# leggedrobotics/wild_visual_navigation

Measured on NVIDIA H100. Metric: frames/sec end-to-end (DINO feat + seg + MLP train-step) at 448x448, higher is better.
Workload: dtype bf16 operands / fp32 accumulate (ViT, STEGO head, per-pixel MLP); fp32 (k-means, train step)

## Files before the change

include/wvn_b200.h:

```cpp
#ifndef WVN_B200_H_
#define WVN_B200_H_

#include <stddef.h>
#include <stdint.h>

#ifdef __cplusplus
extern "C" {
#endif

typedef enum {
  WVN_STATUS_OK = 0,
  WVN_STATUS_INVALID = -1,
  WVN_STATUS_CUDA = -2,
  WVN_STATUS_NO_DEVICE = -3,
  WVN_STATUS_STATE = -4
} wvn_status;

const char* wvn_last_error(void);
int wvn_check_device(void);
int wvn_version(void);
long long wvn_launch_count(void);
void wvn_profile_enable(int category_mask);
int wvn_profile_collect(float* host_ms, long long* host_launches);

int wvn_gemm_bf16(const void* a_bf16, long long lda, const void* w_bf16, const float* bias, void* out, long long ldo,
                  int m, int n, int k, int out_kind, int act, int block_n, void* stream);

typedef struct {
  int m, n, k;
  int epi, act;
  int block_n;
  const void* a;
  long long lda;
  const void* w;
  const float* bias;
  void* out;
  long long ldo;
  const float* pos;
  int tokens_in, npad;
  int dim, heads;
  void* q_out;
  void* k_out;
  void* vt_out;
  int feat, trav_col;
  const void* x;
  long long ldx;
  float* trav;
  float* conf;
  float* loss_reco;
  const float* cg_mean;
  const float* cg_std;
  float cg_std_factor;
  int reverse_m;
  int registers;
  const void* residual;
  long long ldr;
} wvn_gemm_ex_args;
int wvn_gemm_bf16_ex(const wvn_gemm_ex_args* args, void* stream);

int wvn_attention_bf16(const void* q, const void* k, const void* vt, void* out, int batch, int heads, int npad,
                       int n_valid, float scale, void* stream);

int wvn_layernorm(const float* x, const float* gamma, const float* beta, void* out_bf16, long long rows, int dim,
                  float eps, void* stream);

typedef struct wvn_vit wvn_vit_t;

typedef struct {
  int image_size;
  int patch_size;
  int dim;
  int depth;
  int heads;
  int mlp_dim;
  int max_batch;
  int chunk;
  float ln_eps;
  int head_out;
  int registers;
} wvn_vit_config;

int wvn_vit_create(const wvn_vit_config* cfg, wvn_vit_t** out);
void wvn_vit_destroy(wvn_vit_t* h);

int wvn_vit_set_weight(wvn_vit_t* h, const char* name, const float* data, long long numel);

int wvn_vit_forward(wvn_vit_t* h, const float* img, int batch, int in_h, int in_w, int resized_h, int resized_w,
                    float* tokens_out, void* stream);

int wvn_vit_forward_tta(wvn_vit_t* h, const float* img, int batch, int in_h, int in_w, int resized_h, int resized_w,
                        float* tokens_out, void* stream);

int wvn_vit_forward_u8(wvn_vit_t* h, const unsigned char* img_hwc, int batch, int in_h, int in_w, int resized_h,
                       int resized_w, float* tokens_out, void* stream);

int wvn_vit_stego_head(wvn_vit_t* h, int batch, float* out, void* stream);
int wvn_vit_npad(const wvn_vit_t* h);

typedef struct wvn_resnet wvn_resnet_t;

typedef struct {
  int image_size;
  int depth;
  int max_batch;
} wvn_resnet_config;

int wvn_resnet_create(const wvn_resnet_config* cfg, wvn_resnet_t** out);
void wvn_resnet_destroy(wvn_resnet_t* h);
size_t wvn_resnet_workspace_bytes(const wvn_resnet_t* h);
int wvn_resnet_set_weight(wvn_resnet_t* h, const char* name, const float* data, long long numel);
int wvn_resnet_forward(wvn_resnet_t* h, const float* img, int batch, void* const* taps, void* stream);

int wvn_im2col_bf16_nhwc(const void* in, int batch, int h, int w, int c, int k, int stride, int pad, void* out,
                         long long pitch, void* stream);
int wvn_im2col_image(const float* img, int batch, int h, int w, int k, int stride, int pad, void* out, long long pitch,
                     void* stream);
int wvn_maxpool3s2_bf16_nhwc(const void* in, int batch, int h, int w, int c, void* out, void* stream);

int wvn_upsample_dense(const float* tokens, float* out, int batch, int dim, int gh, int gw, int out_h, int out_w,
                       void* stream);
int wvn_logits_argmax(const float* logits, long long ld, int col0, int classes, int col0_b, int classes_b, int batch,
                      int npad, int gh, int gw, int out_h, int out_w, long long* seg, long long* seg_b, void* stream);

int wvn_flip_average(float* head, int batch, int npad, int grid, long long ld, void* stream);
size_t wvn_stego_kmeans_workspace_bytes(int batch, int k, int code_dim);
int wvn_stego_kmeans(float* rows, long long ld, int batch, int npad, int patches, int code_col, int code_dim, int logit_col,
                     int k, int iters, float* centroids_out, void* workspace, void* stream);

size_t wvn_segment_workspace_bytes(int batch, int smax, int gh, int gw);
int wvn_segment_reduce(const long long* seg, int batch, int h, int w, int smax, const float* tokens, int gh, int gw,
                       int dim, float* feat, float* centers, long long* edges, int* n_edges, int max_edges,
                       void* workspace, void* stream);
int wvn_segment_pool_pyramid(const long long* seg, int batch, int h, int w, int smax, const float* centers,
                             void* const* taps, const int* tap_h, const int* tap_w, const int* tap_c, float* out,
                             void* stream);
int wvn_segment_relabel(long long* seg, int batch, long long pix_per_frame, int num_labels, int* scratch, int* counts,
                        void* stream);

int wvn_supervision_pool(const long long* seg, const float* mask, int batch, int channels, int h, int w, int smax,
                         float* y, unsigned char* y_valid, float* count_ws, void* stream);

void wvn_slic_tables(int* g256, int* m9, int* f4096);
int wvn_slic_geometry(int h, int w, int num_components, int* grid_interval, int* nx, int* ny);
size_t wvn_slic_workspace_bytes(int batch, int h, int w, int num_components);
int wvn_slic(const float* img, int batch, int h, int w, int num_components, float compactness, int iters,
             const int* lut_g, const int* lut_m, const int* lut_f, long long* labels, void* workspace, void* stream);

int wvn_project_and_render(const float* K, const float* pose_camera_in_world, const float* points, const float* colors,
                           int color_batched, int batch, int n_points, int h, int w, const float* traversability,
                           float* masks, float* projected, unsigned char* valid, float* supervision_inout, void* stream);

typedef struct wvn_mlp_infer wvn_mlp_infer_t;
int wvn_mlp_infer_create(int dim, int h1, int h2, int chunk_rows, wvn_mlp_infer_t** out);
void wvn_mlp_infer_destroy(wvn_mlp_infer_t* h);
int wvn_mlp_infer_reserve(wvn_mlp_infer_t* h, int tokens_per_frame);
int wvn_mlp_infer_set_params(wvn_mlp_infer_t* h, const float* params, void* stream);
int wvn_mlp_infer_pixels(wvn_mlp_infer_t* h, const float* tokens, int batch, int gh, int gw, int out_h, int out_w,
                         const float* cg_mean, const float* cg_std, float std_factor, float* trav, float* conf,
                         void* stream);
int wvn_mlp_infer_pixels_vit(wvn_mlp_infer_t* h, wvn_vit_t* vit, int batch, int out_h, int out_w, const float* cg_mean,
                             const float* cg_std, float std_factor, float* trav, float* conf, void* stream);
int wvn_mlp_infer_rows(wvn_mlp_infer_t* h, const float* x, long long rows, const float* cg_mean,
                       const float* cg_std, float std_factor, float* trav, float* conf, void* stream);

typedef struct {
  float w_trav, w_reco, std_factor;
  int anomaly_balanced;
  float lr, beta1, beta2, eps;
} wvn_train_config;

size_t wvn_mlp_param_count(int dim, int h1, int h2);
size_t wvn_mlp_train_workspace_bytes(int dim, int h1, int h2, int max_rows);
size_t wvn_mlp_train_scalars_bytes(void);
int wvn_mlp_train_forward_stats(int dim, int h1, int h2, const float* params, const float* x, const float* y,
                                const unsigned char* y_valid, int rows, int max_rows, void* workspace, void* scalars,
                                void* stream);
int wvn_mlp_train_backward(int dim, int h1, int h2, const float* params, const float* x, const float* y,
                           const unsigned char* y_valid, int rows, int max_rows, long long n_total,
                           const wvn_train_config* cfg, void* workspace, void* scalars, float* cg_mean, float* cg_std,
                           float* grads, float* confidence_out, void* stream);
int wvn_mlp_train_apply(int dim, int h1, int h2, float* params, const float* grads, float* exp_avg, float* exp_avg_sq,
                        long long* step_counter, long long n_total, const wvn_train_config* cfg, void* scalars,
                        void* stream);
int wvn_mlp_train_read_metrics(const void* scalars, float* metrics_out, void* stream);
int wvn_mlp_forward_f32(int dim, int h1, int h2, const float* params, const float* x, int rows, float* h1_buf,
                        float* h2_buf, float* out, void* stream);

typedef struct wvn_mlp_trainer wvn_mlp_trainer_t;
size_t wvn_mlp_trainer_scalars_bytes(void);
int wvn_mlp_trainer_create(int dim, int h1, int h2, int max_rows, const wvn_train_config* cfg, void* scalars,
                           float* grads, wvn_mlp_trainer_t** out);
void wvn_mlp_trainer_destroy(wvn_mlp_trainer_t* t);
int wvn_comm_unique_id(void* id128);
int wvn_mlp_trainer_init_comm(wvn_mlp_trainer_t* t, const void* id128, int rank, int world);
int wvn_mlp_trainer_set_confidence(wvn_mlp_trainer_t* t, int method, float* var, double* running_n, double* running_sum,
                                   double* running_sum_of_squares, float kf_proc_cov, float kf_meas_cov);
int wvn_mlp_trainer_copy_confidence(wvn_mlp_trainer_t* dst, const wvn_mlp_trainer_t* src, void* stream);
int wvn_mlp_train_step(wvn_mlp_trainer_t* t, float* params, float* exp_avg, float* exp_avg_sq, long long* step_counter,
                       const float* x, int groups, int rows_per_group, const int* n_rows, const float* y,
                       const unsigned char* y_valid, float* cg_mean, float* cg_std, float* confidence_out,
                       float* metrics_out, int phase_mask, void* stream);

typedef struct wvn_flow wvn_flow_t;
typedef struct {
  const float* mask0;
  const float* mask1;
  const long long* p1;
  const long long* invp1;
  const long long* p3;
  const long long* invp3;
} wvn_flow_buffers;
size_t wvn_flow_param_count(int dim, int hidden);
int wvn_flow_create(int dim, int hidden, int max_rows, const wvn_train_config* cfg, float* grads, wvn_flow_t** out);
void wvn_flow_destroy(wvn_flow_t* h);
int wvn_flow_set_confidence(wvn_flow_t* h, int method, float* var, double* running_n, double* running_sum,
                            double* running_sum_of_squares, float kf_proc_cov, float kf_meas_cov);
int wvn_flow_copy_confidence(wvn_flow_t* dst, const wvn_flow_t* src, void* stream);
int wvn_flow_train_step(wvn_flow_t* h, float* params, float* exp_avg, float* exp_avg_sq, long long* step_counter,
                        const wvn_flow_buffers* buffers, const float* x, int rows, const unsigned char* y_valid,
                        float* cg_mean, float* cg_std, float* confidence_out, float* metrics_out, int phase_mask,
                        void* stream);

typedef struct wvn_flow_infer wvn_flow_infer_t;
int wvn_flow_infer_create(int dim, int hidden, int max_rows, int chunk_pixels, wvn_flow_infer_t** out);
void wvn_flow_infer_destroy(wvn_flow_infer_t* h);
int wvn_flow_infer_set_params(wvn_flow_infer_t* h, const float* params, void* stream);
int wvn_flow_infer_rows(wvn_flow_infer_t* h, const float* params, const wvn_flow_buffers* buffers, const float* x, int rows,
                        float* z, float* log_det, float* logprob, const float* cg_mean, const float* cg_std,
                        float std_factor, float* trav, void* stream);
int wvn_flow_infer_pixels(wvn_flow_infer_t* h, const wvn_flow_buffers* buffers, const float* tokens, int batch, int gh,
                          int gw, int out_h, int out_w, const float* cg_mean, const float* cg_std, float std_factor,
                          float* trav, float* nll, void* stream);

#ifdef __cplusplus
}
#endif
#endif
```

wild_visual_navigation_b200/_C.py:

```python
from __future__ import annotations

import ctypes
import os
from ctypes import POINTER, Structure, byref, c_char_p, c_float, c_int, c_longlong, c_size_t, c_void_p

import torch

_HERE = os.path.dirname(os.path.abspath(__file__))
LIB_PATH = os.environ.get("WVN_B200_LIB", os.path.join(_HERE, "libwvn_b200.so"))


class WvnError(RuntimeError):
    pass


class VitConfig(Structure):
    _fields_ = [
        ("image_size", c_int), ("patch_size", c_int), ("dim", c_int), ("depth", c_int), ("heads", c_int),
        ("mlp_dim", c_int), ("max_batch", c_int), ("chunk", c_int), ("ln_eps", c_float), ("head_out", c_int),
        ("registers", c_int),
    ]


class GemmExArgs(Structure):
    _fields_ = [
        ("m", c_int), ("n", c_int), ("k", c_int), ("epi", c_int), ("act", c_int), ("block_n", c_int),
        ("a", c_void_p), ("lda", c_longlong), ("w", c_void_p), ("bias", c_void_p), ("out", c_void_p), ("ldo", c_longlong),
        ("pos", c_void_p), ("tokens_in", c_int), ("npad", c_int), ("dim", c_int), ("heads", c_int),
        ("q_out", c_void_p), ("k_out", c_void_p), ("vt_out", c_void_p),
        ("feat", c_int), ("trav_col", c_int), ("x", c_void_p), ("ldx", c_longlong), ("trav", c_void_p),
        ("conf", c_void_p), ("loss_reco", c_void_p), ("cg_mean", c_void_p), ("cg_std", c_void_p),
        ("cg_std_factor", c_float), ("reverse_m", c_int), ("registers", c_int), ("residual", c_void_p), ("ldr", c_longlong),
    ]


class ResnetConfig(Structure):
    _fields_ = [("image_size", c_int), ("depth", c_int), ("max_batch", c_int)]


class TrainConfig(Structure):
    _fields_ = [
        ("w_trav", c_float), ("w_reco", c_float), ("std_factor", c_float), ("anomaly_balanced", c_int),
        ("lr", c_float), ("beta1", c_float), ("beta2", c_float), ("eps", c_float),
    ]


class FlowBuffers(Structure):
    _fields_ = [("mask0", c_void_p), ("mask1", c_void_p), ("p1", c_void_p), ("invp1", c_void_p), ("p3", c_void_p),
                ("invp3", c_void_p)]


_lib = None

_P, _I, _L, _F, _S = c_void_p, c_int, c_longlong, c_float, c_size_t
SIGNATURES = {
    "wvn_last_error": (c_char_p, []),
    "wvn_check_device": (_I, []),
    "wvn_version": (_I, []),
    "wvn_launch_count": (_L, []),
    "wvn_profile_enable": (None, [_I]),
    "wvn_profile_collect": (_I, [_P, _P]),
    "wvn_gemm_bf16": (_I, [_P, _L, _P, _P, _P, _L, _I, _I, _I, _I, _I, _I, _P]),
    "wvn_gemm_bf16_ex": (_I, [POINTER(GemmExArgs), _P]),
    "wvn_attention_bf16": (_I, [_P, _P, _P, _P, _I, _I, _I, _I, _F, _P]),
    "wvn_layernorm": (_I, [_P, _P, _P, _P, _L, _I, _F, _P]),
    "wvn_vit_create": (_I, [POINTER(VitConfig), POINTER(_P)]),
    "wvn_vit_destroy": (None, [_P]),
    "wvn_vit_set_weight": (_I, [_P, c_char_p, _P, _L]),
    "wvn_vit_forward": (_I, [_P, _P, _I, _I, _I, _I, _I, _P, _P]),
    "wvn_vit_forward_u8": (_I, [_P, _P, _I, _I, _I, _I, _I, _P, _P]),
    "wvn_vit_forward_tta": (_I, [_P, _P, _I, _I, _I, _I, _I, _P, _P]),
    "wvn_vit_stego_head": (_I, [_P, _I, _P, _P]),
    "wvn_vit_npad": (_I, [_P]),
    "wvn_resnet_create": (_I, [POINTER(ResnetConfig), POINTER(_P)]),
    "wvn_resnet_destroy": (None, [_P]),
    "wvn_resnet_workspace_bytes": (_S, [_P]),
    "wvn_resnet_set_weight": (_I, [_P, c_char_p, _P, _L]),
    "wvn_resnet_forward": (_I, [_P, _P, _I, _P, _P]),
    "wvn_im2col_bf16_nhwc": (_I, [_P, _I, _I, _I, _I, _I, _I, _I, _P, _L, _P]),
    "wvn_im2col_image": (_I, [_P, _I, _I, _I, _I, _I, _I, _P, _L, _P]),
    "wvn_maxpool3s2_bf16_nhwc": (_I, [_P, _I, _I, _I, _I, _P, _P]),
    "wvn_segment_pool_pyramid": (_I, [_P, _I, _I, _I, _I, _P, _P, _P, _P, _P, _P, _P]),
    "wvn_upsample_dense": (_I, [_P, _P, _I, _I, _I, _I, _I, _I, _P]),
    "wvn_logits_argmax": (_I, [_P, _L, _I, _I, _I, _I, _I, _I, _I, _I, _I, _I, _P, _P, _P]),
    "wvn_flip_average": (_I, [_P, _I, _I, _I, _L, _P]),
    "wvn_stego_kmeans_workspace_bytes": (_S, [_I, _I, _I]),
    "wvn_stego_kmeans": (_I, [_P, _L, _I, _I, _I, _I, _I, _I, _I, _I, _P, _P, _P]),
    "wvn_segment_workspace_bytes": (_S, [_I, _I, _I, _I]),
    "wvn_segment_reduce": (_I, [_P, _I, _I, _I, _I, _P, _I, _I, _I, _P, _P, _P, _P, _I, _P, _P]),
    "wvn_segment_relabel": (_I, [_P, _I, _L, _I, _P, _P, _P]),
    "wvn_supervision_pool": (_I, [_P, _P, _I, _I, _I, _I, _I, _P, _P, _P, _P]),
    "wvn_slic_tables": (None, [_P, _P, _P]),
    "wvn_slic_geometry": (_I, [_I, _I, _I, _P, _P, _P]),
    "wvn_slic_workspace_bytes": (_S, [_I, _I, _I, _I]),
    "wvn_slic": (_I, [_P, _I, _I, _I, _I, _F, _I, _P, _P, _P, _P, _P, _P]),
    "wvn_project_and_render": (_I, [_P, _P, _P, _P, _I, _I, _I, _I, _I, _P, _P, _P, _P, _P, _P]),
    "wvn_mlp_infer_create": (_I, [_I, _I, _I, _I, POINTER(_P)]),
    "wvn_mlp_infer_destroy": (None, [_P]),
    "wvn_mlp_infer_reserve": (_I, [_P, _I]),
    "wvn_mlp_infer_set_params": (_I, [_P, _P, _P]),
    "wvn_mlp_infer_pixels": (_I, [_P, _P, _I, _I, _I, _I, _I, _P, _P, _F, _P, _P, _P]),
    "wvn_mlp_infer_pixels_vit": (_I, [_P, _P, _I, _I, _I, _P, _P, _F, _P, _P, _P]),
    "wvn_mlp_infer_rows": (_I, [_P, _P, _L, _P, _P, _F, _P, _P, _P]),
    "wvn_mlp_param_count": (_S, [_I, _I, _I]),
    "wvn_mlp_train_workspace_bytes": (_S, [_I, _I, _I, _I]),
    "wvn_mlp_train_scalars_bytes": (_S, []),
    "wvn_mlp_train_forward_stats": (_I, [_I, _I, _I, _P, _P, _P, _P, _I, _I, _P, _P, _P]),
    "wvn_mlp_train_backward": (_I, [_I, _I, _I, _P, _P, _P, _P, _I, _I, _L, POINTER(TrainConfig), _P, _P, _P, _P, _P, _P, _P]),
    "wvn_mlp_train_apply": (_I, [_I, _I, _I, _P, _P, _P, _P, _P, _L, POINTER(TrainConfig), _P, _P]),
    "wvn_mlp_train_read_metrics": (_I, [_P, _P, _P]),
    "wvn_mlp_forward_f32": (_I, [_I, _I, _I, _P, _P, _I, _P, _P, _P, _P]),
    "wvn_mlp_trainer_scalars_bytes": (_S, []),
    "wvn_mlp_trainer_create": (_I, [_I, _I, _I, _I, POINTER(TrainConfig), _P, _P, POINTER(_P)]),
    "wvn_mlp_trainer_destroy": (None, [_P]),
    "wvn_comm_unique_id": (_I, [_P]),
    "wvn_mlp_trainer_init_comm": (_I, [_P, _P, _I, _I]),
    "wvn_mlp_trainer_set_confidence": (_I, [_P, _I, _P, _P, _P, _P, _F, _F]),
    "wvn_mlp_trainer_copy_confidence": (_I, [_P, _P, _P]),
    "wvn_mlp_train_step": (_I, [_P, _P, _P, _P, _P, _P, _I, _I, _P, _P, _P, _P, _P, _P, _P, _I, _P]),
    "wvn_flow_param_count": (_S, [_I, _I]),
    "wvn_flow_create": (_I, [_I, _I, _I, POINTER(TrainConfig), _P, POINTER(_P)]),
    "wvn_flow_destroy": (None, [_P]),
    "wvn_flow_set_confidence": (_I, [_P, _I, _P, _P, _P, _P, _F, _F]),
    "wvn_flow_copy_confidence": (_I, [_P, _P, _P]),
    "wvn_flow_infer_create": (_I, [_I, _I, _I, _I, POINTER(_P)]),
    "wvn_flow_infer_destroy": (None, [_P]),
    "wvn_flow_infer_set_params": (_I, [_P, _P, _P]),
    "wvn_flow_infer_rows": (_I, [_P, _P, POINTER(FlowBuffers), _P, _I, _P, _P, _P, _P, _P, _F, _P, _P]),
    "wvn_flow_infer_pixels": (_I, [_P, POINTER(FlowBuffers), _P, _I, _I, _I, _I, _I, _P, _P, _F, _P, _P, _P]),
    "wvn_flow_train_step": (_I, [_P, _P, _P, _P, _P, POINTER(FlowBuffers), _P, _I, _P, _P, _P, _P, _P, _I, _P]),
}


def lib() -> ctypes.CDLL:
    global _lib
    if _lib is not None:
        return _lib
    if not os.path.exists(LIB_PATH):
        raise WvnError(
            f"{LIB_PATH} not found: build it with `python -c 'import __graft_entry__ as g; g.build()'` "
            "or `make -C wild_visual_navigation_b200/csrc` (there is no CPU fallback)"
        )
    l = ctypes.CDLL(LIB_PATH)
    for name, (res, args) in SIGNATURES.items():
        fn = getattr(l, name)
        fn.restype = res
        fn.argtypes = args
    _lib = l
    return l


def check(status: int) -> None:
    if status != 0:
        msg = lib().wvn_last_error()
        raise WvnError(f"libwvn_b200 error {status}: {msg.decode() if msg else '?'}")


def require_device() -> None:
    if not torch.cuda.is_available():
        raise WvnError("wild_visual_navigation_b200 needs a CUDA (sm_90a) device; no CPU fallback exists")
    check(lib().wvn_check_device())


def ptr(t) -> c_void_p:
    if t is None:
        return c_void_p(0)
    assert t.is_cuda and t.is_contiguous(), "expected a contiguous CUDA tensor"
    return c_void_p(t.data_ptr())


def stream() -> c_void_p:
    return c_void_p(torch.cuda.current_stream().cuda_stream)
```

wild_visual_navigation_b200/csrc/api.cu:

```cuda
#include <cuda_bf16.h>

#include <stdio.h>
#include <stdlib.h>

#include <map>
#include <string>
#include <vector>

#include "../../include/wvn_b200.h"
#include "attention.h"
#include "dense_kernels.h"
#include "gemm.h"
#include "host_common.h"
#include "mlp_train.h"
#include "mlp_train_fused.h"
#include "pixel_head.h"
#include "resnet_kernels.h"
#include "segment_kernels.h"
#include "flow_train.h"
#include "footprint_kernels.h"
#include "slic_kernels.h"
#include "stego_kmeans.h"
#include "train_core.h"
#include "vit_kernels.h"

using namespace wvn;

namespace {

inline cudaStream_t S(void* s) { return reinterpret_cast<cudaStream_t>(s); }
inline int round_up(int v, int m) { return (v + m - 1) / m * m; }

__global__ void cast_f32_to_bf16_kernel(const float* __restrict__ src, __nv_bfloat16* __restrict__ dst, long long n) {
  for (long long i = blockIdx.x * static_cast<long long>(blockDim.x) + threadIdx.x; i < n;
       i += static_cast<long long>(gridDim.x) * blockDim.x)
    dst[i] = __float2bfloat16_rn(src[i]);
}

__global__ void cast_rows_kernel(const float* __restrict__ src, __nv_bfloat16* __restrict__ dst, long long rows, int dim,
                                 long long ld) {
  const long long n = rows * dim;
  for (long long i = blockIdx.x * static_cast<long long>(blockDim.x) + threadIdx.x; i < n;
       i += static_cast<long long>(gridDim.x) * blockDim.x) {
    const long long r = i / dim;
    const int c = static_cast<int>(i - r * dim);
    dst[r * ld + c] = __float2bfloat16_rn(src[i]);
  }
}

int cast_to_bf16(const float* src, void* dst, long long n, cudaStream_t s) {
  if (n <= 0) return WVN_OK;
  int blocks = static_cast<int>(std::min<long long>((n + 255) / 256, 4096));
  cast_f32_to_bf16_kernel<<<blocks, 256, 0, s>>>(src, reinterpret_cast<__nv_bfloat16*>(dst), n);
  WVN_CHECK_LAUNCH("cast_f32_to_bf16_kernel");
  return WVN_OK;
}

struct DevBuf {
  void* p = nullptr;
  size_t bytes = 0;
  int alloc(size_t n) {
    bytes = n;
    WVN_CHECK_CUDA(cudaMalloc(&p, n ? n : 1));
    WVN_CHECK_CUDA(cudaMemset(p, 0, n ? n : 1));
    return WVN_OK;
  }
  void release() {
    if (p) cudaFree(p);
    p = nullptr;
  }
};

struct Weight {
  void* p = nullptr;
  long long numel = 0;
  bool bf16 = false;
  bool loaded = false;
  int cols = 0, ld = 0;
};

}

struct wvn_vit {
  wvn_vit_config cfg;
  int grid = 0, P = 0, t0 = 1, n_valid = 0, npad = 0, kpe = 0, kpe_ld = 0, chunk = 0;
  std::map<std::string, Weight> w;
  std::vector<DevBuf> owned;
  DevBuf x, xn, q, k, vt, attn, hid, ape, stage;
  DevBuf tok_bf16, head_hidden;
  DevBuf qkv_f32;
  bool precise = false;
  bool forwarded = false;
  int last_batch = 0;

  int add_weight(const std::string& name, long long numel, bool bf16, int cols = 0, int ld = 0) {
    DevBuf b;
    const long long stored = cols > 0 ? numel / cols * ld : numel;
    WVN_PROPAGATE(b.alloc(static_cast<size_t>(stored) * (bf16 ? 2 : 4)));
    owned.push_back(b);
    Weight wt;
    wt.p = b.p; wt.numel = numel; wt.bf16 = bf16; wt.cols = cols; wt.ld = ld;
    w[name] = wt;
    return WVN_OK;
  }
  template <class T>
  T* wp(const std::string& name) { return reinterpret_cast<T*>(w[name].p); }
};

extern "C" {

const char* wvn_last_error(void) { return last_error(); }
int wvn_version(void) { return 104; }

int wvn_check_device(void) {
  int n = 0;
  if (cudaGetDeviceCount(&n) != cudaSuccess || n == 0) return set_error(WVN_ERR_NO_DEVICE, "no CUDA device visible");
  int dev = 0;
  cudaGetDevice(&dev);
  int major = 0;
  cudaDeviceGetAttribute(&major, cudaDevAttrComputeCapabilityMajor, dev);
  int minor = 0;
  cudaDeviceGetAttribute(&minor, cudaDevAttrComputeCapabilityMinor, dev);
  if (major != 9 || minor != 0)
    return set_error(WVN_ERR_NO_DEVICE, "device %d has compute capability %d.%d, need 9.0 (sm_90a)", dev, major, minor);
  return WVN_OK;
}

long long wvn_launch_count(void) { return launch_count(); }
void wvn_profile_enable(int category_mask) { prof_enable(category_mask); }
int wvn_profile_collect(float* host_ms, long long* host_launches) {
  WVN_REQUIRE(host_ms && host_launches, "wvn_profile_collect: null argument");
  return prof_collect(host_ms, host_launches);
}

int wvn_gemm_bf16(const void* a, long long lda, const void* w, const float* bias, void* out, long long ldo, int m, int n,
                  int k, int out_kind, int act, int block_n, void* stream) {
  GemmArgs g;
  g.M = m; g.N = n; g.K = k;
  g.epi = out_kind == 0 ? EPI_BF16 : (out_kind == 1 ? EPI_F32 : EPI_RESID_F32);
  WVN_REQUIRE(out_kind >= 0 && out_kind <= 2, "wvn_gemm_bf16: out_kind %d", out_kind);
  g.act = act; g.bias = bias; g.out = out; g.ldo = ldo;
  return gemm_bf16(g, a, lda, w, block_n, S(stream));
}

int wvn_gemm_bf16_ex(const wvn_gemm_ex_args* x, void* stream) {
  WVN_REQUIRE(x, "wvn_gemm_bf16_ex: null argument");
  GemmArgs g;
  g.M = x->m; g.N = x->n; g.K = x->k; g.epi = x->epi; g.act = x->act;
  g.bias = x->bias; g.out = x->out; g.ldo = x->ldo;
  g.pos = x->pos; g.tokens_in = x->tokens_in; g.npad = x->npad;
  g.dim = x->dim; g.heads = x->heads; g.q = x->q_out; g.k = x->k_out; g.vt = x->vt_out;
  g.feat = x->feat; g.trav_col = x->trav_col; g.x = x->x; g.ldx = x->ldx; g.trav = x->trav; g.conf = x->conf;
  g.loss_reco = x->loss_reco; g.cg_mean = x->cg_mean; g.cg_std = x->cg_std; g.cg_std_factor = x->cg_std_factor;
  g.reverse_m = x->reverse_m; g.registers = x->registers;
  g.residual = x->residual; g.ldr = x->ldr;
  return gemm_bf16(g, x->a, x->lda, x->w, x->block_n, S(stream));
}

int wvn_attention_bf16(const void* q, const void* k, const void* vt, void* out, int batch, int heads, int npad,
                       int n_valid, float scale, void* stream) {
  AttnArgs a;
  a.batch = batch; a.heads = heads; a.npad = npad; a.n_valid = n_valid;
  a.scale_log2 = scale * 1.4426950408889634f;
  a.out = out; a.ldo = static_cast<long long>(heads) * 64;
  return attention_bf16(a, q, k, vt, S(stream));
}

int wvn_layernorm(const float* x, const float* gamma, const float* beta, void* out_bf16, long long rows, int dim,
                  float eps, void* stream) {
  LayerNormArgs a;
  a.rows = rows; a.dim = dim; a.eps = eps;
  return layernorm_rows(x, gamma, beta, out_bf16, nullptr, a, S(stream));
}

int wvn_vit_create(const wvn_vit_config* cfg, wvn_vit_t** out) {
  WVN_REQUIRE(cfg && out, "wvn_vit_create: null argument");
  WVN_PROPAGATE(wvn_check_device());
  WVN_REQUIRE(cfg->dim == 384 || cfg->dim == 768, "vit: dim %d unsupported (384, 768)", cfg->dim);
  WVN_REQUIRE(cfg->heads * 64 == cfg->dim, "vit: heads*64 must equal dim");
  WVN_REQUIRE(cfg->patch_size == 8 || cfg->patch_size == 14 || cfg->patch_size == 16, "vit: patch size %d unsupported",
              cfg->patch_size);
  WVN_REQUIRE(cfg->image_size >= cfg->patch_size, "vit: image size too small");
  WVN_REQUIRE(cfg->mlp_dim % 64 == 0 && cfg->depth > 0 && cfg->max_batch > 0, "vit: bad mlp_dim/depth/max_batch");
  WVN_REQUIRE(cfg->head_out % 64 == 0, "vit: head_out must be a multiple of 64");
  WVN_REQUIRE(cfg->registers >= 0, "vit: registers must be >= 0");
  WVN_REQUIRE(cfg->registers == 0 || cfg->head_out == 0, "vit: register tokens and a STEGO head cannot be combined");
  wvn_vit* h = new wvn_vit();
  h->cfg = *cfg;
  if (h->cfg.ln_eps <= 0.f) h->cfg.ln_eps = 1e-6f;
  h->grid = cfg->image_size / cfg->patch_size;
  h->P = h->grid * h->grid;
  h->t0 = 1 + cfg->registers;
  h->n_valid = h->t0 + h->P;
  h->npad = round_up(h->n_valid, 128);
  h->kpe = 3 * cfg->patch_size * cfg->patch_size;
  h->kpe_ld = patch_pitch(cfg->patch_size);
  h->chunk = cfg->chunk > 0 ? cfg->chunk : 8;
  if (h->chunk > cfg->max_batch) h->chunk = cfg->max_batch;
  const int D = cfg->dim;
  int rc = WVN_OK;
  auto add = [&](const std::string& n, long long numel, bool bf) { if (rc == WVN_OK) rc = h->add_weight(n, numel, bf); };
  add("cls_token", D, false);
  add("pos_embed", static_cast<long long>(1 + h->P) * D, false);
  if (cfg->registers > 0) add("register_tokens", static_cast<long long>(cfg->registers) * D, false);
  if (rc == WVN_OK) rc = h->add_weight("patch_embed.proj.weight", static_cast<long long>(D) * h->kpe, true, h->kpe, h->kpe_ld);
  add("patch_embed.proj.bias", D, false);
  for (int i = 0; i < cfg->depth; ++i) {
    const std::string b = "blocks." + std::to_string(i) + ".";
    add(b + "norm1.weight", D, false);
    add(b + "norm1.bias", D, false);
    add(b + "attn.qkv.weight", 3ll * D * D, true);
    add(b + "attn.qkv.bias", 3 * D, false);
    add(b + "attn.proj.weight", static_cast<long long>(D) * D, true);
    add(b + "attn.proj.bias", D, false);
    add(b + "norm2.weight", D, false);
    add(b + "norm2.bias", D, false);
    add(b + "mlp.fc1.weight", static_cast<long long>(cfg->mlp_dim) * D, true);
    add(b + "mlp.fc1.bias", cfg->mlp_dim, false);
    add(b + "mlp.fc2.weight", static_cast<long long>(D) * cfg->mlp_dim, true);
    add(b + "mlp.fc2.bias", D, false);
  }
  add("norm.weight", D, false);
  add("norm.bias", D, false);
  if (cfg->head_out > 0) {
    add("stego.head_a.weight", static_cast<long long>(cfg->head_out) * D, true);
    add("stego.head_a.bias", cfg->head_out, false);
    add("stego.hidden.weight", static_cast<long long>(D) * D, true);
    add("stego.hidden.bias", D, false);
    add("stego.head_b.weight", static_cast<long long>(cfg->head_out) * D, true);
  }
  const size_t rows = static_cast<size_t>(h->chunk) * h->npad;
  const size_t bh = static_cast<size_t>(h->chunk) * cfg->heads;
  auto alloc = [&](DevBuf& b, size_t bytes) { if (rc == WVN_OK) rc = b.alloc(bytes); };
  alloc(h->x, rows * D * 4);
  alloc(h->xn, rows * D * 2);
  alloc(h->q, bh * h->npad * 64 * 2);
  alloc(h->k, bh * h->npad * 64 * 2);
  alloc(h->vt, bh * 64 * h->npad * 2);
  alloc(h->attn, rows * D * 2);
  alloc(h->hid, rows * cfg->mlp_dim * 2);
  alloc(h->ape, static_cast<size_t>(h->chunk) * h->P * h->kpe_ld * 2);
  alloc(h->stage, 8u << 20);
  alloc(h->tok_bf16, static_cast<size_t>(cfg->max_batch) * h->npad * D * 2);
  if (cfg->head_out > 0) alloc(h->head_hidden, static_cast<size_t>(cfg->max_batch) * h->npad * D * 2);
  {
    const char* e = getenv("WVN_VIT_PRECISE");
    h->precise = e && atoi(e) == 1;
    if (h->precise) alloc(h->qkv_f32, rows * 3 * D * 4);
  }
  if (rc != WVN_OK) {
    wvn_vit_destroy(h);
    return rc;
  }
  *out = h;
  return WVN_OK;
}

void wvn_vit_destroy(wvn_vit_t* h) {
  if (!h) return;
  for (auto& b : h->owned) b.release();
  for (DevBuf* b : {&h->x, &h->xn, &h->q, &h->k, &h->vt, &h->attn, &h->hid, &h->ape, &h->stage, &h->tok_bf16,
                    &h->head_hidden, &h->qkv_f32})
    b->release();
  delete h;
}

int wvn_vit_npad(const wvn_vit_t* h) { return h ? h->npad : 0; }

static int load_weight(Weight& wt, DevBuf& stage, const char* name, const float* data, long long numel) {
  WVN_REQUIRE(wt.numel == numel, "set_weight: '%s' expects %lld elements, got %lld", name, wt.numel, numel);
  cudaPointerAttributes attr;
  bool on_device = false;
  if (cudaPointerGetAttributes(&attr, data) == cudaSuccess)
    on_device = (attr.type == cudaMemoryTypeDevice || attr.type == cudaMemoryTypeManaged);
  else
    cudaGetLastError();
  if (!wt.bf16) {
    WVN_CHECK_CUDA(cudaMemcpy(wt.p, data, numel * 4, on_device ? cudaMemcpyDeviceToDevice : cudaMemcpyHostToDevice));
  } else if (wt.cols > 0) {
    const long long chunk_rows = static_cast<long long>(stage.bytes / 4) / wt.cols;
    const long long rows = numel / wt.cols;
    for (long long r0 = 0; r0 < rows; r0 += chunk_rows) {
      const long long n = std::min(chunk_rows, rows - r0);
      const float* src = data + r0 * wt.cols;
      if (!on_device) {
        WVN_CHECK_CUDA(cudaMemcpy(stage.p, src, n * wt.cols * 4, cudaMemcpyHostToDevice));
        src = reinterpret_cast<const float*>(stage.p);
      }
      const int blocks = static_cast<int>(std::min<long long>((n * wt.cols + 255) / 256, 4096));
      cast_rows_kernel<<<blocks, 256, 0, 0>>>(src, reinterpret_cast<__nv_bfloat16*>(wt.p) + r0 * wt.ld, n, wt.cols, wt.ld);
      WVN_CHECK_LAUNCH("cast_rows_kernel");
      WVN_CHECK_CUDA(cudaStreamSynchronize(0));
    }
  } else {
    const long long chunk_elems = static_cast<long long>(stage.bytes / 4);
    for (long long off = 0; off < numel; off += chunk_elems) {
      const long long n = std::min(chunk_elems, numel - off);
      const float* src = data + off;
      if (!on_device) {
        WVN_CHECK_CUDA(cudaMemcpy(stage.p, src, n * 4, cudaMemcpyHostToDevice));
        src = reinterpret_cast<const float*>(stage.p);
      }
      WVN_PROPAGATE(cast_to_bf16(src, reinterpret_cast<__nv_bfloat16*>(wt.p) + off, n, 0));
      WVN_CHECK_CUDA(cudaStreamSynchronize(0));
    }
  }
  wt.loaded = true;
  return WVN_OK;
}


int wvn_vit_set_weight(wvn_vit_t* h, const char* name, const float* data, long long numel) {
  WVN_REQUIRE(h && name && data, "wvn_vit_set_weight: null argument");
  auto it = h->w.find(name);
  WVN_REQUIRE(it != h->w.end(), "wvn_vit_set_weight: unknown weight '%s'", name);
  return load_weight(it->second, h->stage, name, data, numel);
}

static int vit_check_loaded(wvn_vit* h, bool need_head) {
  for (auto& kv : h->w) {
    const bool is_head = kv.first.rfind("stego.", 0) == 0;
    if (is_head && !need_head) continue;
    if (!kv.second.loaded) return set_error(WVN_ERR_STATE, "vit: weight '%s' was never set", kv.first.c_str());
  }
  return WVN_OK;
}

constexpr int kDefaultSubAttn = 1 << 30;

namespace {
int vit_forward_impl(wvn_vit_t* h, const void* img, bool u8_hwc, int batch, int in_h, int in_w, int resized_h, int resized_w,
                     float* tokens_out, void* stream, bool flip_tta = false);
}

int wvn_vit_forward_tta(wvn_vit_t* h, const float* img, int batch, int in_h, int in_w, int resized_h, int resized_w,
                        float* tokens_out, void* stream) {
  return vit_forward_impl(h, img, false, batch, in_h, in_w, resized_h, resized_w, tokens_out, stream, true);
}

int wvn_vit_forward(wvn_vit_t* h, const float* img, int batch, int in_h, int in_w, int resized_h, int resized_w,
                    float* tokens_out, void* stream) {
  return vit_forward_impl(h, img, false, batch, in_h, in_w, resized_h, resized_w, tokens_out, stream);
}

int wvn_vit_forward_u8(wvn_vit_t* h, const unsigned char* img_hwc, int batch, int in_h, int in_w, int resized_h,
                       int resized_w, float* tokens_out, void* stream) {
  return vit_forward_impl(h, img_hwc, true, batch, in_h, in_w, resized_h, resized_w, tokens_out, stream);
}

namespace {
int vit_forward_impl(wvn_vit_t* h, const void* img, bool u8_hwc, int src_batch, int in_h, int in_w, int resized_h, int resized_w,
                     float* tokens_out, void* stream, bool flip_tta) {
  const int batch = flip_tta ? 2 * src_batch : src_batch;
  WVN_REQUIRE(h && img, "wvn_vit_forward: null argument");
  WVN_REQUIRE(batch > 0 && batch <= h->cfg.max_batch, "wvn_vit_forward: batch %d outside (0, %d]", batch, h->cfg.max_batch);
  WVN_REQUIRE(resized_h >= h->cfg.image_size && resized_w >= h->cfg.image_size,
              "wvn_vit_forward: resized image %dx%d smaller than the crop %d", resized_h, resized_w, h->cfg.image_size);
  WVN_PROPAGATE(vit_check_loaded(h, false));
  cudaStream_t s = S(stream);
  const wvn_vit_config& c = h->cfg;
  const int D = c.dim;

  ImagePatchArgs ia;
  ia.in_h = in_h; ia.in_w = in_w; ia.patch = c.patch_size; ia.grid_h = h->grid; ia.grid_w = h->grid;
  ia.crop_top = static_cast<int>(lrintf((resized_h - c.image_size) / 2.0f));
  ia.crop_left = static_cast<int>(lrintf((resized_w - c.image_size) / 2.0f));
  ia.scale_y = static_cast<float>(in_h) / static_cast<float>(resized_h);
  ia.scale_x = static_cast<float>(in_w) / static_cast<float>(resized_w);

  for (int b0 = 0; b0 < batch; b0 += h->chunk) {
    const int nb = std::min(h->chunk, batch - b0);
    const int rows = nb * h->npad;
    float* x = reinterpret_cast<float*>(h->x.p);
    ia.batch = nb;
    ia.frame0 = b0; ia.src_frames = src_batch; ia.flip_from = flip_tta ? src_batch : (1 << 30);
    WVN_PROPAGATE(image_to_patches(img, u8_hwc, h->ape.p, ia, s));
    const float* reg = c.registers > 0 ? h->wp<float>("register_tokens") : nullptr;
    WVN_PROPAGATE(init_token_rows(x, h->wp<float>("cls_token"), h->wp<float>("pos_embed"), reg, c.registers, nb, h->npad,
                                  h->n_valid, D, s));
    {
      GemmArgs g;
      g.M = nb * h->P; g.N = D; g.K = h->kpe; g.epi = EPI_PATCH; g.bias = h->wp<float>("patch_embed.proj.bias");
      g.out = x; g.ldo = D; g.pos = h->wp<float>("pos_embed"); g.tokens_in = h->P; g.npad = h->npad;
      g.registers = c.registers;
      WVN_PROPAGATE(gemm_bf16(g, h->ape.p, h->kpe_ld, h->wp<void>("patch_embed.proj.weight"), 0, s));
    }
    LayerNormArgs la;
    la.rows = rows; la.dim = D; la.eps = c.ln_eps; la.npad = h->npad; la.n_valid = h->n_valid; la.row0 = h->t0;
    static int sub_env = -1;
    if (sub_env < 0) {
      const char* e = getenv("WVN_VIT_SUBCHUNK");
      sub_env = e ? atoi(e) : (1 << 30);
      if (sub_env < 1) sub_env = 1 << 30;
    }
    const int sub = std::min(sub_env, nb);
    static int snake = -1;
    if (snake < 0) { const char* e = getenv("WVN_VIT_SNAKE"); snake = (e && atoi(e) == 0) ? 0 : 1; }
    int dir = 0;
    auto next_dir = [&]() { dir = snake ? dir ^ 1 : 0; return dir; };
    __nv_bfloat16* xn = reinterpret_cast<__nv_bfloat16*>(h->xn.p);
    __nv_bfloat16* attn = reinterpret_cast<__nv_bfloat16*>(h->attn.p);
    static int sub_attn_env = -1;
    if (sub_attn_env < 0) {
      const char* e = getenv("WVN_VIT_SUB_ATTN");
      sub_attn_env = e ? atoi(e) : kDefaultSubAttn;
      if (sub_attn_env < 1) sub_attn_env = 1 << 30;
    }
    const int sub_a = std::min(sub_attn_env, nb);
    for (int l = 0; l < c.depth; ++l) {
      const std::string b = "blocks." + std::to_string(l) + ".";
      for (int s0 = 0; s0 < nb; s0 += sub_a) {
        const int ns = std::min(sub_a, nb - s0);
        const long long roff = static_cast<long long>(s0) * h->npad;
        LayerNormArgs ls = la;
        ls.rows = static_cast<long long>(ns) * h->npad;
        ls.reverse = next_dir();
        WVN_PROPAGATE(layernorm_rows(x + roff * D, h->wp<float>(b + "norm1.weight"), h->wp<float>(b + "norm1.bias"),
                                     xn + roff * D, nullptr, ls, s));
        if (h->precise) {
          GemmArgs g;
          float* qkv = reinterpret_cast<float*>(h->qkv_f32.p) + roff * 3 * D;
          g.M = ns * h->npad; g.N = 3 * D; g.K = D; g.epi = EPI_F32; g.bias = h->wp<float>(b + "attn.qkv.bias");
          g.out = qkv; g.ldo = 3 * D;
          WVN_PROPAGATE(gemm_bf16(g, xn + roff * D, D, h->wp<void>(b + "attn.qkv.weight"), 0, s));
          WVN_PROPAGATE(attention_f32_debug(qkv, attn + roff * D, ns, c.heads, h->npad, h->n_valid, D, 0.125f, s));
          continue;
        }
        GemmArgs g;
        g.M = ns * h->npad; g.N = 3 * D; g.K = D; g.epi = EPI_QKV; g.bias = h->wp<float>(b + "attn.qkv.bias");
        g.npad = h->npad; g.dim = D; g.heads = c.heads;
        const long long hoff = static_cast<long long>(s0) * c.heads * h->npad * 64;
        g.q = reinterpret_cast<__nv_bfloat16*>(h->q.p) + hoff;
        g.k = reinterpret_cast<__nv_bfloat16*>(h->k.p) + hoff;
        g.vt = reinterpret_cast<__nv_bfloat16*>(h->vt.p) + hoff;
        g.reverse_m = next_dir();
        WVN_PROPAGATE(gemm_bf16(g, xn + roff * D, D, h->wp<void>(b + "attn.qkv.weight"), 0, s));
        AttnArgs a;
        a.batch = ns; a.heads = c.heads; a.npad = h->npad; a.n_valid = h->n_valid;
        a.scale_log2 = 0.125f * 1.4426950408889634f;
        a.out = attn + roff * D; a.ldo = D;
        a.reverse = next_dir();
        WVN_PROPAGATE(attention_bf16(a, g.q, g.k, g.vt, s));
      }
      for (int s0 = 0; s0 < nb; s0 += sub) {
        const int ns = std::min(sub, nb - s0);
        const long long roff = static_cast<long long>(s0) * h->npad;
        const int srows = ns * h->npad;
        LayerNormArgs ls = la;
        ls.rows = srows;
        {
          GemmArgs g;
          g.M = srows; g.N = D; g.K = D; g.epi = EPI_RESID_F32; g.bias = h->wp<float>(b + "attn.proj.bias");
          g.out = x + roff * D; g.ldo = D;
          g.reverse_m = next_dir();
          WVN_PROPAGATE(gemm_bf16(g, attn + roff * D, D, h->wp<void>(b + "attn.proj.weight"), 0, s));
        }
        ls.reverse = next_dir();
        WVN_PROPAGATE(layernorm_rows(x + roff * D, h->wp<float>(b + "norm2.weight"), h->wp<float>(b + "norm2.bias"),
                                     xn + roff * D, nullptr, ls, s));
        {
          GemmArgs g;
          g.M = srows; g.N = c.mlp_dim; g.K = D; g.epi = EPI_BF16; g.act = ACT_GELU;
          g.bias = h->wp<float>(b + "mlp.fc1.bias"); g.out = h->hid.p; g.ldo = c.mlp_dim;
          g.reverse_m = next_dir();
          WVN_PROPAGATE(gemm_bf16(g, xn + roff * D, D, h->wp<void>(b + "mlp.fc1.weight"), 0, s));
        }
        {
          GemmArgs g;
          g.M = srows; g.N = D; g.K = c.mlp_dim; g.epi = EPI_RESID_F32; g.bias = h->wp<float>(b + "mlp.fc2.bias");
          g.out = x + roff * D; g.ldo = D;
          g.reverse_m = next_dir();
          WVN_PROPAGATE(gemm_bf16(g, h->hid.p, c.mlp_dim, h->wp<void>(b + "mlp.fc2.weight"), 0, s));
        }
      }
    }
    __nv_bfloat16* tok_bf = reinterpret_cast<__nv_bfloat16*>(h->tok_bf16.p) + static_cast<long long>(b0) * h->npad * D;
    float* tok_f = tokens_out ? tokens_out + static_cast<long long>(b0) * h->P * D : nullptr;
    la.reverse = next_dir();
    WVN_PROPAGATE(layernorm_rows(x, h->wp<float>("norm.weight"), h->wp<float>("norm.bias"), tok_bf, tok_f, la, s));
  }
  h->forwarded = true;
  h->last_batch = batch;
  return WVN_OK;
}
}

int wvn_vit_stego_head(wvn_vit_t* h, int batch, float* out, void* stream) {
  WVN_REQUIRE(h && out, "wvn_vit_stego_head: null argument");
  WVN_REQUIRE(h->cfg.head_out > 0, "wvn_vit_stego_head: handle was created without a head");
  WVN_REQUIRE(h->forwarded && batch == h->last_batch, "wvn_vit_stego_head: call wvn_vit_forward with the same batch first");
  WVN_PROPAGATE(vit_check_loaded(h, true));
  cudaStream_t s = S(stream);
  const int D = h->cfg.dim, rows = batch * h->npad, HO = h->cfg.head_out;
  GemmArgs g;
  g.M = rows; g.N = D; g.K = D; g.epi = EPI_BF16; g.act = ACT_RELU; g.bias = h->wp<float>("stego.hidden.bias");
  g.out = h->head_hidden.p; g.ldo = D;
  WVN_PROPAGATE(gemm_bf16(g, h->tok_bf16.p, D, h->wp<void>("stego.hidden.weight"), 0, s));
  GemmArgs a;
  a.M = rows; a.N = HO; a.K = D; a.epi = EPI_F32; a.bias = h->wp<float>("stego.head_a.bias"); a.out = out; a.ldo = HO;
  WVN_PROPAGATE(gemm_bf16(a, h->tok_bf16.p, D, h->wp<void>("stego.head_a.weight"), 0, s));
  GemmArgs b;
  b.M = rows; b.N = HO; b.K = D; b.epi = EPI_RESID_F32; b.bias = nullptr; b.out = out; b.ldo = HO;
  WVN_PROPAGATE(gemm_bf16(b, h->head_hidden.p, D, h->wp<void>("stego.head_b.weight"), 0, s));
  return WVN_OK;
}

int wvn_upsample_dense(const float* tokens, float* out, int batch, int dim, int gh, int gw, int out_h, int out_w,
                       void* stream) {
  DenseArgs a;
  a.batch = batch; a.dim = dim; a.grid_h = gh; a.grid_w = gw; a.out_h = out_h; a.out_w = out_w;
  a.scale_y = out_h > 1 ? static_cast<float>(gh - 1) / static_cast<float>(out_h - 1) : 0.f;
  a.scale_x = out_w > 1 ? static_cast<float>(gw - 1) / static_cast<float>(out_w - 1) : 0.f;
  return upsample_tokens_dense(tokens, out, a, S(stream));
}

int wvn_logits_argmax(const float* logits, long long ld, int col0, int classes, int col0_b, int classes_b, int batch,
                      int npad, int gh, int gw, int out_h, int out_w, long long* seg, long long* seg_b, void* stream) {
  LogitsArgs a;
  a.batch = batch; a.classes = classes; a.grid_h = gh; a.grid_w = gw; a.out_h = out_h; a.out_w = out_w;
  a.scale_y = static_cast<float>(gh) / static_cast<float>(out_h);
  a.scale_x = static_cast<float>(gw) / static_cast<float>(out_w);
  a.npad = npad; a.ld = ld; a.col0 = col0; a.col0_b = col0_b; a.classes_b = classes_b;
  return logits_argmax(logits, seg, seg_b, a, S(stream));
}

int wvn_flip_average(float* head, int batch, int npad, int grid, long long ld, void* stream) {
  return flip_average(head, batch, npad, grid, ld, S(stream));
}

size_t wvn_stego_kmeans_workspace_bytes(int batch, int k, int code_dim) { return stego_kmeans_workspace_bytes(batch, k, code_dim); }

int wvn_stego_kmeans(float* rows, long long ld, int batch, int npad, int patches, int code_col, int code_dim, int logit_col,
                     int k, int iters, float* centroids_out, void* workspace, void* stream) {
  KmeansArgs a;
  a.batch = batch; a.npad = npad; a.patches = patches; a.ld = ld; a.code_col = code_col; a.code_dim = code_dim;
  a.logit_col = logit_col; a.k = k; a.iters = iters; a.centroids_out = centroids_out;
  return stego_kmeans(rows, a, reinterpret_cast<float*>(workspace), S(stream));
}

static void seg_ws_layout(int batch, int smax, int gh, int gw, size_t& off_w, size_t& off_adj, size_t& total) {
  const size_t stats = static_cast<size_t>(batch) * smax * 3 * sizeof(unsigned long long);
  off_w = (stats + 255) / 256 * 256;
  const size_t wbytes = static_cast<size_t>(batch) * smax * gh * gw * sizeof(float);
  off_adj = off_w + (wbytes + 255) / 256 * 256;
  total = off_adj + static_cast<size_t>(batch) * smax * ((smax + 31) / 32) * sizeof(unsigned int);
}

size_t wvn_segment_workspace_bytes(int batch, int smax, int gh, int gw) {
  size_t a, b, t;
  seg_ws_layout(batch, smax, gh, gw, a, b, t);
  return t;
}

int wvn_segment_reduce(const long long* seg, int batch, int h, int w, int smax, const float* tokens, int gh, int gw,
                       int dim, float* feat, float* centers, long long* edges, int* n_edges, int max_edges,
                       void* workspace, void* stream) {
  WVN_REQUIRE(seg && workspace, "wvn_segment_reduce: null argument");
  WVN_REQUIRE(feat == nullptr || tokens != nullptr, "wvn_segment_reduce: feat requested without tokens");
  WVN_REQUIRE((edges == nullptr) == (n_edges == nullptr), "wvn_segment_reduce: edges and n_edges go together");
  WVN_REQUIRE(feat == nullptr || w <= h, "wvn_segment_reduce: segment map %dx%d is wider than the (h, h) feature map", h, w);
  size_t off_w, off_adj, total;
  seg_ws_layout(batch, smax, gh, gw, off_w, off_adj, total);
  char* ws = reinterpret_cast<char*>(workspace);
  unsigned long long* stats = reinterpret_cast<unsigned long long*>(ws);
  float* wseg = feat ? reinterpret_cast<float*>(ws + off_w) : nullptr;
  unsigned int* adj = edges ? reinterpret_cast<unsigned int*>(ws + off_adj) : nullptr;
  SegmentArgs a;
  a.batch = batch; a.h = h; a.w = w; a.smax = smax; a.grid_h = gh; a.grid_w = gw; a.dim = dim;
  a.scale_y = h > 1 ? static_cast<float>(gh - 1) / static_cast<float>(h - 1) : 0.f;
  a.scale_x = h > 1 ? static_cast<float>(gw - 1) / static_cast<float>(h - 1) : 0.f;
  WVN_PROPAGATE(segment_accumulate(seg, a, stats, wseg, adj, S(stream)));
  if (feat || centers) WVN_PROPAGATE(segment_pool(wseg, tokens, stats, feat, centers, a, S(stream)));
  if (edges) WVN_PROPAGATE(adjacency_emit(adj, edges, n_edges, batch, smax, max_edges, S(stream)));
  return WVN_OK;
}

int wvn_segment_relabel(long long* seg, int batch, long long pix_per_frame, int num_labels, int* scratch, int* counts,
                        void* stream) {
  return relabel_compact(seg, scratch, counts, batch, pix_per_frame, num_labels, S(stream));
}

int wvn_supervision_pool(const long long* seg, const float* mask, int batch, int channels, int h, int w, int smax,
                         float* y, unsigned char* y_valid, float* count_ws, void* stream) {
  WVN_REQUIRE(seg && mask && y && y_valid && count_ws, "wvn_supervision_pool: null argument");
  return supervision_pool(seg, mask, batch, channels, h, w, smax, y, y_valid, count_ws, S(stream));
}

void wvn_slic_tables(int* g256, int* m9, int* f4096) { slic_tables(g256, m9, f4096); }

int wvn_slic_geometry(int h, int w, int num_components, int* grid_interval, int* nx, int* ny) {
  WVN_REQUIRE(h > 0 && w > 0 && num_components > 0 && grid_interval && nx && ny, "wvn_slic_geometry: bad argument");
  slic_geometry(h, w, num_components, grid_interval, nx, ny);
  return WVN_OK;
}

size_t wvn_slic_workspace_bytes(int batch, int h, int w, int num_components) {
  return slic_workspace_bytes(batch, h, w, num_components);
}

int wvn_slic(const float* img, int batch, int h, int w, int num_components, float compactness, int iters,
             const int* lut_g, const int* lut_m, const int* lut_f, long long* labels, void* workspace, void* stream) {
  WVN_REQUIRE(img && lut_g && lut_m && lut_f && labels && workspace, "wvn_slic: null argument");
  return slic_segment(img, batch, h, w, num_components, compactness, iters, lut_g, lut_m, lut_f, labels, workspace,
                      S(stream));
}

int wvn_project_and_render(const float* K, const float* pose_camera_in_world, const float* points, const float* colors,
                           int color_batched, int batch, int n_points, int h, int w, const float* traversability,
                           float* masks, float* projected, unsigned char* valid, float* supervision_inout, void* stream) {
  WVN_REQUIRE(K && pose_camera_in_world && points, "wvn_project_and_render: null argument");
  WVN_REQUIRE(colors || (!masks && !supervision_inout), "wvn_project_and_render: colors are required to render");
  FootprintArgs a;
  a.batch = batch; a.n_points = n_points; a.h = h; a.w = w; a.color_batched = color_batched;
  return footprint_render(a, K, pose_camera_in_world, points, colors, traversability, masks, projected, valid,
                          supervision_inout, S(stream));
}

}

struct wvn_resnet {
  wvn_resnet_config cfg;
  int bottleneck = 0;
  std::map<std::string, Weight> w;
  std::vector<DevBuf> owned;
  DevBuf stage, col;
  DevBuf act[5];
};

namespace {

enum ResnetPass { RN_REGISTER, RN_SIZE, RN_RUN };

const int kBlocks18[4] = {2, 2, 2, 2};
const int kBlocks50[4] = {3, 4, 6, 3};

struct ResnetRun {
  wvn_resnet* h;
  ResnetPass pass;
  int batch;
  cudaStream_t s;
  size_t need_col = 0, need_act[5] = {0, 0, 0, 0, 0};
  int rc = WVN_OK;

  void conv(const std::string& name, const void* in, int H, int W, int C, int k, int stride, int pad, int Cout,
            void* out, int role, bool relu, const void* residual, int* Ho_, int* Wo_, const float* img = nullptr,
            bool stem = false) {
    const int Ho = (H + 2 * pad - k) / stride + 1, Wo = (W + 2 * pad - k) / stride + 1;
    *Ho_ = Ho; *Wo_ = Wo;
    if (rc != WVN_OK) return;
    const int K = k * k * C;
    const long long M = static_cast<long long>(batch) * Ho * Wo;
    const bool direct = k == 1 && stride == 1 && !stem;
    const long long pitch = gemm_w_pitch(K);
    if (pass == RN_REGISTER) {
      wvn_resnet& r = *h;
      DevBuf b;
      if ((rc = b.alloc(static_cast<size_t>(Cout) * pitch * 2)) != WVN_OK) return;
      r.owned.push_back(b);
      Weight wt;
      wt.p = b.p; wt.numel = static_cast<long long>(Cout) * K; wt.bf16 = true; wt.cols = K; wt.ld = static_cast<int>(pitch);
      r.w[name + ".weight"] = wt;
      DevBuf bb;
      if ((rc = bb.alloc(static_cast<size_t>(Cout) * 4)) != WVN_OK) return;
      r.owned.push_back(bb);
      Weight wb;
      wb.p = bb.p; wb.numel = Cout;
      r.w[name + ".bias"] = wb;
      return;
    }
    if (pass == RN_SIZE) {
      if (!direct) need_col = std::max(need_col, static_cast<size_t>(M * pitch * 2));
      if (role >= 0) need_act[role] = std::max(need_act[role], static_cast<size_t>(M * Cout * 2));
      return;
    }
    const void* A = in;
    long long lda = C;
    if (!direct) {
      rc = stem ? im2col_image(img, batch, H, W, k, stride, pad, h->col.p, pitch, s)
               : im2col_nhwc(in, batch, H, W, C, k, stride, pad, h->col.p, pitch, s);
      if (rc != WVN_OK) return;
      A = h->col.p;
      lda = pitch;
    }
    if (M > 0x7fffffff) {
      rc = set_error(WVN_ERR_INVALID, "resnet: %lld output rows", M);
      return;
    }
    GemmArgs g;
    g.M = static_cast<int>(M); g.N = Cout; g.K = K;
    g.epi = residual ? EPI_BF16_RESID : EPI_BF16;
    g.act = relu ? ACT_RELU : ACT_NONE;
    g.bias = reinterpret_cast<const float*>(h->w[name + ".bias"].p);
    g.out = out; g.ldo = Cout;
    g.residual = residual; g.ldr = Cout;
    rc = gemm_bf16(g, A, lda, h->w[name + ".weight"].p, 0, s);
  }

  void walk(const float* img, void* const* taps) {
    const int S = h->cfg.image_size;
    const bool bn = h->bottleneck != 0;
    const int* blocks = bn ? kBlocks50 : kBlocks18;
    void* A[5];
    for (int i = 0; i < 5; ++i) A[i] = h->act[i].p;
    void* T[4] = {nullptr, nullptr, nullptr, nullptr};
    if (taps) for (int i = 0; i < 4; ++i) T[i] = taps[i];
    int Ho, Wo;
    conv("conv1", nullptr, S, S, 3, 7, 2, 3, 64, A[2], 2, true, nullptr, &Ho, &Wo, img, true);
    int H = (Ho - 1) / 2 + 1, W = (Wo - 1) / 2 + 1, C = 64;
    if (pass == RN_SIZE) need_act[0] = std::max(need_act[0], static_cast<size_t>(batch) * H * W * C * 2);
    if (pass == RN_RUN && rc == WVN_OK) rc = maxpool3s2_nhwc(A[2], batch, Ho, Wo, 64, A[0], s);
    const void* cur = A[0];
    int cur_role = 0;
    for (int L = 1; L <= 4; ++L) {
      const int planes = 64 << (L - 1), out_c = bn ? planes * 4 : planes;
      for (int blk = 0; blk < blocks[L - 1]; ++blk) {
        const std::string p = "layer" + std::to_string(L) + "." + std::to_string(blk) + ".";
        const int stride = (blk == 0 && L > 1) ? 2 : 1;
        const int out_role = cur_role == 0 ? 1 : 0;
        const bool out_tap = bn ? (L == 4 && blk == blocks[3] - 1) : (blk == blocks[L - 1] - 1);
        void* out = out_tap ? T[bn ? 3 : L - 1] : A[out_role];
        int h1, w1, h2, w2, hd, wd;
        const void* res = cur;
        if (blk == 0 && (stride != 1 || C != out_c)) {
          conv(p + "downsample", cur, H, W, C, 1, stride, 0, out_c, A[4], 4, false, nullptr, &hd, &wd);
          res = A[4];
        }
        if (bn) {
          const bool t1_tap = blk == 0 && L >= 2;
          void* t1 = t1_tap ? T[L - 2] : A[2];
          conv(p + "conv1", cur, H, W, C, 1, 1, 0, planes, t1, t1_tap ? -1 : 2, true, nullptr, &h1, &w1);
          conv(p + "conv2", t1, h1, w1, planes, 3, stride, 1, planes, A[3], 3, true, nullptr, &h2, &w2);
          conv(p + "conv3", A[3], h2, w2, planes, 1, 1, 0, out_c, out, out_tap ? -1 : out_role, true, res, &H, &W);
        } else {
          conv(p + "conv1", cur, H, W, C, 3, stride, 1, planes, A[2], 2, true, nullptr, &h1, &w1);
          conv(p + "conv2", A[2], h1, w1, planes, 3, 1, 1, out_c, out, out_tap ? -1 : out_role, true, res, &H, &W);
        }
        C = out_c;
        cur = out;
        cur_role = out_tap ? -1 : out_role;
      }
    }
  }
};

}

extern "C" {

int wvn_resnet_create(const wvn_resnet_config* cfg, wvn_resnet_t** out) {
  WVN_REQUIRE(cfg && out, "wvn_resnet_create: null argument");
  WVN_PROPAGATE(wvn_check_device());
  WVN_REQUIRE(cfg->depth == 18 || cfg->depth == 50, "resnet: depth %d unsupported (18, 50)", cfg->depth);
  WVN_REQUIRE(cfg->image_size >= 32 && cfg->image_size % 32 == 0, "resnet: image size %d must be a multiple of 32",
              cfg->image_size);
  WVN_REQUIRE(cfg->max_batch > 0, "resnet: max_batch must be positive");
  wvn_resnet* h = new wvn_resnet();
  h->cfg = *cfg;
  h->bottleneck = cfg->depth == 50;
  ResnetRun reg{h, RN_REGISTER, cfg->max_batch, 0};
  reg.walk(nullptr, nullptr);
  ResnetRun size{h, RN_SIZE, cfg->max_batch, 0};
  size.walk(nullptr, nullptr);
  int rc = reg.rc;
  auto alloc = [&](DevBuf& b, size_t bytes) { if (rc == WVN_OK) rc = b.alloc(bytes); };
  alloc(h->stage, 8u << 20);
  alloc(h->col, size.need_col);
  for (int i = 0; i < 5; ++i) alloc(h->act[i], size.need_act[i]);
  if (rc != WVN_OK) {
    wvn_resnet_destroy(h);
    return rc;
  }
  *out = h;
  return WVN_OK;
}

void wvn_resnet_destroy(wvn_resnet_t* h) {
  if (!h) return;
  for (auto& b : h->owned) b.release();
  h->stage.release();
  h->col.release();
  for (auto& b : h->act) b.release();
  delete h;
}

size_t wvn_resnet_workspace_bytes(const wvn_resnet_t* h) {
  if (!h) return 0;
  size_t n = h->col.bytes;
  for (const auto& b : h->act) n += b.bytes;
  return n;
}

int wvn_resnet_set_weight(wvn_resnet_t* h, const char* name, const float* data, long long numel) {
  WVN_REQUIRE(h && name && data, "wvn_resnet_set_weight: null argument");
  auto it = h->w.find(name);
  WVN_REQUIRE(it != h->w.end(), "wvn_resnet_set_weight: unknown weight '%s'", name);
  return load_weight(it->second, h->stage, name, data, numel);
}

int wvn_resnet_forward(wvn_resnet_t* h, const float* img, int batch, void* const* taps, void* stream) {
  WVN_REQUIRE(h && img && taps, "wvn_resnet_forward: null argument");
  WVN_REQUIRE(batch > 0 && batch <= h->cfg.max_batch, "wvn_resnet_forward: batch %d outside (0, %d]", batch,
              h->cfg.max_batch);
  for (int i = 0; i < 4; ++i) WVN_REQUIRE(taps[i], "wvn_resnet_forward: tap %d is null", i);
  for (auto& kv : h->w)
    if (!kv.second.loaded) return set_error(WVN_ERR_STATE, "resnet: weight '%s' was never set", kv.first.c_str());
  ResnetRun run{h, RN_RUN, batch, S(stream)};
  run.walk(img, taps);
  return run.rc;
}

int wvn_im2col_bf16_nhwc(const void* in, int batch, int h, int w, int c, int k, int stride, int pad, void* out,
                         long long pitch, void* stream) {
  return im2col_nhwc(in, batch, h, w, c, k, stride, pad, out, pitch, S(stream));
}

int wvn_im2col_image(const float* img, int batch, int h, int w, int k, int stride, int pad, void* out, long long pitch,
                     void* stream) {
  return im2col_image(img, batch, h, w, k, stride, pad, out, pitch, S(stream));
}

int wvn_maxpool3s2_bf16_nhwc(const void* in, int batch, int h, int w, int c, void* out, void* stream) {
  return maxpool3s2_nhwc(in, batch, h, w, c, out, S(stream));
}

int wvn_segment_pool_pyramid(const long long* seg, int batch, int h, int w, int smax, const float* centers,
                             void* const* taps, const int* tap_h, const int* tap_w, const int* tap_c, float* out,
                             void* stream) {
  WVN_REQUIRE(taps && tap_h && tap_w && tap_c, "wvn_segment_pool_pyramid: null argument");
  PyramidArgs a;
  a.batch = batch; a.h = h; a.w = w; a.smax = smax;
  for (int l = 0; l < 4; ++l) {
    a.taps[l] = taps[l]; a.th[l] = tap_h[l]; a.tw[l] = tap_w[l]; a.tc[l] = tap_c[l];
  }
  return segment_pool_pyramid(seg, centers, a, out, S(stream));
}

}

struct wvn_mlp_infer {
  int dim, h1, h2;
  int dim_p, h1_p, h2_p, n3, n3_p, bn3, trav_col;
  int chunk_rows;
  DevBuf w1, b1, w2, b2, w3, b3;
  DevBuf x, a1, a2;
  DevBuf wcat, bias_cat, head_consts, tok_bf16, gu, gram;
  int fused_tokens = 0;
  int force_unfused = 0;
  bool loaded = false;
};

static constexpr int kFusedFrames = 8;

namespace {

__global__ void pack_mlp_kernel(const float* __restrict__ p, MlpOffsets o, int dim, int h1, int h2, int dim_p, int h1_p,
                                int h2_p, int n3_p, int trav_col, __nv_bfloat16* w1, float* b1, __nv_bfloat16* w2,
                                float* b2, __nv_bfloat16* w3, float* b3) {
  const long long n1 = static_cast<long long>(h1_p) * dim_p, n2 = static_cast<long long>(h2_p) * h1_p,
                  n3 = static_cast<long long>(n3_p) * h2_p;
  const long long total = n1 + n2 + n3 + h1_p + h2_p + n3_p;
  for (long long i = blockIdx.x * static_cast<long long>(blockDim.x) + threadIdx.x; i < total;
       i += static_cast<long long>(gridDim.x) * blockDim.x) {
    long long j = i;
    if (j < n1) {
      const int r = static_cast<int>(j / dim_p), c = static_cast<int>(j % dim_p);
      w1[j] = __float2bfloat16_rn((r < h1 && c < dim) ? p[o.w1 + static_cast<long long>(r) * dim + c] : 0.f);
      continue;
    }
    j -= n1;
    if (j < n2) {
      const int r = static_cast<int>(j / h1_p), c = static_cast<int>(j % h1_p);
      w2[j] = __float2bfloat16_rn((r < h2 && c < h1) ? p[o.w2 + static_cast<long long>(r) * h1 + c] : 0.f);
      continue;
    }
    j -= n2;
    if (j < n3) {
      const int r = static_cast<int>(j / h2_p), c = static_cast<int>(j % h2_p);
      int src = -1;
      if (r < dim) src = 1 + r; else if (r == trav_col) src = 0;
      w3[j] = __float2bfloat16_rn((src >= 0 && c < h2) ? p[o.w3 + static_cast<long long>(src) * h2 + c] : 0.f);
      continue;
    }
    j -= n3;
    if (j < h1_p) { b1[j] = j < h1 ? p[o.b1 + j] : 0.f; continue; }
    j -= h1_p;
    if (j < h2_p) { b2[j] = j < h2 ? p[o.b2 + j] : 0.f; continue; }
    j -= h2_p;
    {
      int src = -1;
      if (j < dim) src = 1 + static_cast<int>(j); else if (j == trav_col) src = 0;
      b3[j] = src >= 0 ? p[o.b3 + src] : 0.f;
    }
  }
}

int mlp_infer_chunk(wvn_mlp_infer* h, long long rows, long long row0, const float* cg_mean, const float* cg_std,
                    float std_factor, float* trav, float* conf, cudaStream_t s) {
  GemmArgs g1;
  g1.M = static_cast<int>(rows); g1.N = h->h1_p; g1.K = h->dim_p; g1.epi = EPI_BF16; g1.act = ACT_RELU;
  g1.bias = reinterpret_cast<float*>(h->b1.p); g1.out = h->a1.p; g1.ldo = h->h1_p;
  WVN_PROPAGATE(gemm_bf16(g1, h->x.p, h->dim_p, h->w1.p, 0, s));
  GemmArgs g2;
  g2.M = static_cast<int>(rows); g2.N = h->h2_p; g2.K = h->h1_p; g2.epi = EPI_BF16; g2.act = ACT_RELU;
  g2.bias = reinterpret_cast<float*>(h->b2.p); g2.out = h->a2.p; g2.ldo = h->h2_p;
  WVN_PROPAGATE(gemm_bf16(g2, h->a1.p, h->h1_p, h->w2.p, 0, s));
  GemmArgs g3;
  g3.M = static_cast<int>(rows); g3.N = h->n3_p; g3.K = h->h2_p; g3.epi = EPI_MLP_HEAD;
  g3.bias = reinterpret_cast<float*>(h->b3.p); g3.feat = h->dim; g3.trav_col = h->trav_col; g3.x = h->x.p;
  g3.ldx = h->dim_p; g3.trav = trav + row0; g3.conf = conf + row0; g3.cg_mean = cg_mean; g3.cg_std = cg_std;
  g3.cg_std_factor = std_factor;
  WVN_PROPAGATE(gemm_bf16(g3, h->a2.p, h->h2_p, h->w3.p, h->bn3, s));
  return WVN_OK;
}

}

extern "C" {

int wvn_mlp_infer_create(int dim, int h1, int h2, int chunk_rows, wvn_mlp_infer_t** out) {
  WVN_REQUIRE(out && dim > 0 && h1 > 0 && h2 > 0, "wvn_mlp_infer_create: bad arguments");
  WVN_PROPAGATE(wvn_check_device());
  wvn_mlp_infer* h = new wvn_mlp_infer();
  h->dim = dim; h->h1 = h1; h->h2 = h2;
  h->dim_p = round_up(dim, 64); h->h1_p = round_up(h1, 64); h->h2_p = round_up(h2, 64);
  h->trav_col = round_up(dim, 32);
  h->n3 = h->trav_col + 1;
  int best_bn = 64, best_n = round_up(h->n3, 64);
  for (int bn : {128, 192, 224, 256}) {
    const int n = round_up(h->n3, bn);
    if (n <= best_n) { best_n = n; best_bn = bn; }
  }
  h->bn3 = best_bn; h->n3_p = best_n;
  h->chunk_rows = chunk_rows > 0 ? round_up(chunk_rows, 128) : sm_count() * 128 * 3;
  int rc = WVN_OK;
  auto alloc = [&](DevBuf& b, size_t bytes) { if (rc == WVN_OK) rc = b.alloc(bytes); };
  alloc(h->w1, static_cast<size_t>(h->h1_p) * h->dim_p * 2);
  alloc(h->b1, static_cast<size_t>(h->h1_p) * 4);
  alloc(h->w2, static_cast<size_t>(h->h2_p) * h->h1_p * 2);
  alloc(h->b2, static_cast<size_t>(h->h2_p) * 4);
  alloc(h->w3, static_cast<size_t>(h->n3_p) * h->h2_p * 2);
  alloc(h->b3, static_cast<size_t>(h->n3_p) * 4);
  alloc(h->x, static_cast<size_t>(h->chunk_rows) * h->dim_p * 2);
  alloc(h->a1, static_cast<size_t>(h->chunk_rows) * h->h1_p * 2);
  alloc(h->a2, static_cast<size_t>(h->chunk_rows) * h->h2_p * 2);
  alloc(h->wcat, static_cast<size_t>(kPixelHeadN) * h->dim_p * 2);
  alloc(h->bias_cat, static_cast<size_t>(kPixelHeadN) * 4);
  alloc(h->head_consts, sizeof(PixelHeadConsts));
  {
    const char* e = getenv("WVN_PIXEL_HEAD");
    h->force_unfused = (e && std::string(e) == "unfused") ? 1 : 0;
  }
  if (rc != WVN_OK) {
    wvn_mlp_infer_destroy(h);
    return rc;
  }
  *out = h;
  return WVN_OK;
}

void wvn_mlp_infer_destroy(wvn_mlp_infer_t* h) {
  if (!h) return;
  for (DevBuf* b : {&h->w1, &h->b1, &h->w2, &h->b2, &h->w3, &h->b3, &h->x, &h->a1, &h->a2, &h->wcat, &h->bias_cat,
                    &h->head_consts, &h->tok_bf16, &h->gu, &h->gram})
    b->release();
  delete h;
}

int wvn_mlp_infer_reserve(wvn_mlp_infer_t* h, int tokens_per_frame) {
  WVN_REQUIRE(h && tokens_per_frame > 0, "wvn_mlp_infer_reserve: bad arguments");
  const int P = tokens_per_frame;
  if (h->fused_tokens >= kFusedFrames * P) return WVN_OK;
  for (DevBuf* b : {&h->tok_bf16, &h->gu, &h->gram}) b->release();
  WVN_PROPAGATE(h->tok_bf16.alloc(static_cast<size_t>(kFusedFrames) * P * h->dim_p * 2));
  WVN_PROPAGATE(h->gu.alloc(static_cast<size_t>(kFusedFrames) * P * kPixelHeadN * 4));
  WVN_PROPAGATE(h->gram.alloc(static_cast<size_t>(kFusedFrames) * P * 5 * 4));
  h->fused_tokens = kFusedFrames * P;
  return WVN_OK;
}

int wvn_mlp_infer_set_params(wvn_mlp_infer_t* h, const float* params, void* stream) {
  WVN_REQUIRE(h && params, "wvn_mlp_infer_set_params: null argument");
  MlpShape sh;
  sh.dim = h->dim; sh.h1 = h->h1; sh.h2 = h->h2;
  pack_mlp_kernel<<<256, 256, 0, S(stream)>>>(
      params, mlp_offsets(sh), h->dim, h->h1, h->h2, h->dim_p, h->h1_p, h->h2_p, h->n3_p, h->trav_col,
      reinterpret_cast<__nv_bfloat16*>(h->w1.p), reinterpret_cast<float*>(h->b1.p),
      reinterpret_cast<__nv_bfloat16*>(h->w2.p), reinterpret_cast<float*>(h->b2.p),
      reinterpret_cast<__nv_bfloat16*>(h->w3.p), reinterpret_cast<float*>(h->b3.p));
  WVN_CHECK_LAUNCH("pack_mlp_kernel");
  if (h->h1 == 256 && h->h2 == 32)
    WVN_PROPAGATE(pixel_head_pack(params, sh, h->dim_p, h->wcat.p, reinterpret_cast<float*>(h->bias_cat.p),
                                  reinterpret_cast<PixelHeadConsts*>(h->head_consts.p), S(stream)));
  h->loaded = true;
  return WVN_OK;
}

static int pixels_fused_chunk(wvn_mlp_infer_t* h, const void* tok_bf16, long long frame_rows, int row0, int b0, int nb,
                              int gh, int gw, int out_h, int out_w, int ww, const float* cg_mean, const float* cg_std,
                              float std_factor, float* trav, float* conf, cudaStream_t s) {
  const long long rows = static_cast<long long>(nb) * frame_rows;
  GemmArgs g;
  g.M = static_cast<int>(rows); g.N = kPixelHeadN; g.K = h->dim_p; g.epi = EPI_F32;
  g.bias = reinterpret_cast<float*>(h->bias_cat.p); g.out = h->gu.p; g.ldo = kPixelHeadN;
  WVN_PROPAGATE(gemm_bf16(g, tok_bf16, h->dim_p, h->wcat.p, 64, s));
  WVN_PROPAGATE(token_gram(tok_bf16, reinterpret_cast<float*>(h->gram.p), nb, gh, gw, h->dim_p, frame_rows, row0, s));
  PixelHeadArgs a;
  a.gu = reinterpret_cast<float*>(h->gu.p); a.ldg = kPixelHeadN; a.gram = reinterpret_cast<float*>(h->gram.p);
  a.consts = reinterpret_cast<PixelHeadConsts*>(h->head_consts.p);
  a.cg_mean = cg_mean; a.cg_std = cg_std; a.std_factor = std_factor;
  a.trav = trav + static_cast<long long>(b0) * out_h * out_w;
  a.conf = conf + static_cast<long long>(b0) * out_h * out_w;
  a.batch = nb; a.gh = gh; a.gw = gw; a.H = out_h; a.W = out_w;
  a.sy = static_cast<float>(gh - 1) / static_cast<float>(out_h - 1);
  a.sx = static_cast<float>(gw - 1) / static_cast<float>(out_w - 1);
  a.ww = ww; a.feat = h->dim;
  a.frame_rows = frame_rows; a.row0 = row0;
  WVN_PROPAGATE(pixel_head(a, h->w2.p, h->h1_p, s));
  return WVN_OK;
}

int wvn_mlp_infer_pixels_vit(wvn_mlp_infer_t* h, wvn_vit_t* vit, int batch, int out_h, int out_w, const float* cg_mean,
                             const float* cg_std, float std_factor, float* trav, float* conf, void* stream) {
  WVN_REQUIRE(h && vit && trav && conf && cg_mean && cg_std, "wvn_mlp_infer_pixels_vit: null argument");
  if (!h->loaded) return set_error(WVN_ERR_STATE, "wvn_mlp_infer_pixels_vit: parameters were never set");
  if (!vit->forwarded || batch > vit->last_batch)
    return set_error(WVN_ERR_STATE, "wvn_mlp_infer_pixels_vit: the backbone holds the tokens of %d frames, %d asked",
                     vit->forwarded ? vit->last_batch : 0, batch);
  WVN_REQUIRE(h->dim == vit->cfg.dim && h->dim_p == vit->cfg.dim, "wvn_mlp_infer_pixels_vit: the MLP takes %d-d features, "
              "the backbone's tokens are %d-d", h->dim, vit->cfg.dim);
  const int g = vit->grid;
  const int ww = pixel_head_supported(h->h1, h->h2, g, g, out_h, out_w);
  WVN_REQUIRE(ww > 0, "wvn_mlp_infer_pixels_vit: geometry outside the fused per-pixel head (use wvn_mlp_infer_pixels)");
  if (h->fused_tokens < kFusedFrames * vit->npad) WVN_PROPAGATE(wvn_mlp_infer_reserve(h, vit->npad));
  for (int b0 = 0; b0 < batch; b0 += kFusedFrames) {
    const int nb = std::min(kFusedFrames, batch - b0);
    const __nv_bfloat16* tok = reinterpret_cast<const __nv_bfloat16*>(vit->tok_bf16.p) +
                               static_cast<long long>(b0) * vit->npad * vit->cfg.dim;
    WVN_PROPAGATE(pixels_fused_chunk(h, tok, vit->npad, vit->t0, b0, nb, g, g, out_h, out_w, ww, cg_mean, cg_std, std_factor, trav,
                                     conf, S(stream)));
  }
  return WVN_OK;
}

int wvn_mlp_infer_pixels(wvn_mlp_infer_t* h, const float* tokens, int batch, int gh, int gw, int out_h, int out_w,
                         const float* cg_mean, const float* cg_std, float std_factor, float* trav, float* conf,
                         void* stream) {
  WVN_REQUIRE(h && tokens && trav && conf && cg_mean && cg_std, "wvn_mlp_infer_pixels: null argument");
  if (!h->loaded) return set_error(WVN_ERR_STATE, "wvn_mlp_infer_pixels: parameters were never set");
  cudaStream_t s = S(stream);
  const int ww = h->force_unfused ? 0 : pixel_head_supported(h->h1, h->h2, gh, gw, out_h, out_w);
  if (ww > 0) {
    const int P = gh * gw;
    if (h->fused_tokens < kFusedFrames * P) WVN_PROPAGATE(wvn_mlp_infer_reserve(h, P));
    for (int b0 = 0; b0 < batch; b0 += kFusedFrames) {
      const int nb = std::min(kFusedFrames, batch - b0);
      const long long rows = static_cast<long long>(nb) * P;
      const long long elems = rows * h->dim;
      int blocks = static_cast<int>(std::min<long long>((elems + 255) / 256, 8192));
      cast_rows_kernel<<<blocks, 256, 0, s>>>(tokens + static_cast<long long>(b0) * P * h->dim,
                                             reinterpret_cast<__nv_bfloat16*>(h->tok_bf16.p), rows, h->dim, h->dim_p);
      WVN_CHECK_LAUNCH("cast_rows_kernel");
      WVN_PROPAGATE(pixels_fused_chunk(h, h->tok_bf16.p, P, 0, b0, nb, gh, gw, out_h, out_w, ww, cg_mean, cg_std,
                                       std_factor, trav, conf, s));
    }
    return WVN_OK;
  }
  DenseArgs d;
  d.batch = batch; d.dim = h->dim; d.grid_h = gh; d.grid_w = gw; d.out_h = out_h; d.out_w = out_w;
  d.scale_y = out_h > 1 ? static_cast<float>(gh - 1) / static_cast<float>(out_h - 1) : 0.f;
  d.scale_x = out_w > 1 ? static_cast<float>(gw - 1) / static_cast<float>(out_w - 1) : 0.f;
  d.ld_out = h->dim_p;
  const long long total = static_cast<long long>(batch) * out_h * out_w;
  for (long long p0 = 0; p0 < total; p0 += h->chunk_rows) {
    const long long n = std::min<long long>(h->chunk_rows, total - p0);
    WVN_PROPAGATE(interp_pixel_rows(tokens, h->x.p, d, p0, n, s));
    WVN_PROPAGATE(mlp_infer_chunk(h, n, p0, cg_mean, cg_std, std_factor, trav, conf, s));
  }
  return WVN_OK;
}

int wvn_mlp_infer_rows(wvn_mlp_infer_t* h, const float* x, long long rows, const float* cg_mean, const float* cg_std,
                       float std_factor, float* trav, float* conf, void* stream) {
  WVN_REQUIRE(h && x && trav && conf && cg_mean && cg_std, "wvn_mlp_infer_rows: null argument");
  if (!h->loaded) return set_error(WVN_ERR_STATE, "wvn_mlp_infer_rows: parameters were never set");
  cudaStream_t s = S(stream);
  for (long long r0 = 0; r0 < rows; r0 += h->chunk_rows) {
    const long long n = std::min<long long>(h->chunk_rows, rows - r0);
    const long long elems = n * h->dim;
    int blocks = static_cast<int>(std::min<long long>((elems + 255) / 256, 8192));
    cast_rows_kernel<<<blocks, 256, 0, s>>>(x + r0 * h->dim, reinterpret_cast<__nv_bfloat16*>(h->x.p), n, h->dim,
                                           h->dim_p);
    WVN_CHECK_LAUNCH("cast_rows_kernel");
    WVN_PROPAGATE(mlp_infer_chunk(h, n, r0, cg_mean, cg_std, std_factor, trav, conf, s));
  }
  return WVN_OK;
}

static MlpShape shape_of(int dim, int h1, int h2) {
  MlpShape s;
  s.dim = dim; s.h1 = h1; s.h2 = h2;
  return s;
}
static LossCfg loss_of(const wvn_train_config* c) {
  LossCfg l;
  l.w_trav = c->w_trav; l.w_reco = c->w_reco; l.std_factor = c->std_factor; l.anomaly_balanced = c->anomaly_balanced;
  return l;
}

size_t wvn_mlp_param_count(int dim, int h1, int h2) { return mlp_param_count(shape_of(dim, h1, h2)); }
size_t wvn_mlp_train_workspace_bytes(int dim, int h1, int h2, int max_rows) {
  return mlp_train_workspace_floats(shape_of(dim, h1, h2), max_rows) * sizeof(float);
}
size_t wvn_mlp_train_scalars_bytes(void) { return sizeof(TrainScalars); }

int wvn_mlp_train_forward_stats(int dim, int h1, int h2, const float* params, const float* x, const float* y,
                                const unsigned char* y_valid, int rows, int max_rows, void* workspace, void* scalars,
                                void* stream) {
  WVN_REQUIRE(params && x && y && y_valid && workspace && scalars, "wvn_mlp_train_forward_stats: null argument");
  return mlp_train_forward_stats(shape_of(dim, h1, h2), params, x, y, y_valid, rows, max_rows,
                                 reinterpret_cast<float*>(workspace), reinterpret_cast<TrainScalars*>(scalars), S(stream));
}

int wvn_mlp_train_backward(int dim, int h1, int h2, const float* params, const float* x, const float* y,
                           const unsigned char* y_valid, int rows, int max_rows, long long n_total,
                           const wvn_train_config* cfg, void* workspace, void* scalars, float* cg_mean, float* cg_std,
                           float* grads, float* confidence_out, void* stream) {
  WVN_REQUIRE(params && x && y && y_valid && workspace && scalars && cfg && grads && confidence_out,
              "wvn_mlp_train_backward: null argument");
  return mlp_train_backward(shape_of(dim, h1, h2), params, x, y, y_valid, rows, max_rows, n_total, loss_of(cfg),
                            reinterpret_cast<float*>(workspace), reinterpret_cast<TrainScalars*>(scalars), cg_mean,
                            cg_std, grads, confidence_out, S(stream));
}

int wvn_mlp_train_apply(int dim, int h1, int h2, float* params, const float* grads, float* exp_avg, float* exp_avg_sq,
                        long long* step_counter, long long n_total, const wvn_train_config* cfg, void* scalars,
                        void* stream) {
  WVN_REQUIRE(params && grads && exp_avg && exp_avg_sq && step_counter && cfg && scalars,
              "wvn_mlp_train_apply: null argument");
  const long long n = static_cast<long long>(mlp_param_count(shape_of(dim, h1, h2)));
  WVN_PROPAGATE(mlp_train_finalize(reinterpret_cast<TrainScalars*>(scalars), grads, n, n_total, loss_of(cfg), S(stream)));
  AdamCfg a;
  a.lr = cfg->lr; a.beta1 = cfg->beta1; a.beta2 = cfg->beta2; a.eps = cfg->eps;
  return mlp_adam_step(params, grads, exp_avg, exp_avg_sq, n, a, step_counter, S(stream));
}

__global__ void read_metrics_kernel(const TrainScalars* sc, float* out) {
  out[0] = sc->loss_total; out[1] = sc->loss_trav; out[2] = sc->loss_reco; out[3] = sc->loss_trav_conf;
  out[4] = sc->mean; out[5] = sc->std;
}

int wvn_mlp_train_read_metrics(const void* scalars, float* metrics_out, void* stream) {
  WVN_REQUIRE(scalars && metrics_out, "wvn_mlp_train_read_metrics: null argument");
  read_metrics_kernel<<<1, 1, 0, S(stream)>>>(reinterpret_cast<const TrainScalars*>(scalars), metrics_out);
  WVN_CHECK_LAUNCH("read_metrics_kernel");
  return WVN_OK;
}

int wvn_mlp_forward_f32(int dim, int h1, int h2, const float* params, const float* x, int rows, float* h1_buf,
                        float* h2_buf, float* out, void* stream) {
  WVN_REQUIRE(params && x && h1_buf && h2_buf && out && rows > 0, "wvn_mlp_forward_f32: bad argument");
  return mlp_forward_f32(shape_of(dim, h1, h2), params, x, rows, h1_buf, h2_buf, out, S(stream));
}


struct wvn_mlp_trainer {
  FusedTrainer* impl = nullptr;
};

size_t wvn_mlp_trainer_scalars_bytes(void) { return sizeof(FusedScalars); }

int wvn_mlp_trainer_create(int dim, int h1, int h2, int max_rows, const wvn_train_config* cfg, void* scalars, float* grads,
                           wvn_mlp_trainer_t** out) {
  WVN_REQUIRE(cfg && out, "wvn_mlp_trainer_create: null argument");
  WVN_PROPAGATE(wvn_check_device());
  AdamCfg a;
  a.lr = cfg->lr; a.beta1 = cfg->beta1; a.beta2 = cfg->beta2; a.eps = cfg->eps;
  FusedTrainer* impl = nullptr;
  WVN_PROPAGATE(fused_trainer_create(shape_of(dim, h1, h2), max_rows, loss_of(cfg), a, scalars, grads, &impl));
  wvn_mlp_trainer* t = new wvn_mlp_trainer();
  t->impl = impl;
  *out = t;
  return WVN_OK;
}

void wvn_mlp_trainer_destroy(wvn_mlp_trainer_t* t) {
  if (!t) return;
  fused_trainer_destroy(t->impl);
  delete t;
}

int wvn_comm_unique_id(void* id128) { return fused_comm_unique_id(id128); }

int wvn_mlp_trainer_init_comm(wvn_mlp_trainer_t* t, const void* id128, int rank, int world) {
  WVN_REQUIRE(t, "wvn_mlp_trainer_init_comm: null trainer");
  return fused_trainer_init_comm(t->impl, id128, rank, world);
}

int wvn_mlp_trainer_set_confidence(wvn_mlp_trainer_t* t, int method, float* var, double* running_n, double* running_sum,
                                   double* running_sum_of_squares, float kf_proc_cov, float kf_meas_cov) {
  WVN_REQUIRE(t, "wvn_mlp_trainer_set_confidence: null trainer");
  return trainer_conf_bind(fused_trainer_conf(t->impl), method, var, running_n, running_sum, running_sum_of_squares,
                           kf_proc_cov, kf_meas_cov);
}

int wvn_mlp_trainer_copy_confidence(wvn_mlp_trainer_t* dst, const wvn_mlp_trainer_t* src, void* stream) {
  WVN_REQUIRE(dst && src, "wvn_mlp_trainer_copy_confidence: null trainer");
  return trainer_conf_copy(fused_trainer_conf(dst->impl), fused_trainer_conf(src->impl), S(stream));
}

int wvn_mlp_train_step(wvn_mlp_trainer_t* t, float* params, float* exp_avg, float* exp_avg_sq, long long* step_counter,
                       const float* x, int groups, int rows_per_group, const int* n_rows, const float* y,
                       const unsigned char* y_valid, float* cg_mean, float* cg_std, float* confidence_out,
                       float* metrics_out, int phase_mask, void* stream) {
  WVN_REQUIRE(t, "wvn_mlp_train_step: null trainer");
  return fused_train_step(t->impl, params, exp_avg, exp_avg_sq, step_counter, x, groups, rows_per_group, n_rows, y, y_valid,
                          cg_mean, cg_std, confidence_out, metrics_out, phase_mask, S(stream));
}

}

struct wvn_flow {
  FlowTrainer* impl = nullptr;
};

struct wvn_flow_infer {
  FlowTrainer* rows = nullptr;
  FlowPixels* pix = nullptr;
};

namespace {
FlowBuffers buffers_of(const wvn_flow_buffers* b) {
  FlowBuffers f;
  if (b) {
    f.mask0 = b->mask0; f.mask1 = b->mask1; f.p1 = b->p1; f.invp1 = b->invp1; f.p3 = b->p3; f.invp3 = b->invp3;
  }
  return f;
}
}

extern "C" {

size_t wvn_flow_param_count(int dim, int hidden) {
  FlowShape s;
  s.dim = dim; s.hidden = hidden;
  return flow_param_count(s);
}

int wvn_flow_create(int dim, int hidden, int max_rows, const wvn_train_config* cfg, float* grads, wvn_flow_t** out) {
  WVN_REQUIRE(cfg && out, "wvn_flow_create: null argument");
  WVN_PROPAGATE(wvn_check_device());
  FlowShape s;
  s.dim = dim; s.hidden = hidden;
  AdamCfg a;
  a.lr = cfg->lr; a.beta1 = cfg->beta1; a.beta2 = cfg->beta2; a.eps = cfg->eps;
  FlowTrainer* impl = nullptr;
  WVN_PROPAGATE(flow_trainer_create(s, max_rows, cfg->std_factor, a, grads, false, &impl));
  wvn_flow* h = new wvn_flow();
  h->impl = impl;
  *out = h;
  return WVN_OK;
}

void wvn_flow_destroy(wvn_flow_t* h) {
  if (!h) return;
  flow_trainer_destroy(h->impl);
  delete h;
}

int wvn_flow_set_confidence(wvn_flow_t* h, int method, float* var, double* running_n, double* running_sum,
                            double* running_sum_of_squares, float kf_proc_cov, float kf_meas_cov) {
  WVN_REQUIRE(h, "wvn_flow_set_confidence: null handle");
  return trainer_conf_bind(flow_trainer_conf(h->impl), method, var, running_n, running_sum, running_sum_of_squares,
                           kf_proc_cov, kf_meas_cov);
}

int wvn_flow_copy_confidence(wvn_flow_t* dst, const wvn_flow_t* src, void* stream) {
  WVN_REQUIRE(dst && src, "wvn_flow_copy_confidence: null handle");
  return trainer_conf_copy(flow_trainer_conf(dst->impl), flow_trainer_conf(src->impl), S(stream));
}

int wvn_flow_train_step(wvn_flow_t* h, float* params, float* exp_avg, float* exp_avg_sq, long long* step_counter,
                        const wvn_flow_buffers* buffers, const float* x, int rows, const unsigned char* y_valid,
                        float* cg_mean, float* cg_std, float* confidence_out, float* metrics_out, int phase_mask,
                        void* stream) {
  WVN_REQUIRE(h && buffers, "wvn_flow_train_step: null argument");
  return flow_train_step(h->impl, params, exp_avg, exp_avg_sq, step_counter, buffers_of(buffers), x, rows, y_valid,
                         cg_mean, cg_std, confidence_out, metrics_out, phase_mask, S(stream));
}

int wvn_flow_infer_create(int dim, int hidden, int max_rows, int chunk_pixels, wvn_flow_infer_t** out) {
  WVN_REQUIRE(out && max_rows > 0, "wvn_flow_infer_create: bad arguments");
  WVN_PROPAGATE(wvn_check_device());
  FlowShape s;
  s.dim = dim; s.hidden = hidden;
  wvn_flow_infer* h = new wvn_flow_infer();
  int rc = flow_trainer_create(s, max_rows, 0.5f, AdamCfg(), nullptr, true, &h->rows);
  if (rc == WVN_OK) rc = flow_pixels_create(s, chunk_pixels, &h->pix);
  if (rc != WVN_OK) {
    wvn_flow_infer_destroy(h);
    return rc;
  }
  *out = h;
  return WVN_OK;
}

void wvn_flow_infer_destroy(wvn_flow_infer_t* h) {
  if (!h) return;
  flow_trainer_destroy(h->rows);
  flow_pixels_destroy(h->pix);
  delete h;
}

int wvn_flow_infer_set_params(wvn_flow_infer_t* h, const float* params, void* stream) {
  WVN_REQUIRE(h, "wvn_flow_infer_set_params: null handle");
  return flow_pixels_set_params(h->pix, params, S(stream));
}

int wvn_flow_infer_rows(wvn_flow_infer_t* h, const float* params, const wvn_flow_buffers* buffers, const float* x, int rows,
                        float* z, float* log_det, float* logprob, const float* cg_mean, const float* cg_std,
                        float std_factor, float* trav, void* stream) {
  WVN_REQUIRE(h && buffers, "wvn_flow_infer_rows: null argument");
  return flow_forward_rows(h->rows, params, buffers_of(buffers), x, rows, z, log_det, logprob, cg_mean, cg_std,
                           std_factor, trav, S(stream));
}

int wvn_flow_infer_pixels(wvn_flow_infer_t* h, const wvn_flow_buffers* buffers, const float* tokens, int batch, int gh,
                          int gw, int out_h, int out_w, const float* cg_mean, const float* cg_std, float std_factor,
                          float* trav, float* nll, void* stream) {
  WVN_REQUIRE(h && buffers, "wvn_flow_infer_pixels: null argument");
  return flow_pixels_run(h->pix, buffers_of(buffers), tokens, batch, gh, gw, out_h, out_w, cg_mean, cg_std, std_factor,
                         trav, nll, S(stream));
}

}
```

wild_visual_navigation_b200/csrc/common.cuh:

```cuda
#pragma once

#include <cuda.h>
#include <cuda_bf16.h>
#include <cuda_runtime.h>
#include <stdint.h>
#include <stdio.h>

namespace wvn {

__device__ __forceinline__ uint32_t smem_u32(const void* p) {
  return static_cast<uint32_t>(__cvta_generic_to_shared(p));
}

__device__ __forceinline__ bool elect_one_sync() {
  uint32_t pred;
  asm volatile(
      "{\n\t"
      ".reg .pred p;\n\t"
      "elect.sync _|p, 0xffffffff;\n\t"
      "selp.u32 %0, 1, 0, p;\n\t"
      "}"
      : "=r"(pred));
  return pred != 0;
}

__device__ __forceinline__ uint32_t pack_bf16x2(float lo, float hi) {
  __nv_bfloat162 v = __floats2bfloat162_rn(lo, hi);
  return *reinterpret_cast<uint32_t*>(&v);
}

__device__ __forceinline__ float bf16_lo(uint32_t v) { return __uint_as_float(v << 16); }
__device__ __forceinline__ float bf16_hi(uint32_t v) { return __uint_as_float(v & 0xffff0000u); }

__device__ __forceinline__ void mbar_init(uint64_t* bar, uint32_t count) {
  asm volatile("mbarrier.init.shared::cta.b64 [%0], %1;" ::"r"(smem_u32(bar)), "r"(count) : "memory");
}

__device__ __forceinline__ void fence_mbar_init() {
  asm volatile("fence.mbarrier_init.release.cluster;" ::: "memory");
}

__device__ __forceinline__ void mbar_arrive_expect_tx(uint64_t* bar, uint32_t bytes) {
  asm volatile("mbarrier.arrive.expect_tx.shared::cta.b64 _, [%0], %1;" ::"r"(smem_u32(bar)), "r"(bytes)
               : "memory");
}

__device__ __forceinline__ void mbar_arrive(uint64_t* bar) {
  asm volatile("mbarrier.arrive.shared::cta.b64 _, [%0];" ::"r"(smem_u32(bar)) : "memory");
}

__device__ __forceinline__ bool mbar_try_wait(uint64_t* bar, uint32_t parity) {
  uint32_t ok;
  asm volatile(
      "{\n\t"
      ".reg .pred p;\n\t"
      "mbarrier.try_wait.parity.shared::cta.b64 p, [%1], %2;\n\t"
      "selp.u32 %0, 1, 0, p;\n\t"
      "}"
      : "=r"(ok)
      : "r"(smem_u32(bar)), "r"(parity)
      : "memory");
  return ok != 0;
}

__device__ __forceinline__ bool mbar_test_wait(uint64_t* bar, uint32_t parity) {
  uint32_t ok;
  asm volatile(
      "{\n\t"
      ".reg .pred p;\n\t"
      "mbarrier.test_wait.parity.shared::cta.b64 p, [%1], %2;\n\t"
      "selp.u32 %0, 1, 0, p;\n\t"
      "}"
      : "=r"(ok)
      : "r"(smem_u32(bar)), "r"(parity)
      : "memory");
  return ok != 0;
}

#ifndef WVN_MBAR_TIMEOUT_CYCLES
#define WVN_MBAR_TIMEOUT_CYCLES 4000000000ll
#endif

#ifndef WVN_MBAR_HINT_NS
#define WVN_MBAR_HINT_NS 0
#endif
#define WVN_STR2(x) #x
#define WVN_STR(x) WVN_STR2(x)
#if WVN_MBAR_HINT_NS > 0
#define WVN_TRY_WAIT_PTX "mbarrier.try_wait.parity.shared::cta.b64 p, [%1], %2, " WVN_STR(WVN_MBAR_HINT_NS) ";\n\t"
#else
#define WVN_TRY_WAIT_PTX "mbarrier.try_wait.parity.shared::cta.b64 p, [%1], %2;\n\t"
#endif

__device__ __forceinline__ bool mbar_try_wait_many(uint32_t bar_addr, uint32_t parity) {
  uint32_t ok;
  asm volatile(
      "{\n\t"
      ".reg .pred p;\n\t"
      ".reg .u32 n;\n\t"
      "mov.u32 n, 65536;\n\t"
      "WVN_WAIT_LOOP:\n\t"
      WVN_TRY_WAIT_PTX
      "@p bra WVN_WAIT_DONE;\n\t"
      "sub.u32 n, n, 1;\n\t"
      "setp.ne.u32 p, n, 0;\n\t"
      "@p bra WVN_WAIT_LOOP;\n\t"
      "WVN_WAIT_DONE:\n\t"
      "selp.u32 %0, 1, 0, p;\n\t"
      "}"
      : "=r"(ok)
      : "r"(bar_addr), "r"(parity)
      : "memory");
  return ok != 0;
}

__device__ __forceinline__ void mbar_wait(uint64_t* bar, uint32_t parity) {
  if (mbar_try_wait(bar, parity)) return;
  const uint32_t addr = smem_u32(bar);
  const long long t0 = clock64();
  while (!mbar_try_wait_many(addr, parity)) {
    if (clock64() - t0 > WVN_MBAR_TIMEOUT_CYCLES) {
#ifdef WVN_MBAR_DIAG
      printf("[wvn] mbarrier timeout: block (%d,%d) thread %d bar@%u parity %u\n", blockIdx.x, blockIdx.y,
             threadIdx.x, addr, parity);
#endif
      __trap();
    }
  }
}

__device__ __forceinline__ void fence_proxy_async_smem() {
  asm volatile("fence.proxy.async.shared::cta;" ::: "memory");
}

__device__ __forceinline__ void tma_load_2d(const CUtensorMap* map, uint64_t* bar, void* smem_dst, int32_t c0,
                                            int32_t c1) {
  asm volatile(
      "cp.async.bulk.tensor.2d.shared::cluster.global.mbarrier::complete_tx::bytes [%0], [%1, {%3, %4}], [%2];" ::"r"(
          smem_u32(smem_dst)),
      "l"(reinterpret_cast<uint64_t>(map)), "r"(smem_u32(bar)), "r"(c0), "r"(c1)
      : "memory");
}

__device__ __forceinline__ void tma_load_2d_mcast(const CUtensorMap* map, uint64_t* bar, void* smem_dst, int32_t c0,
                                                  int32_t c1, uint16_t cta_mask) {
  asm volatile(
      "cp.async.bulk.tensor.2d.shared::cluster.global.mbarrier::complete_tx::bytes.multicast::cluster"
      " [%0], [%1, {%4, %5}], [%2], %3;" ::"r"(smem_u32(smem_dst)),
      "l"(reinterpret_cast<uint64_t>(map)), "r"(smem_u32(bar)), "h"(cta_mask), "r"(c0), "r"(c1)
      : "memory");
}

__device__ __forceinline__ void tma_store_2d(const CUtensorMap* map, uint32_t smem_src, int32_t c0, int32_t c1) {
  asm volatile("cp.async.bulk.tensor.2d.global.shared::cta.bulk_group [%0, {%2, %3}], [%1];" ::"l"(
                   reinterpret_cast<uint64_t>(map)),
               "r"(smem_src), "r"(c0), "r"(c1)
               : "memory");
}
__device__ __forceinline__ void tma_reduce_add_2d(const CUtensorMap* map, uint32_t smem_src, int32_t c0, int32_t c1) {
  asm volatile("cp.reduce.async.bulk.tensor.2d.global.shared::cta.add.bulk_group [%0, {%2, %3}], [%1];" ::"l"(
                   reinterpret_cast<uint64_t>(map)),
               "r"(smem_src), "r"(c0), "r"(c1)
               : "memory");
}
__device__ __forceinline__ void tma_store_commit() { asm volatile("cp.async.bulk.commit_group;" ::: "memory"); }
template <int N>
__device__ __forceinline__ void tma_store_wait_read() {
  asm volatile("cp.async.bulk.wait_group.read %0;" ::"n"(N) : "memory");
}
template <int N>
__device__ __forceinline__ void tma_store_wait_all() {
  asm volatile("cp.async.bulk.wait_group %0;" ::"n"(N) : "memory");
}

__device__ __forceinline__ uint32_t cluster_ctarank() {
  uint32_t r;
  asm volatile("mov.u32 %0, %%cluster_ctarank;" : "=r"(r));
  return r;
}

__device__ __forceinline__ void cluster_sync_all() {
  asm volatile("barrier.cluster.arrive.release.aligned;" ::: "memory");
  asm volatile("barrier.cluster.wait.acquire.aligned;" ::: "memory");
}

__device__ __forceinline__ void tma_prefetch_desc(const CUtensorMap* map) {
  asm volatile("prefetch.tensormap [%0];" ::"l"(reinterpret_cast<uint64_t>(map)) : "memory");
}

__device__ __forceinline__ uint64_t make_sw128_kmajor_desc(uint32_t smem_addr) {
  uint64_t d = 0;
  d |= static_cast<uint64_t>((smem_addr & 0x3ffff) >> 4);
  d |= static_cast<uint64_t>(1) << 16;
  d |= static_cast<uint64_t>(1024 >> 4) << 32;
  d |= static_cast<uint64_t>(1) << 62;
  return d;
}

__device__ __forceinline__ void wgmma_fence() { asm volatile("wgmma.fence.sync.aligned;" ::: "memory"); }
__device__ __forceinline__ void wgmma_commit() { asm volatile("wgmma.commit_group.sync.aligned;" ::: "memory"); }
template <int N>
__device__ __forceinline__ void wgmma_wait() {
  asm volatile("wgmma.wait_group.sync.aligned %0;" ::"n"(N) : "memory");
}

template <int N>
__device__ __forceinline__ void wgmma_fence_regs(float (&d)[N]) {
#pragma unroll
  for (int i = 0; i < N; ++i) asm volatile("" : "+f"(d[i])::"memory");
}
template <int N>
__device__ __forceinline__ void wgmma_fence_regs(uint32_t (&a)[N]) {
#pragma unroll
  for (int i = 0; i < N; ++i) asm volatile("" : "+r"(a[i])::"memory");
}

template <int N>
__device__ __forceinline__ void setmaxnreg_inc() { asm volatile("setmaxnreg.inc.sync.aligned.u32 %0;" ::"n"(N)); }
template <int N>
__device__ __forceinline__ void setmaxnreg_dec() { asm volatile("setmaxnreg.dec.sync.aligned.u32 %0;" ::"n"(N)); }

__device__ __forceinline__ void wgmma_m64n32k16_ss(float (&d)[16], uint64_t desc_a, uint64_t desc_b, uint32_t accumulate) {
  asm volatile(
      "{\n\t"
      ".reg .pred p;\n\t"
      "setp.ne.b32 p, %18, 0;\n\t"
      "wgmma.mma_async.sync.aligned.m64n32k16.f32.bf16.bf16 "
      "{%0, %1, %2, %3, %4, %5, %6, %7, %8, %9, %10, %11, %12, %13, %14, %15}, "
      "%16, %17, p, 1, 1, 0, 0;\n\t"
      "}"
      : "+f"(d[0]), "+f"(d[1]), "+f"(d[2]), "+f"(d[3]), "+f"(d[4]), "+f"(d[5]), "+f"(d[6]), "+f"(d[7]),
        "+f"(d[8]), "+f"(d[9]), "+f"(d[10]), "+f"(d[11]), "+f"(d[12]), "+f"(d[13]), "+f"(d[14]), "+f"(d[15])
      : "l"(desc_a), "l"(desc_b), "r"(accumulate));
}

__device__ __forceinline__ void wgmma_m64n64k16_ss(float (&d)[32], uint64_t desc_a, uint64_t desc_b, uint32_t accumulate) {
  asm volatile(
      "{\n\t"
      ".reg .pred p;\n\t"
      "setp.ne.b32 p, %34, 0;\n\t"
      "wgmma.mma_async.sync.aligned.m64n64k16.f32.bf16.bf16 "
      "{%0, %1, %2, %3, %4, %5, %6, %7, %8, %9, %10, %11, %12, %13, %14, %15, %16, %17, %18, %19, %20, "
      "%21, %22, %23, %24, %25, %26, %27, %28, %29, %30, %31}, "
      "%32, %33, p, 1, 1, 0, 0;\n\t"
      "}"
      : "+f"(d[0]), "+f"(d[1]), "+f"(d[2]), "+f"(d[3]), "+f"(d[4]), "+f"(d[5]), "+f"(d[6]), "+f"(d[7]),
        "+f"(d[8]), "+f"(d[9]), "+f"(d[10]), "+f"(d[11]), "+f"(d[12]), "+f"(d[13]), "+f"(d[14]), "+f"(d[15]),
        "+f"(d[16]), "+f"(d[17]), "+f"(d[18]), "+f"(d[19]), "+f"(d[20]), "+f"(d[21]), "+f"(d[22]), "+f"(d[23]),
        "+f"(d[24]), "+f"(d[25]), "+f"(d[26]), "+f"(d[27]), "+f"(d[28]), "+f"(d[29]), "+f"(d[30]), "+f"(d[31])
      : "l"(desc_a), "l"(desc_b), "r"(accumulate));
}

__device__ __forceinline__ void wgmma_m64n128k16_ss(float (&d)[64], uint64_t desc_a, uint64_t desc_b, uint32_t accumulate) {
  asm volatile(
      "{\n\t"
      ".reg .pred p;\n\t"
      "setp.ne.b32 p, %66, 0;\n\t"
      "wgmma.mma_async.sync.aligned.m64n128k16.f32.bf16.bf16 "
      "{%0, %1, %2, %3, %4, %5, %6, %7, %8, %9, %10, %11, %12, %13, %14, %15, %16, %17, %18, %19, %20, "
      "%21, %22, %23, %24, %25, %26, %27, %28, %29, %30, %31, %32, %33, %34, %35, %36, %37, %38, %39, "
      "%40, %41, %42, %43, %44, %45, %46, %47, %48, %49, %50, %51, %52, %53, %54, %55, %56, %57, %58, "
      "%59, %60, %61, %62, %63}, "
      "%64, %65, p, 1, 1, 0, 0;\n\t"
      "}"
      : "+f"(d[0]), "+f"(d[1]), "+f"(d[2]), "+f"(d[3]), "+f"(d[4]), "+f"(d[5]), "+f"(d[6]), "+f"(d[7]),
        "+f"(d[8]), "+f"(d[9]), "+f"(d[10]), "+f"(d[11]), "+f"(d[12]), "+f"(d[13]), "+f"(d[14]), "+f"(d[15]),
        "+f"(d[16]), "+f"(d[17]), "+f"(d[18]), "+f"(d[19]), "+f"(d[20]), "+f"(d[21]), "+f"(d[22]), "+f"(d[23]),
        "+f"(d[24]), "+f"(d[25]), "+f"(d[26]), "+f"(d[27]), "+f"(d[28]), "+f"(d[29]), "+f"(d[30]), "+f"(d[31]),
        "+f"(d[32]), "+f"(d[33]), "+f"(d[34]), "+f"(d[35]), "+f"(d[36]), "+f"(d[37]), "+f"(d[38]), "+f"(d[39]),
        "+f"(d[40]), "+f"(d[41]), "+f"(d[42]), "+f"(d[43]), "+f"(d[44]), "+f"(d[45]), "+f"(d[46]), "+f"(d[47]),
        "+f"(d[48]), "+f"(d[49]), "+f"(d[50]), "+f"(d[51]), "+f"(d[52]), "+f"(d[53]), "+f"(d[54]), "+f"(d[55]),
        "+f"(d[56]), "+f"(d[57]), "+f"(d[58]), "+f"(d[59]), "+f"(d[60]), "+f"(d[61]), "+f"(d[62]), "+f"(d[63])
      : "l"(desc_a), "l"(desc_b), "r"(accumulate));
}

__device__ __forceinline__ void wgmma_m64n64k16_rs(float (&d)[32], uint32_t a0, uint32_t a1, uint32_t a2, uint32_t a3,
                                                   uint64_t desc_b, uint32_t accumulate) {
  asm volatile(
      "{\n\t"
      ".reg .pred p;\n\t"
      "setp.ne.b32 p, %37, 0;\n\t"
      "wgmma.mma_async.sync.aligned.m64n64k16.f32.bf16.bf16 "
      "{%0, %1, %2, %3, %4, %5, %6, %7, %8, %9, %10, %11, %12, %13, %14, %15, %16, %17, %18, %19, %20, "
      "%21, %22, %23, %24, %25, %26, %27, %28, %29, %30, %31}, "
      "{%32, %33, %34, %35}, %36, p, 1, 1, 0;\n\t"
      "}"
      : "+f"(d[0]), "+f"(d[1]), "+f"(d[2]), "+f"(d[3]), "+f"(d[4]), "+f"(d[5]), "+f"(d[6]), "+f"(d[7]),
        "+f"(d[8]), "+f"(d[9]), "+f"(d[10]), "+f"(d[11]), "+f"(d[12]), "+f"(d[13]), "+f"(d[14]), "+f"(d[15]),
        "+f"(d[16]), "+f"(d[17]), "+f"(d[18]), "+f"(d[19]), "+f"(d[20]), "+f"(d[21]), "+f"(d[22]), "+f"(d[23]),
        "+f"(d[24]), "+f"(d[25]), "+f"(d[26]), "+f"(d[27]), "+f"(d[28]), "+f"(d[29]), "+f"(d[30]), "+f"(d[31])
      : "r"(a0), "r"(a1), "r"(a2), "r"(a3), "l"(desc_b), "r"(accumulate));
}

__device__ __forceinline__ void named_bar_sync(int id, int nthreads) {
  asm volatile("bar.sync %0, %1;" ::"r"(id), "r"(nthreads) : "memory");
}
__device__ __forceinline__ void named_bar_arrive(int id, int nthreads) {
  asm volatile("bar.arrive %0, %1;" ::"r"(id), "r"(nthreads) : "memory");
}

__device__ __forceinline__ void sts128(uint32_t addr, uint32_t a, uint32_t b, uint32_t c, uint32_t d) {
  asm volatile("st.shared.v4.b32 [%0], {%1, %2, %3, %4};" ::"r"(addr), "r"(a), "r"(b), "r"(c), "r"(d) : "memory");
}
__device__ __forceinline__ void sts64(uint32_t addr, float a, float b) {
  asm volatile("st.shared.v2.f32 [%0], {%1, %2};" ::"r"(addr), "f"(a), "f"(b) : "memory");
}
__device__ __forceinline__ void sts32(uint32_t addr, uint32_t a) {
  asm volatile("st.shared.b32 [%0], %1;" ::"r"(addr), "r"(a) : "memory");
}
__device__ __forceinline__ void sts16(uint32_t addr, __nv_bfloat16 a) {
  asm volatile("st.shared.b16 [%0], %1;" ::"r"(addr), "h"(__bfloat16_as_ushort(a)) : "memory");
}
__device__ __forceinline__ uint4 lds128(uint32_t addr) {
  uint4 v;
  asm volatile("ld.shared.v4.b32 {%0, %1, %2, %3}, [%4];" : "=r"(v.x), "=r"(v.y), "=r"(v.z), "=r"(v.w) : "r"(addr) : "memory");
  return v;
}

__device__ __forceinline__ void st_global_v4(void* p, uint32_t a, uint32_t b, uint32_t c, uint32_t d) {
  asm volatile("st.global.v4.b32 [%0], {%1, %2, %3, %4};" ::"l"(p), "r"(a), "r"(b), "r"(c), "r"(d) : "memory");
}

__device__ __forceinline__ float warp_sum(float v) {
#pragma unroll
  for (int o = 16; o > 0; o >>= 1) v += __shfl_xor_sync(0xffffffffu, v, o);
  return v;
}

__device__ __forceinline__ float warp_max(float v) {
#pragma unroll
  for (int o = 16; o > 0; o >>= 1) v = fmaxf(v, __shfl_xor_sync(0xffffffffu, v, o));
  return v;
}

}
```

wild_visual_navigation_b200/csrc/gemm.h:

```cpp
#pragma once

#include <cuda_runtime.h>

namespace wvn {

enum GemmEpilogue : int {
  EPI_BF16 = 0,
  EPI_F32 = 1,
  EPI_RESID_F32 = 2,
  EPI_PATCH = 3,
  EPI_QKV = 4,
  EPI_MLP_HEAD = 5,
  EPI_BF16_RESID = 6,
};

enum GemmAct : int { ACT_NONE = 0, ACT_RELU = 1, ACT_GELU = 2 };

struct GemmArgs {
  int M = 0, N = 0, K = 0;
  int epi = EPI_BF16, act = ACT_NONE;
  const float* bias = nullptr;
  void* out = nullptr;
  long long ldo = 0;
  const float* pos = nullptr;
  int tokens_in = 0;
  int registers = 0;
  int npad = 0;
  int dim = 0, heads = 0;
  void* q = nullptr;
  void* k = nullptr;
  void* vt = nullptr;
  int feat = 0;
  int trav_col = 0;
  const void* x = nullptr;
  long long ldx = 0;
  float* trav = nullptr;
  float* conf = nullptr;
  float* loss_reco = nullptr;
  const float* cg_mean = nullptr;
  const float* cg_std = nullptr;
  float cg_std_factor = 0.5f;
  const void* residual = nullptr;
  long long ldr = 0;
  int max_ctas = 0;
  int reverse_m = 0;
};

int pick_block_n(int N);

inline long long gemm_w_pitch(int K) { return (static_cast<long long>(K) + 7) / 8 * 8; }

int gemm_bf16(const GemmArgs& args, const void* A, long long lda, const void* W, int block_n, cudaStream_t stream);

}
```

wild_visual_navigation_b200/csrc/gemm_wgmma.cu:

```cuda
#include <stdlib.h>

#include <algorithm>

#include "common.cuh"
#include "gemm.h"
#include "host_common.h"

namespace wvn {

namespace {

constexpr int BM = 64;
constexpr int BK = 64;
constexpr int kConsumerWarps = 8;
constexpr int kNumThreads = 128 + kConsumerWarps * 32;
constexpr int kMaxSmemBytes = 227 * 1024;
constexpr int kMaxStages = 8;
constexpr int kFixedSmemBytes = 1024  + 1024 ;
constexpr int kSliceCols = 32;
constexpr int kResidMaxBlockN = 192;

template <bool ROW_OWNER>
struct TileIter {
  int num_m, num_n, m_blk, n_blk, lin;
  __device__ TileIter(int nm, int nn) : num_m(nm), num_n(nn), m_blk(0), n_blk(0), lin(0) {
    if (ROW_OWNER) { m_blk = blockIdx.x; n_blk = 0; }
    else { lin = blockIdx.x; m_blk = lin / num_n; n_blk = lin % num_n; }
  }
  __device__ bool valid() const { return m_blk < num_m; }
  __device__ void next() {
    if (ROW_OWNER) { if (++n_blk == num_n) { n_blk = 0; m_blk += gridDim.x; } }
    else { lin += gridDim.x; m_blk = lin / num_n; n_blk = lin % num_n; }
  }
};

template <int EPI>
constexpr bool kStaged = EPI == EPI_BF16 || EPI == EPI_F32 || EPI == EPI_RESID_F32 || EPI == EPI_QKV || EPI == EPI_BF16_RESID;

template <int BN, int EPI>
struct GemmCfg {
  static constexpr uint32_t kABytes = BM * BK * 2;
  static constexpr uint32_t kBBytes = BN * BK * 2;
  static constexpr uint32_t kStageBytes = kABytes + kBBytes;
  static constexpr uint32_t kSliceBytes = BM * kSliceCols * ((EPI == EPI_F32 || EPI == EPI_RESID_F32) ? 4 : 2);
  static constexpr uint32_t kStagingBytes = kStaged<EPI> ? 2 * 2 * kSliceBytes : 0;
  static constexpr int kStagesRaw = (kMaxSmemBytes - kFixedSmemBytes - kStagingBytes) / kStageBytes;
  static constexpr int kStages = kStagesRaw > kMaxStages ? kMaxStages : kStagesRaw;
  static constexpr uint32_t kSmemBytes = kStages * kStageBytes + kStagingBytes + kFixedSmemBytes;
  static constexpr int kN128 = BN / 128;
  static constexpr int kN64 = (BN % 128) / 64;
  static constexpr int kN32 = (BN % 64) / 32;
};

__device__ __forceinline__ float gelu_erf_fast(float x) {
  const float t = fminf(fabsf(x), 5.5f);
  float p = fmaf(-0.0003865310864f, t, 0.006509808358f);
  p = fmaf(p, t, -0.05048002675f);
  p = fmaf(p, t, -0.4613505006f);
  p = fmaf(p, t, -1.150225043f);
  p = fmaf(p, t, -1.00010848f);
  float e;
  asm("ex2.approx.ftz.f32 %0, %1;" : "=f"(e) : "f"(p));
  return fmaf(-t, e, fmaxf(x, 0.f));
}

template <int ACT>
__device__ __forceinline__ float activate(float v) {
  if (ACT == ACT_RELU) return fmaxf(v, 0.f);
  if (ACT == ACT_GELU) return gelu_erf_fast(v);
  return v;
}

template <int EPI, int ACT, int NREG>
__device__ __forceinline__ void epilogue_frag(const GemmArgs& args, const float (&d)[NREG], const int row0,
                                              const int col_base, const int lane, float (&head_partial)[2]) {
  const int q = lane & 3;
  bool ok[2];
  long long orow[2];
  int tok[2];
#pragma unroll
  for (int h = 0; h < 2; ++h) {
    const int row = row0 + 8 * h;
    ok[h] = row < args.M;
    orow[h] = row;
    tok[h] = 0;
    if (EPI == EPI_PATCH) {
      const int frame = row / args.tokens_in;
      tok[h] = row - frame * args.tokens_in;
      orow[h] = static_cast<long long>(frame) * args.npad + (1 + args.registers) + tok[h];
    }
  }
#pragma unroll
  for (int j = 0; j < NREG / 4; ++j) {
    const int col = col_base + 8 * j + 2 * q;
    float2 b = make_float2(0.f, 0.f);
    if (args.bias != nullptr) b = __ldg(reinterpret_cast<const float2*>(args.bias + col));
#pragma unroll
    for (int h = 0; h < 2; ++h) {
      const float v0 = activate<ACT>(d[4 * j + 2 * h] + b.x), v1 = activate<ACT>(d[4 * j + 2 * h + 1] + b.y);
      if (!ok[h]) continue;
      if (EPI == EPI_PATCH) {
        const float2 pe = __ldg(reinterpret_cast<const float2*>(args.pos + static_cast<long long>(1 + tok[h]) * args.ldo + col));
        *reinterpret_cast<float2*>(reinterpret_cast<float*>(args.out) + orow[h] * args.ldo + col) = make_float2(v0 + pe.x, v1 + pe.y);
      } else if (EPI == EPI_MLP_HEAD) {
        if (col < args.feat) {
          const uint32_t xv = __ldg(reinterpret_cast<const uint32_t*>(
              reinterpret_cast<const __nv_bfloat16*>(args.x) + orow[h] * args.ldx + col));
          const float d0 = v0 - bf16_lo(xv), d1 = v1 - bf16_hi(xv);
          head_partial[h] = fmaf(d0, d0, head_partial[h]);
          if (col + 1 < args.feat) head_partial[h] = fmaf(d1, d1, head_partial[h]);
        } else if (col == args.trav_col) {
          args.trav[orow[h]] = 1.f / (1.f + __expf(-v0));
        }
      }
    }
  }
}

template <int EPI, int ACT, int NREG>
__device__ __forceinline__ void store_frag(const GemmArgs& args, const CUtensorMap* tm0, const CUtensorMap* tm1,
                                           const CUtensorMap* tm2, const float (&d)[NREG], const int row_tile,
                                           const int col_base, const int row_local, const int lane, const bool leader,
                                           const int bar_id, const uint32_t staging, const uint32_t slice_bytes,
                                           const int slice0) {
  const int q = lane & 3;
#pragma unroll
  for (int s = 0; s < NREG / 16; ++s) {
    const int col = col_base + kSliceCols * s;
    const int si = slice0 + s;
    const uint32_t buf = staging + (si & 1) * slice_bytes;
    int which = 0, within = 0;
    if (EPI == EPI_QKV) {
      which = col / args.dim;
      within = col - which * args.dim;
    }
    if (leader) {
      if (si == 0) tma_store_wait_read<0>();
      else tma_store_wait_read<1>();
    }
    named_bar_sync(bar_id, 128);
#pragma unroll
    for (int js = 0; js < 4; ++js) {
      const int j = 4 * s + js;
      const int c = col + 8 * js + 2 * q;
      float2 b = make_float2(0.f, 0.f);
      if (args.bias != nullptr) b = __ldg(reinterpret_cast<const float2*>(args.bias + c));
#pragma unroll
      for (int h = 0; h < 2; ++h) {
        const int r = row_local + 8 * h;
        float a0 = d[4 * j + 2 * h] + b.x, a1 = d[4 * j + 2 * h + 1] + b.y;
        if (EPI == EPI_BF16_RESID && row_tile + r < args.M) {
          const uint32_t rv = __ldg(reinterpret_cast<const uint32_t*>(
              reinterpret_cast<const __nv_bfloat16*>(args.residual) + static_cast<long long>(row_tile + r) * args.ldr + c));
          a0 += bf16_lo(rv);
          a1 += bf16_hi(rv);
        }
        const float v0 = activate<ACT>(a0), v1 = activate<ACT>(a1);
        if (EPI == EPI_F32 || EPI == EPI_RESID_F32) {
          sts64(buf + r * 128 + ((((2 * js + (q >> 1)) ^ (r & 7))) << 4) + (q & 1) * 8, v0, v1);
        } else if (EPI == EPI_QKV && which == 2) {
          const int dd = 8 * js + 2 * q;
          const uint32_t t = 2 * r;
          sts16(buf + dd * 128 + (((t >> 4) ^ (dd & 7)) << 4) + (t & 15), __float2bfloat16_rn(v0));
          sts16(buf + (dd + 1) * 128 + (((t >> 4) ^ ((dd + 1) & 7)) << 4) + (t & 15), __float2bfloat16_rn(v1));
        } else {
          sts32(buf + r * 64 + ((js ^ ((r >> 1) & 3)) << 4) + q * 4, pack_bf16x2(v0, v1));
        }
      }
    }
    fence_proxy_async_smem();
    named_bar_sync(bar_id, 128);
    if (leader) {
      if (EPI == EPI_BF16 || EPI == EPI_F32 || EPI == EPI_BF16_RESID) {
        tma_store_2d(tm0, buf, col, row_tile);
      } else if (EPI == EPI_RESID_F32) {
        tma_reduce_add_2d(tm0, buf, col, row_tile);
      } else if (EPI == EPI_QKV) {
        const int frame = row_tile / args.npad;
        const int tok0 = row_tile - frame * args.npad;
        const int bh = frame * args.heads + (within >> 6);
        if (which < 2) tma_store_2d(which == 0 ? tm0 : tm1, buf, within & 63, bh * args.npad + tok0);
        else tma_store_2d(tm2, buf, tok0, bh * 64 + (within & 63));
      }
      tma_store_commit();
    }
  }
}

template <int BN, int EPI, int ACT>
__global__ void __launch_bounds__(kNumThreads, 1)
gemm_bf16_kernel(const __grid_constant__ CUtensorMap tmap_a, const __grid_constant__ CUtensorMap tmap_b,
                 const __grid_constant__ CUtensorMap tmap_c0, const __grid_constant__ CUtensorMap tmap_c1,
                 const __grid_constant__ CUtensorMap tmap_c2, const GemmArgs args) {
  using Cfg = GemmCfg<BN, EPI>;
  constexpr int STAGES = Cfg::kStages;

  extern __shared__ uint8_t smem_raw[];
  uint8_t* smem = reinterpret_cast<uint8_t*>((reinterpret_cast<uintptr_t>(smem_raw) + 1023) & ~uintptr_t(1023));
  uint8_t* smem_b = smem;
  uint8_t* smem_a = smem + STAGES * Cfg::kBBytes;
  uint8_t* smem_c = smem_a + STAGES * Cfg::kABytes;
  uint64_t* bars = reinterpret_cast<uint64_t*>(smem_c + Cfg::kStagingBytes);
  uint64_t* full_bar = bars;
  uint64_t* empty_bar = bars + kMaxStages;

  const int warp = threadIdx.x >> 5;
  const int lane = threadIdx.x & 31;

  const int num_m = (args.M + BM - 1) / BM;
  const int num_n = args.N / BN;
  const int num_k = (args.K + BK - 1) / BK;
  constexpr bool ROW_OWNER = (EPI == EPI_MLP_HEAD);

  if (threadIdx.x == 0) {
    tma_prefetch_desc(&tmap_a);
    tma_prefetch_desc(&tmap_b);
    for (int i = 0; i < kMaxStages; ++i) {
      mbar_init(&full_bar[i], 1);
      mbar_init(&empty_bar[i], kConsumerWarps / 2);
    }
    fence_mbar_init();
  }
  __syncthreads();

  if (warp < 4) {
    setmaxnreg_dec<40>();
    if (warp == 0) {
      int stage = 0;
      uint32_t phase = 0;
      for (TileIter<ROW_OWNER> it(num_m, num_n); it.valid(); it.next()) {
        const int m_eff = args.reverse_m ? num_m - 1 - it.m_blk : it.m_blk;
        for (int kb = 0; kb < num_k; ++kb) {
          mbar_wait(&empty_bar[stage], phase ^ 1);
          if (elect_one_sync()) {
            mbar_arrive_expect_tx(&full_bar[stage], Cfg::kStageBytes);
            tma_load_2d(&tmap_a, &full_bar[stage], smem_a + stage * Cfg::kABytes, kb * BK, m_eff * BM);
            tma_load_2d(&tmap_b, &full_bar[stage], smem_b + stage * Cfg::kBBytes, kb * BK, it.n_blk * BN);
          }
          __syncwarp();
          if (++stage == STAGES) { stage = 0; phase ^= 1; }
        }
      }
    }
  } else {
    setmaxnreg_inc<232>();
    const int cwarp = warp - 4;
    const int wg = cwarp >> 2;
    const int row_local = (cwarp & 3) * 16 + (lane >> 2);
    const bool leader = (threadIdx.x & 127) == 0;
    const uint32_t staging = smem_u32(smem_c) + wg * 2 * Cfg::kSliceBytes;
    if (kStaged<EPI> && leader) {
      tma_prefetch_desc(&tmap_c0);
      if (EPI == EPI_QKV) {
        tma_prefetch_desc(&tmap_c1);
        tma_prefetch_desc(&tmap_c2);
      }
    }
    if (wg == 1) named_bar_arrive(1, 256);
    float acc128[Cfg::kN128 > 0 ? Cfg::kN128 : 1][64];
    float acc64[32];
    float acc32[16];
    float head_partial[2] = {0.f, 0.f};
    int stage = 0;
    uint32_t phase = 0;
    int unit = 0;
    for (TileIter<ROW_OWNER> it(num_m, num_n); it.valid(); it.next()) {
      const bool unit_end = !ROW_OWNER || it.n_blk == num_n - 1;
      if ((unit & 1) != wg) {
        for (int kb = 0; kb < num_k; ++kb)
          if (++stage == STAGES) { stage = 0; phase ^= 1; }
        if (unit_end) ++unit;
        continue;
      }
      if (!ROW_OWNER || it.n_blk == 0) named_bar_sync(1 + wg, 256);
      int prev_stage = 0;
      for (int kb = 0; kb < num_k; ++kb) {
        mbar_wait(&full_bar[stage], phase);
        const uint64_t desc_a = make_sw128_kmajor_desc(smem_u32(smem_a + stage * Cfg::kABytes));
        const uint32_t b_addr = smem_u32(smem_b + stage * Cfg::kBBytes);
#pragma unroll
        for (int c = 0; c < Cfg::kN128; ++c) wgmma_fence_regs(acc128[c]);
        if (Cfg::kN64) wgmma_fence_regs(acc64);
        if (Cfg::kN32) wgmma_fence_regs(acc32);
        wgmma_fence();
#pragma unroll
        for (int k = 0; k < BK / 16; ++k) {
          const uint32_t accumulate = (kb | k) != 0 ? 1u : 0u;
#pragma unroll
          for (int c = 0; c < Cfg::kN128; ++c)
            wgmma_m64n128k16_ss(acc128[c], desc_a + 2 * k, make_sw128_kmajor_desc(b_addr + c * 128 * 128) + 2 * k, accumulate);
          if (Cfg::kN64)
            wgmma_m64n64k16_ss(acc64, desc_a + 2 * k, make_sw128_kmajor_desc(b_addr + Cfg::kN128 * 128 * 128) + 2 * k, accumulate);
          if (Cfg::kN32)
            wgmma_m64n32k16_ss(acc32, desc_a + 2 * k,
                               make_sw128_kmajor_desc(b_addr + (Cfg::kN128 * 128 + Cfg::kN64 * 64) * 128) + 2 * k, accumulate);
        }
        wgmma_commit();
        if (kb > 0) {
          wgmma_wait<1>();
          if (lane == 0) mbar_arrive(&empty_bar[prev_stage]);
        }
        prev_stage = stage;
        if (++stage == STAGES) { stage = 0; phase ^= 1; }
      }
      if (unit_end && (ROW_OWNER ? it.m_blk + static_cast<int>(gridDim.x) < num_m : it.lin + static_cast<int>(gridDim.x) < num_m * num_n))
        named_bar_arrive(2 - wg, 256);
      wgmma_wait<0>();
#pragma unroll
      for (int c = 0; c < Cfg::kN128; ++c) wgmma_fence_regs(acc128[c]);
      if (Cfg::kN64) wgmma_fence_regs(acc64);
      if (Cfg::kN32) wgmma_fence_regs(acc32);
      if (lane == 0) mbar_arrive(&empty_bar[prev_stage]);

      const int m_eff = args.reverse_m ? num_m - 1 - it.m_blk : it.m_blk;
      const int row_tile = m_eff * BM;
      const int col0 = it.n_blk * BN;
      if (kStaged<EPI>) {
        const int bar_id = 3 + wg;
#pragma unroll
        for (int c = 0; c < Cfg::kN128; ++c)
          store_frag<EPI, ACT>(args, &tmap_c0, &tmap_c1, &tmap_c2, acc128[c], row_tile, col0 + c * 128, row_local, lane,
                               leader, bar_id, staging, Cfg::kSliceBytes, 4 * c);
        if (Cfg::kN64)
          store_frag<EPI, ACT>(args, &tmap_c0, &tmap_c1, &tmap_c2, acc64, row_tile, col0 + Cfg::kN128 * 128, row_local,
                               lane, leader, bar_id, staging, Cfg::kSliceBytes, 4 * Cfg::kN128);
        if (Cfg::kN32)
          store_frag<EPI, ACT>(args, &tmap_c0, &tmap_c1, &tmap_c2, acc32, row_tile, col0 + Cfg::kN128 * 128 + Cfg::kN64 * 64,
                               row_local, lane, leader, bar_id, staging, Cfg::kSliceBytes, 4 * Cfg::kN128 + 2 * Cfg::kN64);
      } else {
        const int row0 = row_tile + row_local;
#pragma unroll
        for (int c = 0; c < Cfg::kN128; ++c)
          epilogue_frag<EPI, ACT>(args, acc128[c], row0, col0 + c * 128, lane, head_partial);
        if (Cfg::kN64) epilogue_frag<EPI, ACT>(args, acc64, row0, col0 + Cfg::kN128 * 128, lane, head_partial);
        if (Cfg::kN32) epilogue_frag<EPI, ACT>(args, acc32, row0, col0 + Cfg::kN128 * 128 + Cfg::kN64 * 64, lane, head_partial);
      }

      if (EPI == EPI_MLP_HEAD && it.n_blk == num_n - 1) {
#pragma unroll
        for (int h = 0; h < 2; ++h) {
          float s = head_partial[h];
          s += __shfl_xor_sync(0xffffffffu, s, 1);
          s += __shfl_xor_sync(0xffffffffu, s, 2);
          head_partial[h] = 0.f;
          const int row = row_tile + row_local + 8 * h;
          if ((lane & 3) == 0 && row < args.M) {
            const float loss = s / static_cast<float>(args.feat);
            const float mean = __ldg(args.cg_mean), sd = __ldg(args.cg_std);
            const float shifted = mean + sd * args.cg_std_factor;
            const float lo = fmaxf(shifted - sd, 0.f);
            const float hi = shifted + sd;
            const float xc = fminf(fmaxf(loss, lo), hi);
            args.conf[row] = 1.f - (xc - lo) / (hi - lo);
            if (args.loss_reco != nullptr) args.loss_reco[row] = loss;
          }
        }
      }
      if (unit_end) ++unit;
    }
    if (kStaged<EPI> && leader) tma_store_wait_all<0>();
  }
}

template <int BN, int EPI, int ACT>
int launch_gemm(const GemmArgs& a, const CUtensorMap& ta, const CUtensorMap& tb, const CUtensorMap (&tc)[3],
                cudaStream_t stream) {
  using Cfg = GemmCfg<BN, EPI>;
  static_assert(Cfg::kStages >= 2, "tile too wide for the shared-memory budget");
  auto kern = gemm_bf16_kernel<BN, EPI, ACT>;
  static bool attr_set = false;
  if (!attr_set) {
    WVN_CHECK_CUDA(cudaFuncSetAttribute(kern, cudaFuncAttributeMaxDynamicSharedMemorySize, kMaxSmemBytes));
    attr_set = true;
  }
  const int num_m = (a.M + BM - 1) / BM, num_n = a.N / BN;
  const int num_tiles = (EPI == EPI_MLP_HEAD) ? num_m : num_m * num_n;
  int grid = sm_count();
  if (a.max_ctas > 0 && a.max_ctas < grid) grid = a.max_ctas;
  if (grid > num_tiles) grid = num_tiles;
  prof_begin(PROF_GEMM, stream);
  kern<<<grid, kNumThreads, Cfg::kSmemBytes, stream>>>(ta, tb, tc[0], tc[1], tc[2], a);
  prof_end(PROF_GEMM, stream);
  WVN_CHECK_LAUNCH("gemm_bf16_kernel");
  return WVN_OK;
}

template <int BN>
int dispatch_epi(const GemmArgs& a, const CUtensorMap& ta, const CUtensorMap& tb, const CUtensorMap (&tc)[3],
                 cudaStream_t s) {
  switch (a.epi) {
    case EPI_BF16:
      if (a.act == ACT_NONE) return launch_gemm<BN, EPI_BF16, ACT_NONE>(a, ta, tb, tc, s);
      if (a.act == ACT_RELU) return launch_gemm<BN, EPI_BF16, ACT_RELU>(a, ta, tb, tc, s);
      if (a.act == ACT_GELU) return launch_gemm<BN, EPI_BF16, ACT_GELU>(a, ta, tb, tc, s);
      break;
    case EPI_F32:
      if (a.act == ACT_NONE) return launch_gemm<BN, EPI_F32, ACT_NONE>(a, ta, tb, tc, s);
      break;
    case EPI_RESID_F32:
      if (a.act == ACT_NONE) return launch_gemm<BN, EPI_RESID_F32, ACT_NONE>(a, ta, tb, tc, s);
      break;
    case EPI_PATCH:
      if (a.act == ACT_NONE) return launch_gemm<BN, EPI_PATCH, ACT_NONE>(a, ta, tb, tc, s);
      break;
    case EPI_QKV:
      if (a.act == ACT_NONE) return launch_gemm<BN, EPI_QKV, ACT_NONE>(a, ta, tb, tc, s);
      break;
    case EPI_MLP_HEAD:
      if (a.act == ACT_NONE) return launch_gemm<BN, EPI_MLP_HEAD, ACT_NONE>(a, ta, tb, tc, s);
      break;
    case EPI_BF16_RESID:
      if constexpr (BN <= kResidMaxBlockN) {
        if (a.act == ACT_NONE) return launch_gemm<BN, EPI_BF16_RESID, ACT_NONE>(a, ta, tb, tc, s);
        if (a.act == ACT_RELU) return launch_gemm<BN, EPI_BF16_RESID, ACT_RELU>(a, ta, tb, tc, s);
      }
      break;
  }
  return set_error(WVN_ERR_INVALID, "gemm: unsupported epilogue/activation combination (%d, %d)", a.epi, a.act);
}

}

int pick_block_n(int N) {
  if (N % 256 == 0) return 256;
  if (N % 224 == 0) return 224;
  if (N % 192 == 0) return 192;
  if (N % 128 == 0) return 128;
  if (N % 64 == 0) return 64;
  return 0;
}

int gemm_bf16(const GemmArgs& a, const void* A, long long lda, const void* W, int block_n, cudaStream_t stream) {
  WVN_REQUIRE(a.M > 0 && a.N > 0 && a.K > 0, "gemm: empty problem (M=%d N=%d K=%d)", a.M, a.N, a.K);
  WVN_REQUIRE(lda >= a.K, "gemm: lda=%lld is smaller than K=%d", lda, a.K);
  if (block_n == 0) {
    block_n = pick_block_n(a.N);
    if (a.epi == EPI_BF16_RESID && block_n > kResidMaxBlockN) block_n = a.N % 192 == 0 ? 192 : (a.N % 128 == 0 ? 128 : 64);
  }
  WVN_REQUIRE(a.epi != EPI_BF16_RESID || block_n <= kResidMaxBlockN, "gemm: the residual epilogue takes block_n <= %d",
              kResidMaxBlockN);
  WVN_REQUIRE(block_n == 64 || block_n == 128 || block_n == 192 || block_n == 224 || block_n == 256,
              "gemm: bad block_n %d", block_n);
  WVN_REQUIRE(a.N % block_n == 0, "gemm: N=%d must be a multiple of block_n=%d (pad the weights)", a.N, block_n);
  if (a.epi == EPI_MLP_HEAD)
    WVN_REQUIRE(a.feat > 0 && a.trav_col % 32 == 0 && a.trav_col >= a.feat && a.trav_col < a.N && a.x != nullptr &&
                    a.trav != nullptr && a.conf != nullptr && a.cg_mean != nullptr && a.cg_std != nullptr &&
                    a.ldx % 8 == 0 && a.ldx >= a.trav_col,
                "gemm: bad MLP-head epilogue arguments (feat=%d trav_col=%d N=%d)", a.feat, a.trav_col, a.N);
  if (a.epi == EPI_QKV)
    WVN_REQUIRE(a.dim % 64 == 0 && a.N == 3 * a.dim && a.heads * 64 == a.dim && a.npad % 8 == 0 && a.npad % BM == 0 &&
                    a.M % a.npad == 0,
                "gemm: bad QKV epilogue geometry (dim=%d heads=%d npad=%d N=%d M=%d)", a.dim, a.heads, a.npad, a.N, a.M);
  if (a.epi == EPI_PATCH)
    WVN_REQUIRE(a.tokens_in > 0 && a.registers >= 0 && 1 + a.registers + a.tokens_in <= a.npad,
                "gemm: bad patch-embed epilogue geometry (tokens_in=%d registers=%d npad=%d)", a.tokens_in, a.registers,
                a.npad);
  if (a.epi == EPI_F32 || a.epi == EPI_RESID_F32) WVN_REQUIRE(a.ldo % 4 == 0, "gemm: fp32 output pitch must be a multiple of 4");
  if (a.epi == EPI_BF16 || a.epi == EPI_BF16_RESID) WVN_REQUIRE(a.ldo % 8 == 0, "gemm: bf16 output pitch must be a multiple of 8");
  if (a.epi == EPI_BF16_RESID)
    WVN_REQUIRE(a.residual != nullptr && a.ldr >= a.N && a.ldr % 2 == 0,
                "gemm: the residual epilogue needs a bf16 residual with an even pitch ldr >= N (ldr=%lld N=%d)", a.ldr, a.N);
  CUtensorMap ta, tb, tc[3] = {};
  WVN_PROPAGATE(make_tmap_bf16_2d(&ta, A, a.K, a.M, static_cast<uint64_t>(lda) * 2, BK, BM));
  WVN_PROPAGATE(make_tmap_bf16_2d(&tb, W, a.K, a.N, static_cast<uint64_t>(gemm_w_pitch(a.K)) * 2, BK, block_n));
  if (a.epi == EPI_BF16 || a.epi == EPI_BF16_RESID)
    WVN_PROPAGATE(make_tmap_2d(&tc[0], a.out, 2, a.N, a.M, static_cast<uint64_t>(a.ldo) * 2, kSliceCols, BM, 64));
  if (a.epi == EPI_F32 || a.epi == EPI_RESID_F32)
    WVN_PROPAGATE(make_tmap_2d(&tc[0], a.out, 4, a.N, a.M, static_cast<uint64_t>(a.ldo) * 4, kSliceCols, BM, 128));
  if (a.epi == EPI_QKV) {
    const uint64_t bh = static_cast<uint64_t>(a.M / a.npad) * a.heads;
    WVN_PROPAGATE(make_tmap_2d(&tc[0], a.q, 2, 64, bh * a.npad, 128, kSliceCols, BM, 64));
    WVN_PROPAGATE(make_tmap_2d(&tc[1], a.k, 2, 64, bh * a.npad, 128, kSliceCols, BM, 64));
    WVN_PROPAGATE(make_tmap_2d(&tc[2], a.vt, 2, a.npad, bh * 64, static_cast<uint64_t>(a.npad) * 2, BM, kSliceCols, 128));
  }
  switch (block_n) {
    case 64: return dispatch_epi<64>(a, ta, tb, tc, stream);
    case 128: return dispatch_epi<128>(a, ta, tb, tc, stream);
    case 192: return dispatch_epi<192>(a, ta, tb, tc, stream);
    case 224: return dispatch_epi<224>(a, ta, tb, tc, stream);
    case 256: return dispatch_epi<256>(a, ta, tb, tc, stream);
  }
  return set_error(WVN_ERR_INVALID, "gemm: unreachable");
}

}
```

wild_visual_navigation_b200/csrc/vit_kernels.cu:

```cuda
#include "common.cuh"
#include "host_common.h"
#include "vit_kernels.h"

namespace wvn {

namespace {

template <bool U8_HWC, int G>
__global__ void image_to_patches_kernel(const void* __restrict__ img_raw, __nv_bfloat16* __restrict__ out,
                                        ImagePatchArgs a) {
  const float* img = reinterpret_cast<const float*>(img_raw);
  const unsigned char* img8 = reinterpret_cast<const unsigned char*>(img_raw);
  const int ps = a.patch;
  const int k_total = 3 * ps * ps;
  const int pitch = patch_pitch(ps);
  const int groups_per_row = k_total / G;
  const long long total = static_cast<long long>(a.batch) * a.grid_h * a.grid_w * groups_per_row;
  for (long long idx = blockIdx.x * static_cast<long long>(blockDim.x) + threadIdx.x; idx < total;
       idx += static_cast<long long>(gridDim.x) * blockDim.x) {
    const int g = static_cast<int>(idx % groups_per_row);
    const long long prow = idx / groups_per_row;
    const int pw = static_cast<int>(prow % a.grid_w);
    const int ph = static_cast<int>((prow / a.grid_w) % a.grid_h);
    const int b = static_cast<int>(prow / (static_cast<long long>(a.grid_w) * a.grid_h));
    const int k0 = g * G;
    const int c = k0 / (ps * ps);
    const int ky = (k0 / ps) % ps;
    const int kx0 = k0 % ps;
    const int y = ph * ps + ky;
    const int sy = min(static_cast<int>(floorf((y + a.crop_top) * a.scale_y)), a.in_h - 1);
    const float mean = a.mean[c], inv_std = a.inv_std[c];
    const int gb = a.frame0 + b;
    const bool flip = gb >= a.flip_from;
    const int sb = gb % a.src_frames;
    const int crop_w = a.grid_w * ps;
    const float* src_row = img + ((static_cast<long long>(sb) * 3 + c) * a.in_h + sy) * a.in_w;
    const unsigned char* src_row8 = img8 + (static_cast<long long>(sb) * a.in_h + sy) * a.in_w * 3 + c;
    float v[G];
#pragma unroll
    for (int i = 0; i < G; ++i) {
      const int xo = pw * ps + kx0 + i;
      const int x = flip ? crop_w - 1 - xo : xo;
      const int sx = min(static_cast<int>(floorf((x + a.crop_left) * a.scale_x)), a.in_w - 1);
      const float px = U8_HWC ? static_cast<float>(__ldg(src_row8 + 3 * sx)) / 255.f : __ldg(src_row + sx);
      v[i] = (px - mean) * inv_std;
    }
    __nv_bfloat16* dst = out + prow * pitch + k0;
    if (G == 8) {
      st_global_v4(dst, pack_bf16x2(v[0], v[1]), pack_bf16x2(v[2], v[3]), pack_bf16x2(v[4], v[5]),
                   pack_bf16x2(v[6], v[7]));
    } else {
#pragma unroll
      for (int i = 0; i < G; i += 2) *reinterpret_cast<uint32_t*>(dst + i) = pack_bf16x2(v[i], v[i + 1]);
    }
  }
}

__global__ void init_token_rows_kernel(float* __restrict__ x, const float* __restrict__ cls,
                                       const float* __restrict__ pos, const float* __restrict__ reg, int registers,
                                       int batch, int npad, int n_valid, int dim) {
  const int head_rows = 1 + registers;
  const int rows_per_frame = head_rows + (npad - n_valid);
  const long long total = static_cast<long long>(batch) * rows_per_frame * dim;
  for (long long idx = blockIdx.x * static_cast<long long>(blockDim.x) + threadIdx.x; idx < total;
       idx += static_cast<long long>(gridDim.x) * blockDim.x) {
    const int d = static_cast<int>(idx % dim);
    const long long r = idx / dim;
    const int rr = static_cast<int>(r % rows_per_frame);
    const int b = static_cast<int>(r / rows_per_frame);
    const int row = (rr < head_rows) ? rr : (n_valid + rr - head_rows);
    const float v = (rr == 0) ? (cls[d] + pos[d]) : (rr < head_rows ? reg[static_cast<long long>(rr - 1) * dim + d] : 0.f);
    x[(static_cast<long long>(b) * npad + row) * dim + d] = v;
  }
}

template <int ITERS>
__global__ void __launch_bounds__(256)
layernorm_rows_kernel(const float* __restrict__ x, const float* __restrict__ gamma, const float* __restrict__ beta,
                      __nv_bfloat16* __restrict__ out_bf16, float* __restrict__ out_f32, LayerNormArgs a) {
  constexpr int D = 128 * ITERS;
  const int warp_global = (blockIdx.x * blockDim.x + threadIdx.x) >> 5;
  const int lane = threadIdx.x & 31;
  const int warps_total = (gridDim.x * blockDim.x) >> 5;
  for (long long r = warp_global; r < a.rows; r += warps_total) {
    const long long row = a.reverse ? a.rows - 1 - r : r;
    const float4* src = reinterpret_cast<const float4*>(x + row * D);
    float4 v[ITERS];
    float s = 0.f;
#pragma unroll
    for (int i = 0; i < ITERS; ++i) {
      v[i] = src[lane + 32 * i];
      s += (v[i].x + v[i].y) + (v[i].z + v[i].w);
    }
    const float mean = warp_sum(s) * (1.f / D);
    float q = 0.f;
#pragma unroll
    for (int i = 0; i < ITERS; ++i) {
      const float dx = v[i].x - mean, dy = v[i].y - mean, dz = v[i].z - mean, dw = v[i].w - mean;
      q += (dx * dx + dy * dy) + (dz * dz + dw * dw);
    }
    const float rstd = rsqrtf(warp_sum(q) * (1.f / D) + a.eps);
    long long f32_row = -1;
    if (out_f32 != nullptr) {
      const int tok = static_cast<int>(row % a.npad);
      const long long frame = row / a.npad;
      if (tok >= a.row0 && tok < a.n_valid) f32_row = frame * (a.n_valid - a.row0) + (tok - a.row0);
    }
#pragma unroll
    for (int i = 0; i < ITERS; ++i) {
      const int c4 = lane + 32 * i;
      const float4 g = __ldg(reinterpret_cast<const float4*>(gamma) + c4);
      const float4 bt = __ldg(reinterpret_cast<const float4*>(beta) + c4);
      float4 y;
      y.x = (v[i].x - mean) * rstd * g.x + bt.x;
      y.y = (v[i].y - mean) * rstd * g.y + bt.y;
      y.z = (v[i].z - mean) * rstd * g.z + bt.z;
      y.w = (v[i].w - mean) * rstd * g.w + bt.w;
      if (out_bf16 != nullptr) {
        uint2 p = make_uint2(pack_bf16x2(y.x, y.y), pack_bf16x2(y.z, y.w));
        *reinterpret_cast<uint2*>(out_bf16 + row * D + 4 * c4) = p;
      }
      if (f32_row >= 0) reinterpret_cast<float4*>(out_f32 + f32_row * D)[c4] = y;
    }
  }
}


__global__ void __launch_bounds__(128)
attention_f32_debug_kernel(const float* __restrict__ qkv, __nv_bfloat16* __restrict__ out, int npad, int n_valid, int heads,
                           int dim, float scale) {
  __shared__ float ks[64][65];
  __shared__ float vs[64][65];
  const int h = blockIdx.y, b = blockIdx.z;
  const int qi = blockIdx.x * 128 + threadIdx.x;
  const long long row0 = static_cast<long long>(b) * npad;
  const int ld = 3 * dim;
  float q[64], o[64];
  const bool active = qi < npad;
#pragma unroll
  for (int d = 0; d < 64; ++d) {
    q[d] = active ? qkv[(row0 + qi) * ld + h * 64 + d] * scale : 0.f;
    o[d] = 0.f;
  }
  float m = -INFINITY, l = 0.f;
  for (int k0 = 0; k0 < n_valid; k0 += 64) {
    __syncthreads();
    for (int i = threadIdx.x; i < 64 * 64; i += 128) {
      const int kk = i >> 6, d = i & 63;
      const bool ok = k0 + kk < n_valid;
      ks[kk][d] = ok ? qkv[(row0 + k0 + kk) * ld + dim + h * 64 + d] : 0.f;
      vs[kk][d] = ok ? qkv[(row0 + k0 + kk) * ld + 2 * dim + h * 64 + d] : 0.f;
    }
    __syncthreads();
    for (int c0 = 0; c0 < 64; c0 += 16) {
      float sc[16], cmax = -INFINITY;
#pragma unroll
      for (int j = 0; j < 16; ++j) {
        float acc = 0.f;
#pragma unroll
        for (int d = 0; d < 64; ++d) acc = fmaf(q[d], ks[c0 + j][d], acc);
        sc[j] = (k0 + c0 + j < n_valid) ? acc : -INFINITY;
        cmax = fmaxf(cmax, sc[j]);
      }
      if (cmax == -INFINITY) continue;
      const float m_new = fmaxf(m, cmax);
      const float alpha = expf(m - m_new);
      l *= alpha;
#pragma unroll
      for (int d = 0; d < 64; ++d) o[d] *= alpha;
#pragma unroll
      for (int j = 0; j < 16; ++j) {
        const float p = expf(sc[j] - m_new);
        l += p;
#pragma unroll
        for (int d = 0; d < 64; ++d) o[d] = fmaf(p, vs[c0 + j][d], o[d]);
      }
      m = m_new;
    }
  }
  if (active) {
    const float inv = 1.f / l;
    __nv_bfloat16* dst = out + (row0 + qi) * dim + h * 64;
#pragma unroll
    for (int d = 0; d < 64; ++d) dst[d] = __float2bfloat16_rn(o[d] * inv);
  }
}

}

int image_to_patches(const void* img, bool u8_hwc, void* out_bf16, const ImagePatchArgs& a, cudaStream_t stream) {
  WVN_REQUIRE(a.patch == 8 || a.patch == 14 || a.patch == 16, "image_to_patches: patch size %d unsupported", a.patch);
  const int group = a.patch == 14 ? 14 : 8;
  const long long total = static_cast<long long>(a.batch) * a.grid_h * a.grid_w * (3 * a.patch * a.patch / group);
  const int threads = 256;
  long long blocks = (total + threads - 1) / threads;
  const long long max_blocks = static_cast<long long>(sm_count()) * 16;
  if (blocks > max_blocks) blocks = max_blocks;
  __nv_bfloat16* out = reinterpret_cast<__nv_bfloat16*>(out_bf16);
  const unsigned nb = static_cast<unsigned>(blocks);
  if (group == 14) {
    if (u8_hwc) image_to_patches_kernel<true, 14><<<nb, threads, 0, stream>>>(img, out, a);
    else image_to_patches_kernel<false, 14><<<nb, threads, 0, stream>>>(img, out, a);
  } else {
    if (u8_hwc) image_to_patches_kernel<true, 8><<<nb, threads, 0, stream>>>(img, out, a);
    else image_to_patches_kernel<false, 8><<<nb, threads, 0, stream>>>(img, out, a);
  }
  WVN_CHECK_LAUNCH("image_to_patches_kernel");
  return WVN_OK;
}

int init_token_rows(float* x, const float* cls, const float* pos, const float* reg, int registers, int batch, int npad,
                    int n_valid, int dim, cudaStream_t stream) {
  WVN_REQUIRE(registers >= 0 && (registers == 0 || reg != nullptr), "init_token_rows: %d registers without their weights",
              registers);
  const long long total = static_cast<long long>(batch) * (1 + registers + npad - n_valid) * dim;
  const int threads = 256;
  long long blocks = (total + threads - 1) / threads;
  if (blocks > 4096) blocks = 4096;
  init_token_rows_kernel<<<static_cast<unsigned>(blocks), threads, 0, stream>>>(x, cls, pos, reg, registers, batch, npad,
                                                                                n_valid, dim);
  WVN_CHECK_LAUNCH("init_token_rows_kernel");
  return WVN_OK;
}

int layernorm_rows(const float* x, const float* gamma, const float* beta, void* out_bf16, float* out_f32,
                   const LayerNormArgs& a, cudaStream_t stream) {
  WVN_REQUIRE(a.dim == 384 || a.dim == 768, "layernorm: dim %d unsupported (384 or 768)", a.dim);
  const int threads = 256;
  long long blocks = (a.rows * 32 + threads - 1) / threads;
  const long long max_blocks = static_cast<long long>(sm_count()) * 8;
  if (blocks > max_blocks) blocks = max_blocks;
  if (a.dim == 384)
    layernorm_rows_kernel<3><<<static_cast<unsigned>(blocks), threads, 0, stream>>>(
        x, gamma, beta, reinterpret_cast<__nv_bfloat16*>(out_bf16), out_f32, a);
  else
    layernorm_rows_kernel<6><<<static_cast<unsigned>(blocks), threads, 0, stream>>>(
        x, gamma, beta, reinterpret_cast<__nv_bfloat16*>(out_bf16), out_f32, a);
  WVN_CHECK_LAUNCH("layernorm_rows_kernel");
  return WVN_OK;
}

int attention_f32_debug(const float* qkv, void* out_bf16, int batch, int heads, int npad, int n_valid, int dim, float scale,
                        cudaStream_t stream) {
  WVN_REQUIRE(dim == heads * 64, "attention_f32_debug: head dim must be 64");
  dim3 grid((npad + 127) / 128, heads, batch);
  attention_f32_debug_kernel<<<grid, 128, 0, stream>>>(qkv, reinterpret_cast<__nv_bfloat16*>(out_bf16), npad, n_valid, heads,
                                                      dim, scale);
  WVN_CHECK_LAUNCH("attention_f32_debug_kernel");
  return WVN_OK;
}

}
```

Baseline: 971.4.

## Fuse LayerNorm into the QKV and FC1 GEMM A-operand producer for D=384

For ViT width 384, the separate layernorm_rows kernel before the QKV and MLP fc1 GEMMs is removed. Producer warps inside the wgmma GEMM now read the fp32 residual stream, normalize each row, and write the bf16 A tile into swizzled shared memory. That A block stays resident across all N tiles of the row, so each CTA owns whole rows, and the next block is prefetched into L2. This drops the bf16 xn round trip through global memory and one launch per norm. The cost is fewer pipeline stages from the extra shared memory, row-owner scheduling that may hurt load balance, and a new block_n=192 choice for fc1.

```diff
diff --git a/include/wvn_b200.h b/include/wvn_b200.h
--- a/include/wvn_b200.h
+++ b/include/wvn_b200.h
@@ -55,6 +55,10 @@
   int registers;
   const void* residual;
   long long ldr;
+  const float* ln_x;
+  const float* ln_gamma;
+  const float* ln_beta;
+  float ln_eps;
 } wvn_gemm_ex_args;
 int wvn_gemm_bf16_ex(const wvn_gemm_ex_args* args, void* stream);
 
diff --git a/wild_visual_navigation_b200/_C.py b/wild_visual_navigation_b200/_C.py
--- a/wild_visual_navigation_b200/_C.py
+++ b/wild_visual_navigation_b200/_C.py
@@ -31,6 +31,7 @@
         ("feat", c_int), ("trav_col", c_int), ("x", c_void_p), ("ldx", c_longlong), ("trav", c_void_p),
         ("conf", c_void_p), ("loss_reco", c_void_p), ("cg_mean", c_void_p), ("cg_std", c_void_p),
         ("cg_std_factor", c_float), ("reverse_m", c_int), ("registers", c_int), ("residual", c_void_p), ("ldr", c_longlong),
+        ("ln_x", c_void_p), ("ln_gamma", c_void_p), ("ln_beta", c_void_p), ("ln_eps", c_float),
     ]
 
 
diff --git a/wild_visual_navigation_b200/csrc/api.cu b/wild_visual_navigation_b200/csrc/api.cu
--- a/wild_visual_navigation_b200/csrc/api.cu
+++ b/wild_visual_navigation_b200/csrc/api.cu
@@ -110,7 +110,7 @@
 extern "C" {
 
 const char* wvn_last_error(void) { return last_error(); }
-int wvn_version(void) { return 104; }
+int wvn_version(void) { return 105; }
 
 int wvn_check_device(void) {
   int n = 0;
@@ -154,6 +154,7 @@
   g.loss_reco = x->loss_reco; g.cg_mean = x->cg_mean; g.cg_std = x->cg_std; g.cg_std_factor = x->cg_std_factor;
   g.reverse_m = x->reverse_m; g.registers = x->registers;
   g.residual = x->residual; g.ldr = x->ldr;
+  g.ln_x = x->ln_x; g.ln_gamma = x->ln_gamma; g.ln_beta = x->ln_beta; g.ln_eps = x->ln_eps;
   return gemm_bf16(g, x->a, x->lda, x->w, x->block_n, S(stream));
 }
 
@@ -233,7 +234,7 @@
   const size_t bh = static_cast<size_t>(h->chunk) * cfg->heads;
   auto alloc = [&](DevBuf& b, size_t bytes) { if (rc == WVN_OK) rc = b.alloc(bytes); };
   alloc(h->x, rows * D * 4);
-  alloc(h->xn, rows * D * 2);
+  if (!gemm_ln_a_supported(D)) alloc(h->xn, rows * D * 2);
   alloc(h->q, bh * h->npad * 64 * 2);
   alloc(h->k, bh * h->npad * 64 * 2);
   alloc(h->vt, bh * 64 * h->npad * 2);
@@ -400,6 +401,21 @@
     auto next_dir = [&]() { dir = snake ? dir ^ 1 : 0; return dir; };
     __nv_bfloat16* xn = reinterpret_cast<__nv_bfloat16*>(h->xn.p);
     __nv_bfloat16* attn = reinterpret_cast<__nv_bfloat16*>(h->attn.p);
+    const bool fused_ln = gemm_ln_a_supported(D);
+    auto layernorm_a = [&](GemmArgs& g, const std::string& norm, long long roff, long long nrows) -> int {
+      if (fused_ln) {
+        g.ln_x = x + roff * D;
+        g.ln_gamma = h->wp<float>(norm + ".weight");
+        g.ln_beta = h->wp<float>(norm + ".bias");
+        g.ln_eps = c.ln_eps;
+        return WVN_OK;
+      }
+      LayerNormArgs ls = la;
+      ls.rows = nrows;
+      ls.reverse = next_dir();
+      return layernorm_rows(x + roff * D, h->wp<float>(norm + ".weight"), h->wp<float>(norm + ".bias"), xn + roff * D,
+                            nullptr, ls, s);
+    };
     static int sub_attn_env = -1;
     if (sub_attn_env < 0) {
       const char* e = getenv("WVN_VIT_SUB_ATTN");
@@ -412,29 +428,25 @@
       for (int s0 = 0; s0 < nb; s0 += sub_a) {
         const int ns = std::min(sub_a, nb - s0);
         const long long roff = static_cast<long long>(s0) * h->npad;
-        LayerNormArgs ls = la;
-        ls.rows = static_cast<long long>(ns) * h->npad;
-        ls.reverse = next_dir();
-        WVN_PROPAGATE(layernorm_rows(x + roff * D, h->wp<float>(b + "norm1.weight"), h->wp<float>(b + "norm1.bias"),
-                                     xn + roff * D, nullptr, ls, s));
+        GemmArgs g;
+        g.M = ns * h->npad; g.N = 3 * D; g.K = D; g.bias = h->wp<float>(b + "attn.qkv.bias");
+        WVN_PROPAGATE(layernorm_a(g, b + "norm1", roff, static_cast<long long>(ns) * h->npad));
+        const void* a_in = fused_ln ? nullptr : xn + roff * D;
         if (h->precise) {
-          GemmArgs g;
           float* qkv = reinterpret_cast<float*>(h->qkv_f32.p) + roff * 3 * D;
-          g.M = ns * h->npad; g.N = 3 * D; g.K = D; g.epi = EPI_F32; g.bias = h->wp<float>(b + "attn.qkv.bias");
-          g.out = qkv; g.ldo = 3 * D;
-          WVN_PROPAGATE(gemm_bf16(g, xn + roff * D, D, h->wp<void>(b + "attn.qkv.weight"), 0, s));
+          g.epi = EPI_F32; g.out = qkv; g.ldo = 3 * D;
+          WVN_PROPAGATE(gemm_bf16(g, a_in, D, h->wp<void>(b + "attn.qkv.weight"), 0, s));
           WVN_PROPAGATE(attention_f32_debug(qkv, attn + roff * D, ns, c.heads, h->npad, h->n_valid, D, 0.125f, s));
           continue;
         }
-        GemmArgs g;
-        g.M = ns * h->npad; g.N = 3 * D; g.K = D; g.epi = EPI_QKV; g.bias = h->wp<float>(b + "attn.qkv.bias");
+        g.epi = EPI_QKV;
         g.npad = h->npad; g.dim = D; g.heads = c.heads;
         const long long hoff = static_cast<long long>(s0) * c.heads * h->npad * 64;
         g.q = reinterpret_cast<__nv_bfloat16*>(h->q.p) + hoff;
         g.k = reinterpret_cast<__nv_bfloat16*>(h->k.p) + hoff;
         g.vt = reinterpret_cast<__nv_bfloat16*>(h->vt.p) + hoff;
         g.reverse_m = next_dir();
-        WVN_PROPAGATE(gemm_bf16(g, xn + roff * D, D, h->wp<void>(b + "attn.qkv.weight"), 0, s));
+        WVN_PROPAGATE(gemm_bf16(g, a_in, D, h->wp<void>(b + "attn.qkv.weight"), 0, s));
         AttnArgs a;
         a.batch = ns; a.heads = c.heads; a.npad = h->npad; a.n_valid = h->n_valid;
         a.scale_log2 = 0.125f * 1.4426950408889634f;
@@ -446,8 +458,6 @@
         const int ns = std::min(sub, nb - s0);
         const long long roff = static_cast<long long>(s0) * h->npad;
         const int srows = ns * h->npad;
-        LayerNormArgs ls = la;
-        ls.rows = srows;
         {
           GemmArgs g;
           g.M = srows; g.N = D; g.K = D; g.epi = EPI_RESID_F32; g.bias = h->wp<float>(b + "attn.proj.bias");
@@ -455,15 +465,14 @@
           g.reverse_m = next_dir();
           WVN_PROPAGATE(gemm_bf16(g, attn + roff * D, D, h->wp<void>(b + "attn.proj.weight"), 0, s));
         }
-        ls.reverse = next_dir();
-        WVN_PROPAGATE(layernorm_rows(x + roff * D, h->wp<float>(b + "norm2.weight"), h->wp<float>(b + "norm2.bias"),
-                                     xn + roff * D, nullptr, ls, s));
         {
           GemmArgs g;
           g.M = srows; g.N = c.mlp_dim; g.K = D; g.epi = EPI_BF16; g.act = ACT_GELU;
           g.bias = h->wp<float>(b + "mlp.fc1.bias"); g.out = h->hid.p; g.ldo = c.mlp_dim;
+          WVN_PROPAGATE(layernorm_a(g, b + "norm2", roff, srows));
           g.reverse_m = next_dir();
-          WVN_PROPAGATE(gemm_bf16(g, xn + roff * D, D, h->wp<void>(b + "mlp.fc1.weight"), 0, s));
+          WVN_PROPAGATE(gemm_bf16(g, fused_ln ? nullptr : xn + roff * D, D, h->wp<void>(b + "mlp.fc1.weight"),
+                                  fused_ln && c.mlp_dim % 192 == 0 ? 192 : 0, s));
         }
         {
           GemmArgs g;
diff --git a/wild_visual_navigation_b200/csrc/common.cuh b/wild_visual_navigation_b200/csrc/common.cuh
--- a/wild_visual_navigation_b200/csrc/common.cuh
+++ b/wild_visual_navigation_b200/csrc/common.cuh
@@ -47,6 +47,10 @@
 
 __device__ __forceinline__ void mbar_arrive(uint64_t* bar) {
   asm volatile("mbarrier.arrive.shared::cta.b64 _, [%0];" ::"r"(smem_u32(bar)) : "memory");
+}
+
+__device__ __forceinline__ void mbar_arrive_cnt(uint64_t* bar, uint32_t count) {
+  asm volatile("mbarrier.arrive.shared::cta.b64 _, [%0], %1;" ::"r"(smem_u32(bar)), "r"(count) : "memory");
 }
 
 __device__ __forceinline__ bool mbar_try_wait(uint64_t* bar, uint32_t parity) {
@@ -184,6 +188,10 @@
   asm volatile("barrier.cluster.wait.acquire.aligned;" ::: "memory");
 }
 
+__device__ __forceinline__ void l2_prefetch_bulk(const void* p, uint32_t bytes) {
+  asm volatile("cp.async.bulk.prefetch.L2.global [%0], %1;" ::"l"(reinterpret_cast<uint64_t>(p)), "r"(bytes) : "memory");
+}
+
 __device__ __forceinline__ void tma_prefetch_desc(const CUtensorMap* map) {
   asm volatile("prefetch.tensormap [%0];" ::"l"(reinterpret_cast<uint64_t>(map)) : "memory");
 }
@@ -305,6 +313,9 @@
 __device__ __forceinline__ void sts64(uint32_t addr, float a, float b) {
   asm volatile("st.shared.v2.f32 [%0], {%1, %2};" ::"r"(addr), "f"(a), "f"(b) : "memory");
 }
+__device__ __forceinline__ void sts64u(uint32_t addr, uint32_t a, uint32_t b) {
+  asm volatile("st.shared.v2.b32 [%0], {%1, %2};" ::"r"(addr), "r"(a), "r"(b) : "memory");
+}
 __device__ __forceinline__ void sts32(uint32_t addr, uint32_t a) {
   asm volatile("st.shared.b32 [%0], %1;" ::"r"(addr), "r"(a) : "memory");
 }
@@ -317,6 +328,12 @@
   return v;
 }
 
+__device__ __forceinline__ float4 lds128f(uint32_t addr) {
+  float4 v;
+  asm volatile("ld.shared.v4.f32 {%0, %1, %2, %3}, [%4];" : "=f"(v.x), "=f"(v.y), "=f"(v.z), "=f"(v.w) : "r"(addr) : "memory");
+  return v;
+}
+
 __device__ __forceinline__ void st_global_v4(void* p, uint32_t a, uint32_t b, uint32_t c, uint32_t d) {
   asm volatile("st.global.v4.b32 [%0], {%1, %2, %3, %4};" ::"l"(p), "r"(a), "r"(b), "r"(c), "r"(d) : "memory");
 }
diff --git a/wild_visual_navigation_b200/csrc/gemm.h b/wild_visual_navigation_b200/csrc/gemm.h
--- a/wild_visual_navigation_b200/csrc/gemm.h
+++ b/wild_visual_navigation_b200/csrc/gemm.h
@@ -42,6 +42,10 @@
   float cg_std_factor = 0.5f;
   const void* residual = nullptr;
   long long ldr = 0;
+  const float* ln_x = nullptr;
+  const float* ln_gamma = nullptr;
+  const float* ln_beta = nullptr;
+  float ln_eps = 1e-6f;
   int max_ctas = 0;
   int reverse_m = 0;
 };
@@ -50,6 +54,8 @@
 
 inline long long gemm_w_pitch(int K) { return (static_cast<long long>(K) + 7) / 8 * 8; }
 
+bool gemm_ln_a_supported(int D);
+
 int gemm_bf16(const GemmArgs& args, const void* A, long long lda, const void* W, int block_n, cudaStream_t stream);
 
 }
diff --git a/wild_visual_navigation_b200/csrc/gemm_wgmma.cu b/wild_visual_navigation_b200/csrc/gemm_wgmma.cu
--- a/wild_visual_navigation_b200/csrc/gemm_wgmma.cu
+++ b/wild_visual_navigation_b200/csrc/gemm_wgmma.cu
@@ -5,6 +5,7 @@
 #include "common.cuh"
 #include "gemm.h"
 #include "host_common.h"
+#include "layernorm_row.cuh"
 
 namespace wvn {
 
@@ -37,16 +38,23 @@
 template <int EPI>
 constexpr bool kStaged = EPI == EPI_BF16 || EPI == EPI_F32 || EPI == EPI_RESID_F32 || EPI == EPI_QKV || EPI == EPI_BF16_RESID;
 
-template <int BN, int EPI>
+template <int BN, int EPI, int LN = 0>
 struct GemmCfg {
-  static constexpr uint32_t kABytes = BM * BK * 2;
+  static constexpr uint32_t kATileBytes = BM * BK * 2;
+  static constexpr uint32_t kABytes = LN ? 0 : kATileBytes;
   static constexpr uint32_t kBBytes = BN * BK * 2;
   static constexpr uint32_t kStageBytes = kABytes + kBBytes;
+  static constexpr int kABufs = 2;
+  static constexpr uint32_t kABlockBytes = BM * 128 * LN * 2;
+  static constexpr uint32_t kAResBytes = LN ? kABufs * kABlockBytes : 0;
   static constexpr uint32_t kSliceBytes = BM * kSliceCols * ((EPI == EPI_F32 || EPI == EPI_RESID_F32) ? 4 : 2);
   static constexpr uint32_t kStagingBytes = kStaged<EPI> ? 2 * 2 * kSliceBytes : 0;
-  static constexpr int kStagesRaw = (kMaxSmemBytes - kFixedSmemBytes - kStagingBytes) / kStageBytes;
+  static constexpr uint32_t kGammaBetaBytes = LN ? 2 * 128 * LN * 4 : 0;
+  static constexpr int kStagesRaw = (kMaxSmemBytes - kFixedSmemBytes - kStagingBytes -
+                                     static_cast<int>(kAResBytes + kGammaBetaBytes)) / static_cast<int>(kStageBytes);
   static constexpr int kStages = kStagesRaw > kMaxStages ? kMaxStages : kStagesRaw;
-  static constexpr uint32_t kSmemBytes = kStages * kStageBytes + kStagingBytes + kFixedSmemBytes;
+  static constexpr uint32_t kSmemBytes =
+      kStages * kStageBytes + kAResBytes + kStagingBytes + kGammaBetaBytes + kFixedSmemBytes;
   static constexpr int kN128 = BN / 128;
   static constexpr int kN64 = (BN % 128) / 64;
   static constexpr int kN32 = (BN % 64) / 32;
@@ -187,22 +195,96 @@
   }
 }
 
-template <int BN, int EPI, int ACT>
+template <int ITERS>
+__device__ __forceinline__ void ln_a_rows(const GemmArgs& args, const uint32_t base, const uint32_t gb, const int m_eff,
+                                          const int first, const int stride, const int lane) {
+  constexpr int D = 128 * ITERS;
+  for (int r = first; r < BM; r += 2 * stride) {
+    float4 v[2][ITERS];
+#pragma unroll
+    for (int h = 0; h < 2; ++h) {
+      const long long row = static_cast<long long>(m_eff) * BM + r + stride * h;
+      const float4* src = reinterpret_cast<const float4*>(args.ln_x + row * D);
+      const bool ok = r + stride * h < BM && row < args.M;
+#pragma unroll
+      for (int i = 0; i < ITERS; ++i) v[h][i] = ok ? __ldcs(src + lane + 32 * i) : make_float4(0.f, 0.f, 0.f, 0.f);
+    }
+#pragma unroll
+    for (int h = 0; h < 2; ++h) {
+      const int rr = r + stride * h;
+      if (rr >= BM) break;
+      if (static_cast<long long>(m_eff) * BM + rr < args.M) {
+        const float rstd = ln_row_center<ITERS>(v[h], args.ln_eps);
+#pragma unroll
+        for (int i = 0; i < ITERS; ++i)
+          v[h][i] = ln_row_affine(v[h][i], rstd, lds128f(gb + (lane + 32 * i) * 16),
+                                  lds128f(gb + (D + 4 * (lane + 32 * i)) * 4));
+      }
+#pragma unroll
+      for (int i = 0; i < ITERS; ++i) {
+        const int c4 = lane + 32 * i;
+        sts64u(base + (c4 >> 4) * (BM * 128) + rr * 128 + ((((c4 & 15) >> 1) ^ (rr & 7)) << 4) + (c4 & 1) * 8,
+               pack_bf16x2(v[h][i].x, v[h][i].y), pack_bf16x2(v[h][i].z, v[h][i].w));
+      }
+    }
+  }
+}
+
+constexpr int kFirstBlockWarps = 3 + kConsumerWarps;
+
+template <int ITERS, int NBUF>
+__device__ __forceinline__ void ln_a_fill(const GemmArgs& args, uint8_t* smem_a, float* smem_gb, uint64_t* a_full,
+                                          uint64_t* a_empty, const int num_m, const int nw, const int lane) {
+  constexpr int D = 128 * ITERS;
+  constexpr uint32_t kBlockBytes = BM * D * 2;
+  for (int i = nw * 32 + lane; i < D / 4; i += 96) {
+    reinterpret_cast<float4*>(smem_gb)[i] = __ldg(reinterpret_cast<const float4*>(args.ln_gamma) + i);
+    reinterpret_cast<float4*>(smem_gb + D)[i] = __ldg(reinterpret_cast<const float4*>(args.ln_beta) + i);
+  }
+  named_bar_sync(5, 32 * kFirstBlockWarps);
+  const uint32_t gb = smem_u32(smem_gb);
+  auto block_rows = [&](int m_eff) { return min(BM, args.M - m_eff * BM); };
+  auto m_of = [&](int m_blk) { return args.reverse_m ? num_m - 1 - m_blk : m_blk; };
+  int j = 0;
+  for (int m_blk = blockIdx.x; m_blk < num_m; m_blk += gridDim.x, ++j) {
+    const int m_eff = m_of(m_blk);
+    if (nw == 0 && lane == 0 && m_blk + static_cast<int>(gridDim.x) < num_m) {
+      const int mn = m_of(m_blk + gridDim.x);
+      l2_prefetch_bulk(args.ln_x + static_cast<long long>(mn) * BM * D, block_rows(mn) * D * 4);
+    }
+    const int buf = j % NBUF;
+    mbar_wait(&a_empty[buf], ((j / NBUF) & 1) ^ 1);
+    const uint32_t base = smem_u32(smem_a) + buf * kBlockBytes;
+    if (j == 0) ln_a_rows<ITERS>(args, base, gb, m_eff, nw, kFirstBlockWarps, lane);
+    else ln_a_rows<ITERS>(args, base, gb, m_eff, nw, 3, lane);
+    fence_proxy_async_smem();
+    __syncwarp();
+    if (lane == 0) {
+      if (j > 0 && nw == 0) mbar_arrive_cnt(&a_full[buf], 1 + kConsumerWarps);
+      else mbar_arrive(&a_full[buf]);
+    }
+  }
+}
+
+template <int BN, int EPI, int ACT, int LN>
 __global__ void __launch_bounds__(kNumThreads, 1)
 gemm_bf16_kernel(const __grid_constant__ CUtensorMap tmap_a, const __grid_constant__ CUtensorMap tmap_b,
                  const __grid_constant__ CUtensorMap tmap_c0, const __grid_constant__ CUtensorMap tmap_c1,
                  const __grid_constant__ CUtensorMap tmap_c2, const GemmArgs args) {
-  using Cfg = GemmCfg<BN, EPI>;
+  using Cfg = GemmCfg<BN, EPI, LN>;
   constexpr int STAGES = Cfg::kStages;
 
   extern __shared__ uint8_t smem_raw[];
   uint8_t* smem = reinterpret_cast<uint8_t*>((reinterpret_cast<uintptr_t>(smem_raw) + 1023) & ~uintptr_t(1023));
   uint8_t* smem_b = smem;
   uint8_t* smem_a = smem + STAGES * Cfg::kBBytes;
-  uint8_t* smem_c = smem_a + STAGES * Cfg::kABytes;
+  uint8_t* smem_c = smem_a + (LN ? Cfg::kAResBytes : STAGES * Cfg::kABytes);
   uint64_t* bars = reinterpret_cast<uint64_t*>(smem_c + Cfg::kStagingBytes);
+  uint8_t* smem_gb = smem_c + Cfg::kStagingBytes + 1024;
   uint64_t* full_bar = bars;
   uint64_t* empty_bar = bars + kMaxStages;
+  uint64_t* a_full = bars + 2 * kMaxStages;
+  uint64_t* a_empty = bars + 2 * kMaxStages + 2;
 
   const int warp = threadIdx.x >> 5;
   const int lane = threadIdx.x & 31;
@@ -210,21 +292,26 @@
   const int num_m = (args.M + BM - 1) / BM;
   const int num_n = args.N / BN;
   const int num_k = (args.K + BK - 1) / BK;
-  constexpr bool ROW_OWNER = (EPI == EPI_MLP_HEAD);
+  constexpr bool ROW_OWNER = (EPI == EPI_MLP_HEAD) || LN > 0;
+  constexpr bool UNIT_ROW = (EPI == EPI_MLP_HEAD);
 
   if (threadIdx.x == 0) {
-    tma_prefetch_desc(&tmap_a);
+    if (!LN) tma_prefetch_desc(&tmap_a);
     tma_prefetch_desc(&tmap_b);
     for (int i = 0; i < kMaxStages; ++i) {
       mbar_init(&full_bar[i], 1);
       mbar_init(&empty_bar[i], kConsumerWarps / 2);
     }
+    for (int i = 0; i < 2; ++i) {
+      mbar_init(&a_full[i], kFirstBlockWarps);
+      mbar_init(&a_empty[i], kConsumerWarps);
+    }
     fence_mbar_init();
   }
   __syncthreads();
 
   if (warp < 4) {
-    setmaxnreg_dec<40>();
+    setmaxnreg_dec<LN ? 72 : 40>();
     if (warp == 0) {
       int stage = 0;
       uint32_t phase = 0;
@@ -234,16 +321,19 @@
           mbar_wait(&empty_bar[stage], phase ^ 1);
           if (elect_one_sync()) {
             mbar_arrive_expect_tx(&full_bar[stage], Cfg::kStageBytes);
-            tma_load_2d(&tmap_a, &full_bar[stage], smem_a + stage * Cfg::kABytes, kb * BK, m_eff * BM);
+            if (!LN) tma_load_2d(&tmap_a, &full_bar[stage], smem_a + stage * Cfg::kABytes, kb * BK, m_eff * BM);
             tma_load_2d(&tmap_b, &full_bar[stage], smem_b + stage * Cfg::kBBytes, kb * BK, it.n_blk * BN);
           }
           __syncwarp();
           if (++stage == STAGES) { stage = 0; phase ^= 1; }
         }
       }
+    } else if (LN) {
+      ln_a_fill<(LN > 0 ? LN : 1), Cfg::kABufs>(args, smem_a, reinterpret_cast<float*>(smem_gb), a_full, a_empty, num_m,
+                                                warp - 1, lane);
     }
   } else {
-    setmaxnreg_inc<232>();
+    setmaxnreg_inc<LN ? 216 : 232>();
     const int cwarp = warp - 4;
     const int wg = cwarp >> 2;
     const int row_local = (cwarp & 3) * 16 + (lane >> 2);
@@ -256,6 +346,14 @@
         tma_prefetch_desc(&tmap_c2);
       }
     }
+    if (LN) {
+      named_bar_sync(5, 32 * kFirstBlockWarps);
+      const int m_eff = args.reverse_m ? num_m - 1 - static_cast<int>(blockIdx.x) : static_cast<int>(blockIdx.x);
+      ln_a_rows<(LN > 0 ? LN : 1)>(args, smem_u32(smem_a), smem_u32(smem_gb), m_eff, 3 + cwarp, kFirstBlockWarps, lane);
+      fence_proxy_async_smem();
+      __syncwarp();
+      if (lane == 0) mbar_arrive(&a_full[0]);
+    }
     if (wg == 1) named_bar_arrive(1, 256);
     float acc128[Cfg::kN128 > 0 ? Cfg::kN128 : 1][64];
     float acc64[32];
@@ -265,18 +363,27 @@
     uint32_t phase = 0;
     int unit = 0;
     for (TileIter<ROW_OWNER> it(num_m, num_n); it.valid(); it.next()) {
-      const bool unit_end = !ROW_OWNER || it.n_blk == num_n - 1;
+      const bool unit_end = !UNIT_ROW || it.n_blk == num_n - 1;
       if ((unit & 1) != wg) {
         for (int kb = 0; kb < num_k; ++kb)
           if (++stage == STAGES) { stage = 0; phase ^= 1; }
         if (unit_end) ++unit;
         continue;
       }
-      if (!ROW_OWNER || it.n_blk == 0) named_bar_sync(1 + wg, 256);
+      if (!UNIT_ROW || it.n_blk == 0) named_bar_sync(1 + wg, 256);
+      int a_buf = 0;
+      uint32_t a_base = 0;
+      if (LN) {
+        const int j = (it.m_blk - static_cast<int>(blockIdx.x)) / static_cast<int>(gridDim.x);
+        a_buf = j % Cfg::kABufs;
+        mbar_wait(&a_full[a_buf], (j / Cfg::kABufs) & 1);
+        a_base = smem_u32(smem_a) + a_buf * Cfg::kABlockBytes;
+      }
       int prev_stage = 0;
       for (int kb = 0; kb < num_k; ++kb) {
         mbar_wait(&full_bar[stage], phase);
-        const uint64_t desc_a = make_sw128_kmajor_desc(smem_u32(smem_a + stage * Cfg::kABytes));
+        const uint64_t desc_a = make_sw128_kmajor_desc(LN ? a_base + kb * Cfg::kATileBytes
+                                                           : smem_u32(smem_a + stage * Cfg::kABytes));
         const uint32_t b_addr = smem_u32(smem_b + stage * Cfg::kBBytes);
 #pragma unroll
         for (int c = 0; c < Cfg::kN128; ++c) wgmma_fence_regs(acc128[c]);
@@ -303,14 +410,18 @@
         prev_stage = stage;
         if (++stage == STAGES) { stage = 0; phase ^= 1; }
       }
-      if (unit_end && (ROW_OWNER ? it.m_blk + static_cast<int>(gridDim.x) < num_m : it.lin + static_cast<int>(gridDim.x) < num_m * num_n))
-        named_bar_arrive(2 - wg, 256);
+      const bool last_block = it.m_blk + static_cast<int>(gridDim.x) >= num_m;
+      const bool last_unit = UNIT_ROW ? last_block
+                             : ROW_OWNER ? last_block && it.n_blk == num_n - 1
+                                         : it.lin + static_cast<int>(gridDim.x) >= num_m * num_n;
+      if (unit_end && !last_unit) named_bar_arrive(2 - wg, 256);
       wgmma_wait<0>();
 #pragma unroll
       for (int c = 0; c < Cfg::kN128; ++c) wgmma_fence_regs(acc128[c]);
       if (Cfg::kN64) wgmma_fence_regs(acc64);
       if (Cfg::kN32) wgmma_fence_regs(acc32);
       if (lane == 0) mbar_arrive(&empty_bar[prev_stage]);
+      if (LN && it.n_blk >= num_n - 2 && lane == 0) mbar_arrive(&a_empty[a_buf]);
 
       const int m_eff = args.reverse_m ? num_m - 1 - it.m_blk : it.m_blk;
       const int row_tile = m_eff * BM;
@@ -362,19 +473,19 @@
   }
 }
 
-template <int BN, int EPI, int ACT>
+template <int BN, int EPI, int ACT, int LN = 0>
 int launch_gemm(const GemmArgs& a, const CUtensorMap& ta, const CUtensorMap& tb, const CUtensorMap (&tc)[3],
                 cudaStream_t stream) {
-  using Cfg = GemmCfg<BN, EPI>;
+  using Cfg = GemmCfg<BN, EPI, LN>;
   static_assert(Cfg::kStages >= 2, "tile too wide for the shared-memory budget");
-  auto kern = gemm_bf16_kernel<BN, EPI, ACT>;
+  auto kern = gemm_bf16_kernel<BN, EPI, ACT, LN>;
   static bool attr_set = false;
   if (!attr_set) {
     WVN_CHECK_CUDA(cudaFuncSetAttribute(kern, cudaFuncAttributeMaxDynamicSharedMemorySize, kMaxSmemBytes));
     attr_set = true;
   }
   const int num_m = (a.M + BM - 1) / BM, num_n = a.N / BN;
-  const int num_tiles = (EPI == EPI_MLP_HEAD) ? num_m : num_m * num_n;
+  const int num_tiles = (EPI == EPI_MLP_HEAD || LN > 0) ? num_m : num_m * num_n;
   int grid = sm_count();
   if (a.max_ctas > 0 && a.max_ctas < grid) grid = a.max_ctas;
   if (grid > num_tiles) grid = num_tiles;
@@ -419,7 +530,22 @@
   return set_error(WVN_ERR_INVALID, "gemm: unsupported epilogue/activation combination (%d, %d)", a.epi, a.act);
 }
 
-}
+int dispatch_ln(const GemmArgs& a, int block_n, const CUtensorMap& tb, const CUtensorMap (&tc)[3], cudaStream_t s) {
+  const CUtensorMap ta = {};
+  if (block_n == 192) {
+    if (a.epi == EPI_QKV && a.act == ACT_NONE) return launch_gemm<192, EPI_QKV, ACT_NONE, 3>(a, ta, tb, tc, s);
+    if (a.epi == EPI_F32 && a.act == ACT_NONE) return launch_gemm<192, EPI_F32, ACT_NONE, 3>(a, ta, tb, tc, s);
+    if (a.epi == EPI_BF16 && a.act == ACT_GELU) return launch_gemm<192, EPI_BF16, ACT_GELU, 3>(a, ta, tb, tc, s);
+  }
+  if (block_n == 256 && a.epi == EPI_BF16 && a.act == ACT_GELU)
+    return launch_gemm<256, EPI_BF16, ACT_GELU, 3>(a, ta, tb, tc, s);
+  return set_error(WVN_ERR_INVALID, "gemm: no LN-A kernel for block_n=%d epilogue %d activation %d", block_n, a.epi,
+                   a.act);
+}
+
+}
+
+bool gemm_ln_a_supported(int D) { return D == 384; }
 
 int pick_block_n(int N) {
   if (N % 256 == 0) return 256;
@@ -432,7 +558,7 @@
 
 int gemm_bf16(const GemmArgs& a, const void* A, long long lda, const void* W, int block_n, cudaStream_t stream) {
   WVN_REQUIRE(a.M > 0 && a.N > 0 && a.K > 0, "gemm: empty problem (M=%d N=%d K=%d)", a.M, a.N, a.K);
-  WVN_REQUIRE(lda >= a.K, "gemm: lda=%lld is smaller than K=%d", lda, a.K);
+  WVN_REQUIRE(a.ln_x != nullptr || lda >= a.K, "gemm: lda=%lld is smaller than K=%d", lda, a.K);
   if (block_n == 0) {
     block_n = pick_block_n(a.N);
     if (a.epi == EPI_BF16_RESID && block_n > kResidMaxBlockN) block_n = a.N % 192 == 0 ? 192 : (a.N % 128 == 0 ? 128 : 64);
@@ -460,8 +586,13 @@
   if (a.epi == EPI_BF16_RESID)
     WVN_REQUIRE(a.residual != nullptr && a.ldr >= a.N && a.ldr % 2 == 0,
                 "gemm: the residual epilogue needs a bf16 residual with an even pitch ldr >= N (ldr=%lld N=%d)", a.ldr, a.N);
+  const bool ln = a.ln_x != nullptr;
+  if (ln)
+    WVN_REQUIRE(gemm_ln_a_supported(a.K) && a.ln_gamma != nullptr && a.ln_beta != nullptr && a.N / block_n >= 2 &&
+                    (a.epi == EPI_QKV || a.epi == EPI_F32 || a.epi == EPI_BF16),
+                "gemm: bad LN-A arguments (D=%d N=%d block_n=%d epilogue %d)", a.K, a.N, block_n, a.epi);
   CUtensorMap ta, tb, tc[3] = {};
-  WVN_PROPAGATE(make_tmap_bf16_2d(&ta, A, a.K, a.M, static_cast<uint64_t>(lda) * 2, BK, BM));
+  if (!ln) WVN_PROPAGATE(make_tmap_bf16_2d(&ta, A, a.K, a.M, static_cast<uint64_t>(lda) * 2, BK, BM));
   WVN_PROPAGATE(make_tmap_bf16_2d(&tb, W, a.K, a.N, static_cast<uint64_t>(gemm_w_pitch(a.K)) * 2, BK, block_n));
   if (a.epi == EPI_BF16 || a.epi == EPI_BF16_RESID)
     WVN_PROPAGATE(make_tmap_2d(&tc[0], a.out, 2, a.N, a.M, static_cast<uint64_t>(a.ldo) * 2, kSliceCols, BM, 64));
@@ -473,6 +604,7 @@
     WVN_PROPAGATE(make_tmap_2d(&tc[1], a.k, 2, 64, bh * a.npad, 128, kSliceCols, BM, 64));
     WVN_PROPAGATE(make_tmap_2d(&tc[2], a.vt, 2, a.npad, bh * 64, static_cast<uint64_t>(a.npad) * 2, BM, kSliceCols, 128));
   }
+  if (ln) return dispatch_ln(a, block_n, tb, tc, stream);
   switch (block_n) {
     case 64: return dispatch_epi<64>(a, ta, tb, tc, stream);
     case 128: return dispatch_epi<128>(a, ta, tb, tc, stream);
diff --git a/wild_visual_navigation_b200/csrc/layernorm_row.cuh b/wild_visual_navigation_b200/csrc/layernorm_row.cuh
--- /dev/null
+++ b/wild_visual_navigation_b200/csrc/layernorm_row.cuh
@@ -0,0 +1,36 @@
+#pragma once
+
+#include "common.cuh"
+
+namespace wvn {
+
+template <int ITERS>
+__device__ __forceinline__ float ln_row_center(float4 (&v)[ITERS], const float eps) {
+  constexpr float kInvD = 1.f / (128 * ITERS);
+  float s = 0.f;
+#pragma unroll
+  for (int i = 0; i < ITERS; ++i) s = __fadd_rn(s, __fadd_rn(__fadd_rn(v[i].x, v[i].y), __fadd_rn(v[i].z, v[i].w)));
+  const float total = warp_sum(s);
+  float q = 0.f;
+#pragma unroll
+  for (int i = 0; i < ITERS; ++i) {
+    v[i].x = __fmaf_rn(total, -kInvD, v[i].x);
+    v[i].y = __fmaf_rn(total, -kInvD, v[i].y);
+    v[i].z = __fmaf_rn(total, -kInvD, v[i].z);
+    v[i].w = __fmaf_rn(total, -kInvD, v[i].w);
+    q = __fadd_rn(q, __fadd_rn(__fmaf_rn(v[i].x, v[i].x, __fmul_rn(v[i].y, v[i].y)),
+                               __fmaf_rn(v[i].z, v[i].z, __fmul_rn(v[i].w, v[i].w))));
+  }
+  return rsqrtf(__fmaf_rn(warp_sum(q), kInvD, eps));
+}
+
+__device__ __forceinline__ float4 ln_row_affine(const float4 d, const float rstd, const float4 g, const float4 b) {
+  float4 y;
+  y.x = __fmaf_rn(g.x, __fmul_rn(d.x, rstd), b.x);
+  y.y = __fmaf_rn(g.y, __fmul_rn(d.y, rstd), b.y);
+  y.z = __fmaf_rn(g.z, __fmul_rn(d.z, rstd), b.z);
+  y.w = __fmaf_rn(g.w, __fmul_rn(d.w, rstd), b.w);
+  return y;
+}
+
+}
diff --git a/wild_visual_navigation_b200/csrc/vit_kernels.cu b/wild_visual_navigation_b200/csrc/vit_kernels.cu
--- a/wild_visual_navigation_b200/csrc/vit_kernels.cu
+++ b/wild_visual_navigation_b200/csrc/vit_kernels.cu
@@ -1,5 +1,6 @@
 #include "common.cuh"
 #include "host_common.h"
+#include "layernorm_row.cuh"
 #include "vit_kernels.h"
 
 namespace wvn {
@@ -86,20 +87,9 @@
     const long long row = a.reverse ? a.rows - 1 - r : r;
     const float4* src = reinterpret_cast<const float4*>(x + row * D);
     float4 v[ITERS];
-    float s = 0.f;
-#pragma unroll
-    for (int i = 0; i < ITERS; ++i) {
-      v[i] = src[lane + 32 * i];
-      s += (v[i].x + v[i].y) + (v[i].z + v[i].w);
-    }
-    const float mean = warp_sum(s) * (1.f / D);
-    float q = 0.f;
-#pragma unroll
-    for (int i = 0; i < ITERS; ++i) {
-      const float dx = v[i].x - mean, dy = v[i].y - mean, dz = v[i].z - mean, dw = v[i].w - mean;
-      q += (dx * dx + dy * dy) + (dz * dz + dw * dw);
-    }
-    const float rstd = rsqrtf(warp_sum(q) * (1.f / D) + a.eps);
+#pragma unroll
+    for (int i = 0; i < ITERS; ++i) v[i] = src[lane + 32 * i];
+    const float rstd = ln_row_center<ITERS>(v, a.eps);
     long long f32_row = -1;
     if (out_f32 != nullptr) {
       const int tok = static_cast<int>(row % a.npad);
@@ -109,13 +99,8 @@
 #pragma unroll
     for (int i = 0; i < ITERS; ++i) {
       const int c4 = lane + 32 * i;
-      const float4 g = __ldg(reinterpret_cast<const float4*>(gamma) + c4);
-      const float4 bt = __ldg(reinterpret_cast<const float4*>(beta) + c4);
-      float4 y;
-      y.x = (v[i].x - mean) * rstd * g.x + bt.x;
-      y.y = (v[i].y - mean) * rstd * g.y + bt.y;
-      y.z = (v[i].z - mean) * rstd * g.z + bt.z;
-      y.w = (v[i].w - mean) * rstd * g.w + bt.w;
+      const float4 y = ln_row_affine(v[i], rstd, __ldg(reinterpret_cast<const float4*>(gamma) + c4),
+                                     __ldg(reinterpret_cast<const float4*>(beta) + c4));
       if (out_bf16 != nullptr) {
         uint2 p = make_uint2(pack_bf16x2(y.x, y.y), pack_bf16x2(y.z, y.w));
         *reinterpret_cast<uint2*>(out_bf16 + row * D + 4 * c4) = p;
```

Result: faster. 989.7, median of 6 (+1.9%).
